# xinyandai/gradient-quantization

Measured on AMD Instinct MI355X. Metric: gradient elements quantized/sec (HSQ d=16 k=8), higher is better.
Workload: dtype f32; 1 GPU; synthetic 25,000,000-float32 flat gradient per rank, HSQ c_dim=16 k_bit=8 n_bit=6 (BASELINE configs[1]), step = encode+levels+decode-mean; elements_per_rank=25000000, random=0, ranks=1, wire_levels=bytes, wire_bytes_per_rank=3125040, inputs=3 gradients of 100 MB used in turn (never Infinity-Cache resident)

## Files before the change

### gradient-quantization_amd/build.py

```python
#!/usr/bin/env python3
import os
import shutil
import subprocess
import sys

HERE = os.path.dirname(os.path.abspath(__file__))
ROOT = os.path.dirname(HERE)
CSRC = os.path.join(HERE, "csrc")
LIB = os.path.join(HERE, "libgq_hsq.so")
TOPK_LIB = os.path.join(HERE, "libgq_topk.so")
TOPK_SOURCES = ["topk.hip"]
SIGN_LIB = os.path.join(HERE, "libgq_sign.so")
SIGN_SOURCES = ["sign.hip"]
PVQ_LIB = os.path.join(HERE, "libgq_pvq.so")
PVQ_SOURCES = ["pvq_batched.hip"]
RQ_LIB = os.path.join(HERE, "libgq_rq.so")
RQ_SOURCES = ["rq_batched.hip"]
SOURCES = ["gq_common.hip", "gq_api.hip", "hsq_encode.hip", "hsq_encode_pf.hip", "hsq_encode_pfd.hip", "hsq_levels.hip", "hsq_batched.hip", "hsq_decode.hip", "qsgd.hip", "qsgd_batched.hip", "qsgd_wide.hip", "pvq.hip"]
FLAGS = ["--offload-arch=gfx950", "-O3", "-ffp-contract=off", "-fPIC", "-shared", "-std=c++17",
         "-Xclang", "-target-feature", "-Xclang", "-packed-fp32-ops",
         "-fvisibility=hidden", "-I" + os.path.join(ROOT, "include"), "-I" + CSRC]


def hipcc():
    for c in (os.environ.get("HIPCC"), shutil.which("hipcc"), "/opt/rocm/bin/hipcc"):
        if c and os.path.exists(c):
            return c
    raise RuntimeError("hipcc not found (ROCm toolchain required)")


HOST_EXT = os.path.join(HERE, "gq_amd", "_gq_host.so")


def needs_build():
    if (not os.path.exists(LIB) or not os.path.exists(os.path.join(HERE, "libgq_hsq_clock.so")) or not os.path.exists(HOST_EXT)
            or not os.path.exists(TOPK_LIB) or not os.path.exists(SIGN_LIB) or not os.path.exists(PVQ_LIB) or not os.path.exists(RQ_LIB)):
        return True
    t = min(os.path.getmtime(LIB), os.path.getmtime(HOST_EXT), os.path.getmtime(TOPK_LIB), os.path.getmtime(SIGN_LIB), os.path.getmtime(PVQ_LIB),
            os.path.getmtime(RQ_LIB))
    deps = ([os.path.join(CSRC, f) for f in os.listdir(CSRC)] + [os.path.join(ROOT, "include", h) for h in ("gq_hsq.h", "gq_topk.h", "gq_sign.h", "gq_pvq.h", "gq_rq.h")]
            + [__file__])
    return any(os.path.getmtime(d) > t for d in deps)


EXTRA = {
    "hsq_encode_pf.hip": ["-fno-honor-nans"],
    "hsq_encode_pfd.hip": ["-fno-honor-nans", "-mllvm", "-amdgpu-mfma-vgpr-form=1"],
    "pvq.hip": ["-mllvm", "-amdgpu-mfma-vgpr-form=1"],
    "pvq_batched.hip": ["-mllvm", "-amdgpu-mfma-vgpr-form=1"],
    "rq_batched.hip": ["-mllvm", "-amdgpu-mfma-vgpr-form=1"],
}


def build(force=False, verbose=False):
    if not force and not needs_build():
        return LIB
    objdir = os.path.join(HERE, "build")
    os.makedirs(objdir, exist_ok=True)
    compile_flags = [f for f in FLAGS if f != "-shared"]
    procs = []
    for src in SOURCES:
        obj = os.path.join(objdir, src.replace(".hip", ".o"))
        cmd = [hipcc()] + compile_flags + EXTRA.get(src, []) + ["-c", os.path.join(CSRC, src), "-o", obj]
        if verbose:
            print(" ".join(cmd))
        procs.append((cmd, subprocess.Popen(cmd), obj))
    topk_objs, sign_objs, pvq_objs, rq_objs = [], [], [], []
    for srcs, own in ((TOPK_SOURCES, topk_objs), (SIGN_SOURCES, sign_objs), (PVQ_SOURCES, pvq_objs), (RQ_SOURCES, rq_objs)):
        for src in srcs:
            obj = os.path.join(objdir, src.replace(".hip", ".o"))
            cmd = [hipcc()] + compile_flags + EXTRA.get(src, []) + ["-c", os.path.join(CSRC, src), "-o", obj]
            if verbose:
                print(" ".join(cmd))
            procs.append((cmd, subprocess.Popen(cmd), obj))
            own.append(obj)
    objs = []
    for cmd, p, obj in procs:
        if p.wait() != 0:
            raise subprocess.CalledProcessError(p.returncode, cmd)
        if obj not in topk_objs and obj not in sign_objs and obj not in pvq_objs and obj not in rq_objs:
            objs.append(obj)
    link = [hipcc(), "--offload-arch=gfx950", "-shared", "-fPIC", "-o", LIB] + objs
    if verbose:
        print(" ".join(link))
    host = None
    try:
        host = build_host_ext(verbose, wait=False)
    except Exception as e:
        print("build.py: host helper not built (%s); gq_amd falls back to its Python walks" % (e,), file=sys.stderr)
    try:
        subprocess.check_call(link)
        subprocess.check_call([hipcc(), "--offload-arch=gfx950", "-shared", "-fPIC", "-o", TOPK_LIB] + topk_objs)
        subprocess.check_call([hipcc(), "--offload-arch=gfx950", "-shared", "-fPIC", "-o", SIGN_LIB] + sign_objs)
        subprocess.check_call([hipcc(), "--offload-arch=gfx950", "-shared", "-fPIC", "-o", PVQ_LIB] + pvq_objs)
        subprocess.check_call([hipcc(), "--offload-arch=gfx950", "-shared", "-fPIC", "-o", RQ_LIB] + rq_objs)
        build_clock_lib(objs, verbose)
    finally:
        if host is not None and host[1].wait() != 0:
            print("build.py: host helper failed to compile (exit %d); gq_amd falls back to its Python walks" % host[1].returncode,
                  file=sys.stderr)
    return LIB


def build_host_ext(verbose=False, wait=True):
    import sysconfig
    import torch
    from torch.utils import cpp_extension as ce
    cmd = (["g++", "-O2", "-std=c++17", "-fPIC", "-shared", "-fvisibility=hidden",
            "-D_GLIBCXX_USE_CXX11_ABI=%d" % int(torch._C._GLIBCXX_USE_CXX11_ABI)]
           + ["-I" + d for d in ce.include_paths() + [sysconfig.get_paths()["include"]]]
           + [os.path.join(CSRC, "host_ext.cpp"), "-o", HOST_EXT]
           + ["-L" + d for d in ce.library_paths()] + ["-ltorch", "-ltorch_cpu", "-ltorch_python", "-lc10"]
           + ["-Wl,-rpath," + d for d in ce.library_paths()])
    if verbose:
        print(" ".join(cmd))
    p = subprocess.Popen(cmd)
    if wait and p.wait() != 0:
        raise subprocess.CalledProcessError(p.returncode, cmd)
    return cmd, p


CLOCK_LIB = os.path.join(HERE, "libgq_hsq_clock.so")


def build_clock_lib(objs=None, verbose=False, source=None, out=None):
    objdir = os.path.join(HERE, "build")
    if objs is None:
        objs = [os.path.join(objdir, f.replace(".hip", ".o")) for f in SOURCES]
    src = source or os.path.join(CSRC, "hsq_encode_pf.hip")
    obj = os.path.join(objdir, "stamps", "hsq_encode_pf_stamps.o" if out is None else os.path.basename(out) + ".o")
    os.makedirs(os.path.dirname(obj), exist_ok=True)
    flags = [f for f in FLAGS if f != "-shared"] + EXTRA.get("hsq_encode_pf.hip", [])
    cmd = [hipcc()] + flags + ["-DGQ_PF_STAMPS", "-c", src, "-o", obj]
    if verbose:
        print(" ".join(cmd))
    subprocess.check_call(cmd, stderr=None if verbose else subprocess.DEVNULL)
    others = [o for o in objs if os.path.basename(o) != "hsq_encode_pf.o"]
    subprocess.check_call([hipcc(), "--offload-arch=gfx950", "-shared", "-fPIC", "-o", out or CLOCK_LIB, obj] + others)
    return out or CLOCK_LIB


if __name__ == "__main__":
    print(build(force="--force" in sys.argv, verbose=True))
```

### gradient-quantization_amd/csrc/gq_internal.h

```cpp
#pragma once
#include "gq_common.hpp"

GQ_INTERNAL int gqi_hsq_encode_batched_pf(const int64_t *seg_table, const int32_t *tile_seg, int nseg, int64_t ntiles,
                                          const float *codebook, int d, int K, int ef, float ef_scale, uint8_t *wire, float *u_flat,
                                          uint32_t *seg_minmax, float *workspace, int profile_slot, void *stream);
GQ_INTERNAL int gqi_hsq_encode_batched_paged(const int64_t *seg_table, const int32_t *tile_seg, int nseg, int64_t ntiles,
                                             const float *codebook, int d, int K, int ef, float ef_scale, uint8_t *wire,
                                             float *u_flat, uint32_t *seg_minmax, float *workspace, void *stream);
GQ_INTERNAL int gqi_hsq_batched_any_supported(int d, int K);
GQ_INTERNAL int gqi_hsq_encode_batched_any(const int64_t *seg_table, const int32_t *tile_seg, int nseg, int64_t ntiles,
                                           const float *codebook, int d, int K, int code_bytes, int ef, float ef_scale,
                                           uint8_t *wire, float *u_flat, uint32_t *seg_minmax, void *stream);

GQ_INTERNAL int gqi_hsq_levels_batched_d16(const int64_t *seg_table, const int32_t *tile_seg, int nseg, int64_t ntiles,
                                           const float *u_flat, const uint32_t *seg_minmax, int n_bit, int random_mode,
                                           uint64_t seed, const float *r_flat, const float *ef_codebook, int K, int packed6,
                                           uint8_t *wire, const int64_t *dense_table, int ndense, void *stream);
GQ_INTERNAL int gqi_hsq_levels_batched_ef_d(const int64_t *seg_table, const int32_t *tile_seg, int nseg, int64_t ntiles,
                                            const float *u_flat, const uint32_t *seg_minmax, int n_bit, int random_mode,
                                            uint64_t seed, const float *r_flat, const float *codebook, int d, int K, uint8_t *wire, const int64_t *dense_table, int ndense,
                                            void *stream);
GQ_INTERNAL int gqi_hsq_levels_batched_ef16(const int64_t *seg_table, const int32_t *tile_seg, int nseg, int64_t ntiles,
                                            const float *u_flat, const uint32_t *seg_minmax, int n_bit, int random_mode,
                                            uint64_t seed, const float *r_flat, const float *codebook, int d, int K, uint8_t *wire,
                                            const int64_t *dense_table, int ndense, void *stream);
GQ_INTERNAL int gqi_hsq_levels_decode_batched(const int64_t *seg_table, const int32_t *tile_seg, int nseg, int64_t ntiles,
                                              const float *u_flat, const uint32_t *seg_minmax, int n_bit, int random_mode,
                                              uint64_t seed, const float *r_flat, const float *codebook, int d, int K, int level_bytes,
                                              uint8_t *wire, const int64_t *dense_table, int ndense, int write_error, float *out,
                                              int plain, const gq::FusedTail *ft, void *stream);
GQ_INTERNAL int gqi_hsq_levels_batched_any(const int64_t *seg_table, const int32_t *tile_seg, int nseg, int64_t ntiles,
                                           const float *u_flat, const uint32_t *seg_minmax, int n_bit, int random_mode,
                                           uint64_t seed, const float *r_flat, int level_bytes, uint8_t *wire, const int64_t *dense_table, int ndense, void *stream);
GQ_INTERNAL int gqi_hsq_error_batched_any(const int64_t *seg_table, const int32_t *tile_seg, int nseg, int64_t ntiles,
                                          const uint8_t *wire, const float *codebook, int d, int K, int code_bytes,
                                          int level_bytes, int n_bit, void *stream);

GQ_INTERNAL int gqi_hsq_decode_sum_batched_d16(const int64_t *seg_table, const int32_t *tile_seg, int nseg, int64_t ntiles,
                                               const uint8_t *gathered, int64_t user_stride_bytes, int R,
                                               const float *codebook, int K, int n_bit, int packed6, float *out, int plain,
                                               const gq::StepTail *tail_or_null, int *tail_taken, void *stream);
GQ_INTERNAL int gqi_hsq_decode_sum_batched_d(const int64_t *seg_table, const int32_t *tile_seg, int nseg, int64_t ntiles,
                                             const uint8_t *gathered, int64_t user_stride_bytes, int R,
                                             const float *codebook, int d, int K, int level_bytes, int n_bit, float *out, int plain,
                                             const gq::StepTail *tail_or_null, int *tail_taken, void *stream);
GQ_INTERNAL int gqi_hsq_decode_sum_batched_any(const int64_t *seg_table, const int32_t *tile_seg, int nseg, int64_t ntiles,
                                               const uint8_t *gathered, int64_t user_stride_bytes, int R,
                                               const float *codebook, int d, int K, int code_bytes, int level_bytes,
                                               int n_bit, float *out, int plain, void *stream);

GQ_INTERNAL int gqi_qsgd_compress_batched(const int64_t *seg_table, const int32_t *bucket_seg, int nseg, int64_t nbuckets,
                                          int n_bit, int random_mode, uint64_t seed, int ef, float ef_scale, uint8_t *wire, const int64_t *dense_table, int ndense,
                                          int bucket_hint, void *stream);
GQ_INTERNAL int gqi_qsgd_decode_sum_batched(const int64_t *seg_table, const int32_t *bucket_seg, int nseg, int64_t nbuckets,
                                            int n_bit, int bits, const uint8_t *gathered, int64_t user_stride_bytes, int R,
                                            float *out, int plain, const gq::StepTail *tail_or_null, int *tail_taken, int bucket_hint,
                                            void *stream);
GQ_INTERNAL int gqi_qsgd_wide_compress(const int64_t *seg_table, const int32_t *chunk_seg, int nseg, int64_t nchunks,
                                       int n_bit, int random_mode, uint64_t seed, int ef, float ef_scale,
                                       uint32_t *norm_bits, uint8_t *wire, const int64_t *dense_table, int ndense, void *stream);
GQ_INTERNAL int gqi_qsgd_wide_decode_sum(const int64_t *seg_table, const int32_t *chunk_seg, int nseg, int64_t nchunks,
                                         int n_bit, int bits, const uint8_t *gathered, int64_t user_stride_bytes, int R,
                                         float *out, int plain, const gq::StepTail *tail_or_null, int *tail_taken, void *stream);
```

### gradient-quantization_amd/csrc/hsq_encode_pf.hip

```cpp
#include <hip/hip_ext.h>

#include <type_traits>

#include "hsq_pf_common.hpp"

#ifdef GQ_PF_STAMPS
#define GQ_STAMP(ID)                                                                                  \
    {                                                                                                 \
        __builtin_amdgcn_sched_barrier(0);                                                            \
        unsigned long long ts_;                                                                       \
        asm volatile("s_memtime %0\n\ts_waitcnt lgkmcnt(0)" : "=s"(ts_)::"memory");                   \
        __builtin_amdgcn_sched_barrier(0);                                                            \
        stamp_acc[ID] += (ts_ - ts_prev);                                                             \
        ts_prev = ts_;                                                                                \
    }
#define GQ_STAMPS_ONLY(...) __VA_ARGS__
#define GQ_LOG_SCAN(...)
#else
#define GQ_STAMP(ID)
#define GQ_STAMPS_ONLY(...)
#define GQ_LOG_SCAN(...) __VA_ARGS__
#endif

namespace gq {

constexpr int PF_WAVES = 8;
constexpr int PF_THREADS = PF_WAVES * 64;
#ifndef GQ_PF_TAIL
#define GQ_PF_TAIL 4
#endif
constexpr int PF_TAIL = GQ_PF_TAIL;
#ifndef GQ_PF_FLUSH_AHEAD
#define GQ_PF_FLUSH_AHEAD 0
#endif
#ifndef GQ_PF_PAIR
#define GQ_PF_PAIR -1
#endif
#ifndef GQ_PF_FLUSH_MIN
#define GQ_PF_FLUSH_MIN 3
#endif
#ifndef GQ_PF_SCAN1_MAX
#define GQ_PF_SCAN1_MAX 4
#endif
constexpr int PF_FLUSH_AHEAD = GQ_PF_FLUSH_AHEAD;
constexpr int PF_FLUSH_MIN = GQ_PF_FLUSH_MIN;
constexpr int PF_SCAN1_MAX = GQ_PF_SCAN1_MAX;
constexpr int PF_LDS_SEGS = 384;
template <int D>
struct PfShape {
    static_assert(D == 8 || D == 16 || D == 32, "the prefilter kernel is built for D = 8, 16 and 32");
    static constexpr int KS = D > 16 ? D / 16 : 1;
    static constexpr bool HALF = D < 16;
    static constexpr int QS = 4 * D + 4;
    static constexpr int QCAP = D > 16 ? 32 : 64;
    static constexpr bool A_REGS = D <= 16;
    static constexpr int NF = 4 * KS;
    static constexpr bool PAIR = GQ_PF_PAIR < 0 ? D > 16 : GQ_PF_PAIR != 0;
    static constexpr float ERR_REL = (D > 16 ? 1.05f : 1.03f) * 4.8828125e-04f;
    static constexpr float ERR2_REL = (D > 16 ? 2.3f : 1.2f) * 7.62939453125e-06f;
    static constexpr float ERR2_SUB = D > 16 ? 3.5e-7f : 2.4e-7f;
};
constexpr float ERR_ABS = 4.76837158203125e-07f;
constexpr unsigned N2_LO_BITS = 0x39800000u;
constexpr unsigned N2_HI_BITS = 0x4B800000u;
constexpr int SIGMA_TARGET_EXP2 = 10;

struct PfArgs {
    const float *grad;
    int64_t M;
    void *codes;
    float *u;
    const float *cb;
    float *ws;
    const int64_t *seg_table;
    const int32_t *tile_seg;
    uint8_t *wire;
    unsigned *seg_minmax;
    int64_t ntiles;
    int nseg;
    int K;
    float ef_scale;
    int tiles_q, tiles_r;
    int tiles_skew, skew_blocks;
};

#ifndef GQ_PF_SKEW_PERMILLE
#define GQ_PF_SKEW_PERMILLE 10
#endif
static void pf_split(PfArgs &a, int64_t ntiles, int64_t blocks) {
    a.tiles_q = (int)(ntiles / blocks);
    a.tiles_r = (int)(ntiles % blocks);
    a.skew_blocks = (int)(blocks & ~(int64_t)1);
    a.tiles_skew = (int)((a.tiles_q * (int64_t)GQ_PF_SKEW_PERMILLE + 500) / 1000);
    if (a.tiles_skew >= a.tiles_q) a.tiles_skew = 0;
}

template <typename CodeT, int D, bool BATCHED, bool EF = false, bool SEGLDS = true, int DR = D, int NRB = 8>
__global__ __launch_bounds__(PF_THREADS, 1) void hsq_encode_pf_kernel(const PfArgs a) {
    typedef PfShape<D> SH;
    static_assert(DR == D || (D == 16 && DR == 12) || (D == 32 && DR == 24), "padded shapes: 12 -> 16, 24 -> 32");
    static_assert(NRB == 1 || NRB == 2 || NRB == 4 || NRB == 8, "row blocks: 1, 2, 4 or 8");
    const int K = a.K;
    constexpr int KS = SH::KS, QS = SH::QS, QCAP = SH::QCAP, NF = SH::NF;
    constexpr bool HALF = SH::HALF, PF_PAIR = SH::PAIR;
    GQ_STAMPS_ONLY(const unsigned long long rt_entry = __builtin_amdgcn_s_memrealtime(); unsigned long long nscanned = 0, npassed = 0;)
    const float *__restrict__ cb = a.cb;
    float *__restrict__ ws = a.ws;
    float *__restrict__ u = a.u;
    const int64_t M = a.M;
    __shared__ __attribute__((aligned(16))) float s_cb[64 * QS];
    __shared__ int s_next;
    __shared__ int s_pairdone[PF_WAVES / 2], s_ringpub[PF_WAVES];
    __shared__ int64_t s_seg[(BATCHED && SEGLDS) ? PF_LDS_SEGS * 8 : 1];
    __shared__ __attribute__((aligned(16))) u32x4 s_frag[8 * KS * 64], s_fragl[8 * KS * 64];
    __shared__ float s_c1[PF_WAVES], s_dc[PF_WAVES];
    __shared__ __attribute__((aligned(16))) float s_qv[PF_WAVES * QCAP * D];
    __shared__ __attribute__((aligned(16))) unsigned s_qm[PF_WAVES * QCAP * 4];

    constexpr int PF_MM_SEGS = 64;
    __shared__ unsigned s_mm[BATCHED ? 2 * PF_MM_SEGS : 2];
    const int lane = threadIdx.x & 63, wave = __builtin_amdgcn_readfirstlane((int)(threadIdx.x >> 6));
    const int j = lane & 31, h = lane >> 5;

    const int64_t ntiles = BATCHED ? a.ntiles : ((M + 63) >> 6);
    const int b = (int)blockIdx.x;
    const bool skewed = b < a.skew_blocks;
    const int lo_tile = b * a.tiles_q + (b < a.tiles_r ? b : a.tiles_r) + ((skewed && (b & 1)) ? a.tiles_skew : 0);
    const int tile_end = lo_tile + a.tiles_q + (b < a.tiles_r ? 1 : 0) + (skewed ? ((b & 1) ? -a.tiles_skew : a.tiles_skew) : 0);
    const int tail_from = (tile_end - lo_tile) - (wave >= PF_WAVES / 2 ? PF_TAIL : 0);
    auto draw = [&]() {
        int k = 0x3FFFFFFF;
        if (lane == 0) {
            if (__hip_atomic_load(&s_next, __ATOMIC_RELAXED, __HIP_MEMORY_SCOPE_WORKGROUP) < tail_from)
                k = __hip_atomic_fetch_add(&s_next, 1, __ATOMIC_RELAXED, __HIP_MEMORY_SCOPE_WORKGROUP);
        }
        return lo_tile + __builtin_amdgcn_readfirstlane(k);
    };
    int t = lo_tile + wave;
    int *const worklist = ws_worklist(ws);

    float lmin = INFINITY, lmax = -INFINITY;
    bool sawnan = false;
    int cur_seg = -1;
    int seg_first = 0;
    f32x4 cur[NF], nxt[NF];
    f32x4 nxte[NF];
    if (HALF) {
#pragma unroll
        for (int i = 0; i < NF; ++i) cur[i] = nxt[i] = nxte[i] = f32x4{0.0f, 0.0f, 0.0f, 0.0f};
    }

    typedef const float __attribute__((address_space(1))) *gcf_ptr;
    typedef float __attribute__((address_space(1))) *gf_ptr;
    typedef const f32x4 __attribute__((address_space(1))) *gcv_ptr;
    typedef f32x4 __attribute__((address_space(1))) *gv_ptr;
    typedef CodeT __attribute__((address_space(1))) *gcode_ptr;
    struct Tile {
        gcf_ptr base;
        int64_t m, sv0;
        int tile0;
        int tiles_end;
        int rem;
        int seg;
        gcode_ptr codes;
        gcf_ptr err;
    };
    auto uniform64 = [](int64_t v) {
        const unsigned lo = (unsigned)__builtin_amdgcn_readfirstlane((int)(unsigned)(uint64_t)v);
        const unsigned hi = (unsigned)__builtin_amdgcn_readfirstlane((int)(unsigned)((uint64_t)v >> 32));
        return (int64_t)(((uint64_t)hi << 32) | lo);
    };
    auto tile_info = [&](int tile, int seg, auto from_global) {
        constexpr bool FROM_GLOBAL = decltype(from_global)::value;
        Tile ti;
        if (BATCHED) {
            ti.seg = seg;
            int64_t r0, r1, r2, r3, r7 = 0;
            if constexpr (SEGLDS && !FROM_GLOBAL) {
                const int64_t *rec = s_seg + 8 * seg;
                r0 = rec[0];
                r1 = rec[1];
                r2 = rec[2];
                r3 = rec[3];
                if (EF) r7 = rec[7];
            } else {
                typedef const int64_t __attribute__((address_space(1))) *grec_ptr;
                const grec_ptr rec = (grec_ptr)(a.seg_table + 8 * (int64_t)seg);
                r0 = rec[0];
                r1 = rec[1];
                r2 = rec[2];
                r3 = rec[3];
                if (EF) r7 = rec[7];
            }
            ti.base = (gcf_ptr)(uintptr_t)uniform64(r0);
            ti.m = uniform64(r1);
            ti.tile0 = (int)uniform64(r2);
            ti.tiles_end = ti.tile0 + (int)((ti.m + 63) >> 6);
            ti.sv0 = (int64_t)(tile - ti.tile0) * 64;
            ti.codes = (gcode_ptr)((uintptr_t)a.wire + (uintptr_t)uniform64(r3));
            ti.err = EF ? (gcf_ptr)(uintptr_t)uniform64(r7) : (gcf_ptr)0;
            const int rem = (int)ti.m - 1 - (int)ti.sv0;
            ti.rem = rem > 63 ? 63 : rem;
        } else {
            ti.seg = 0;
            ti.tile0 = 0;
            ti.tiles_end = 0;
            ti.base = (gcf_ptr)a.grad;
            ti.m = M;
            ti.sv0 = (int64_t)tile * 64;
            ti.codes = (gcode_ptr)static_cast<CodeT *>(a.codes);
            ti.err = (gcf_ptr)0;
            const int rem = (int)M - 1 - (int)ti.sv0;
            ti.rem = rem > 63 ? 63 : rem;
        }
        return ti;
    };
    auto lane_off = [&](const Tile &ti, int blk) {
        const unsigned li = min((unsigned)(blk * 32 + j), (unsigned)ti.rem);
        return li * (unsigned)DR + (HALF ? 0u : 8u * (unsigned)h);
    };
    auto frag_ok = [&](int s_, int q_) { return DR == D || 16 * s_ + 4 * q_ + 4 + 8 * h <= DR; };
    const bool loads_here = !HALF || h == 0;
    auto load_rows = [&](gcf_ptr tb, const Tile &ti, f32x4(&dst)[NF]) {
        if (loads_here) {
#pragma unroll
            for (int blk = 0; blk < 2; ++blk) {
                const gcv_ptr p = (gcv_ptr)(tb + lane_off(ti, blk));
#pragma unroll
                for (int s = 0; s < KS; ++s) {
                    const f32x4 z = {0.0f, 0.0f, 0.0f, 0.0f};
                    dst[(blk * KS + s) * 2] = frag_ok(s, 0) ? p[4 * s] : z;
                    dst[(blk * KS + s) * 2 + 1] = frag_ok(s, 1) ? p[4 * s + 1] : z;
                }
            }
        }
    };
    auto load_tile = [&](const Tile &ti, f32x4(&dst)[NF]) { load_rows(ti.base + ti.sv0 * DR, ti, dst); };
    auto load_err = [&](const Tile &ti, f32x4(&dst)[NF]) {
        if (EF && ti.err) load_rows(ti.err + ti.sv0 * DR, ti, dst);
    };
    auto fold_err = [&](const Tile &ti, f32x4(&g)[NF], const f32x4(&e)[NF]) {
        if (EF && ti.err) {
            const gf_ptr tb = (gf_ptr)(ti.base + ti.sv0 * DR);
#pragma unroll
            for (int blk = 0; blk < 2; ++blk) {
#pragma unroll
                for (int q = 0; q < 2 * KS; ++q) {
                    f32x4 &x = g[2 * KS * blk + q];
                    const f32x4 &y = e[2 * KS * blk + q];
#pragma unroll
                    for (int c = 0; c < 4; ++c) {
                        const float prod = a.ef_scale * y[c];
                        x[c] = x[c] + prod;
                    }
                }
                if (blk * 32 + j <= ti.rem && loads_here) {
                    const gv_ptr p = (gv_ptr)(tb + (unsigned)((blk * 32 + j) * DR + (HALF ? 0 : 8 * h)));
#pragma unroll
                    for (int s = 0; s < KS; ++s) {
                        if (frag_ok(s, 0)) p[4 * s] = g[(blk * KS + s) * 2];
                        if (frag_ok(s, 1)) p[4 * s + 1] = g[(blk * KS + s) * 2 + 1];
                    }
                }
            }
        }
    };
    auto mm_fold = [&](int seg, unsigned mlo, unsigned mhi) {
        const unsigned idx = (unsigned)(seg - seg_first);
        if (idx < (unsigned)PF_MM_SEGS) {
            atomicMin(&s_mm[2 * idx], mlo);
            atomicMax(&s_mm[2 * idx + 1], mhi);
        } else {
            unsigned *mm = a.seg_minmax + 2 * seg;
            if (mlo < __hip_atomic_load(mm, __ATOMIC_RELAXED, __HIP_MEMORY_SCOPE_AGENT)) atomicMin(mm, mlo);
            if (mhi > __hip_atomic_load(mm + 1, __ATOMIC_RELAXED, __HIP_MEMORY_SCOPE_AGENT)) atomicMax(mm + 1, mhi);
        }
    };
    auto flush_minmax = [&]() {
        const float lo = wave_min(lmin), hi = wave_max(lmax);
        if (lane == 0 && cur_seg >= 0 && lo <= hi) mm_fold(cur_seg, order_map(lo), order_map(hi));
        lmin = INFINITY;
        lmax = -INFINITY;
    };

    half8 vh[2 * KS];
    float n2p[2] = {0.0f, 0.0f};
    Tile ti = {};

    float cbv[256 * DR / PF_THREADS];
#pragma unroll
    for (int n = 0; n < 256 * DR / PF_THREADS; ++n) cbv[n] = (int)threadIdx.x + n * PF_THREADS < K * DR ? cb[threadIdx.x + n * PF_THREADS] : 0.0f;
    f32x4 aq[2 * KS];
#pragma unroll
    for (int i = 0; i < 2 * KS; ++i) aq[i] = f32x4{0.0f, 0.0f, 0.0f, 0.0f};
    if (loads_here && wave * 32 + j < K) {
#pragma unroll
        for (int s = 0; s < KS; ++s) {
            if (frag_ok(s, 0)) aq[2 * s] = *reinterpret_cast<const f32x4 *>(cb + (wave * 32 + j) * DR + 16 * s + (HALF ? 0 : 8 * h));
            if (frag_ok(s, 1)) aq[2 * s + 1] = *reinterpret_cast<const f32x4 *>(cb + (wave * 32 + j) * DR + 16 * s + (HALF ? 0 : 8 * h) + 4);
        }
    }
    const int seg_first_v = (BATCHED && lo_tile < ntiles) ? a.tile_seg[lo_tile] : 0;
    if (t < tile_end) {
        ti = tile_info(t, BATCHED ? __builtin_amdgcn_readfirstlane(a.tile_seg[t]) : 0, std::true_type{});
        load_tile(ti, cur);
        load_err(ti, nxte);
    }
    if (threadIdx.x == 0) {
        s_next = PF_WAVES;
    }
    if (threadIdx.x < PF_WAVES / 2) s_pairdone[threadIdx.x] = 0;
    seg_first = BATCHED ? __builtin_amdgcn_readfirstlane(seg_first_v) : 0;
    if (BATCHED && threadIdx.x < PF_MM_SEGS) {
        s_mm[2 * threadIdx.x] = 0xFFFFFFFFu;
        s_mm[2 * threadIdx.x + 1] = 0u;
    }
#pragma unroll
    for (int n = 0; n < 256 * DR / PF_THREADS; ++n) {
        const int i = threadIdx.x + n * PF_THREADS, k = i / DR, jj = i % DR;
        s_cb[(k >> 2) * QS + 4 * jj + (k & 3)] = cbv[n];
    }
    if constexpr (DR != D) {
#pragma unroll
        for (int n = 0; n < 256 * (D - DR) / PF_THREADS; ++n) {
            const int i = threadIdx.x + n * PF_THREADS, k = i / (D - DR), jj = DR + i % (D - DR);
            s_cb[(k >> 2) * QS + 4 * jj + (k & 3)] = 0.0f;
        }
    }
    if (BATCHED && SEGLDS) {
        const int n = (a.nseg < PF_LDS_SEGS ? a.nseg : PF_LDS_SEGS) * 8;
        for (int i = threadIdx.x; i < n; i += PF_THREADS) s_seg[i] = a.seg_table[i];
    }
    {
        float l2 = 0.0f, d2 = 0.0f;
#pragma unroll
        for (int s = 0; s < KS; ++s) {
            half8 fh, fl;
#pragma unroll
            for (int e = 0; e < 8; ++e) {
                const float x = e < 4 ? aq[2 * s][e] : aq[2 * s + 1][e - 4];
                fh[e] = (_Float16)x;
                const float rr = x - (float)fh[e];
                fl[e] = (_Float16)rr;
                l2 = __fmaf_rn(x, x, l2);
                d2 = __fmaf_rn(rr, rr, d2);
            }
            s_frag[(wave * KS + s) * 64 + lane] = __builtin_bit_cast(u32x4, fh);
            s_fragl[(wave * KS + s) * 64 + lane] = __builtin_bit_cast(u32x4, fl);
        }
        l2 += __shfl_xor(l2, 32, 64);
        d2 += __shfl_xor(d2, 32, 64);
        l2 = wave_max_nan(l2);
        d2 = wave_max_nan(d2);
        if (lane == 0) {
            s_c1[wave] = l2;
            s_dc[wave] = d2;
        }
    }
    __syncthreads();
    half8 ch[SH::A_REGS ? 8 : 1];
    if constexpr (SH::A_REGS) {
#pragma unroll
        for (int rb = 0; rb < 8; ++rb) ch[rb] = __builtin_bit_cast(half8, s_frag[rb * 64 + lane]);
    }
    auto frag_hi = [&](int rb, int s) -> half8 {
        if constexpr (SH::A_REGS) return ch[rb];
        else return __builtin_bit_cast(half8, s_frag[(rb * KS + s) * 64 + lane]);
    };
    unsigned c2b = __float_as_uint(s_c1[0]), dcb = __float_as_uint(s_dc[0]);
#pragma unroll
    for (int w = 1; w < PF_WAVES; ++w) {
        c2b = max(c2b, __float_as_uint(s_c1[w]));
        dcb = max(dcb, __float_as_uint(s_dc[w]));
    }
    const float c2 = __builtin_sqrtf(__uint_as_float(c2b)) * 1.0000002f, dc = __builtin_sqrtf(__uint_as_float(dcb)) * 1.0000002f;
    const bool cb_ok = c2b < 0x4E800000u && dcb < 0x4E800000u;
    const float err_rel = cb_ok ? c2 * SH::ERR_REL + 1.001f * dc : INFINITY;
    const float err_abs = cb_ok ? c2 * ERR_ABS : INFINITY;
    const float err2_rel = cb_ok ? c2 * SH::ERR2_REL + SH::ERR2_SUB : INFINITY;

    int tn = draw();
    float sigma_t = 1.0f;
    if (t < tile_end) {
        fold_err(ti, cur, nxte);
        float m = 0.0f;
#pragma unroll
        for (int i = 0; i < NF; ++i) m = fmaxf(fmaxf(fabsf(cur[i][0]), fabsf(cur[i][1])), fmaxf(fmaxf(fabsf(cur[i][2]), fabsf(cur[i][3])), m));
        const unsigned em = (unsigned)__builtin_amdgcn_readfirstlane((int)(__float_as_uint(wave_max(m)) >> 23));
        if (em >= 1u && em <= 254u) {
            int f = 258 - (int)em;
            f = f < 27 ? 27 : (f > 227 ? 227 : f);
            sigma_t = __uint_as_float((unsigned)__builtin_amdgcn_readfirstlane(f << 23));
        }
#pragma unroll
        for (int blk = 0; blk < 2; ++blk)
#pragma unroll
            for (int s = 0; s < KS; ++s) scale8_f16(cur[(blk * KS + s) * 2], cur[(blk * KS + s) * 2 + 1], sigma_t, vh[blk * KS + s], n2p[blk]);
    }
    auto fold_seg = [&](int seg, float v) {
        const unsigned mv = order_map(v);
        mm_fold(seg, mv, mv);
    };
    auto poison_seg = [&](int seg) {
        atomicMin(a.seg_minmax + 2 * seg, MAPPED_NAN_LO);
        atomicMax(a.seg_minmax + 2 * seg + 1, MAPPED_NAN_HI);
    };
    int qhead = 0, qcnt = 0;
    bool flushed = false;
    const int run_len = tile_end - lo_tile;
    auto scan1 = [&](int slot) {
        GQ_STAMPS_ONLY(nscanned += 1;)
        float w[D];
        {
            const f32x4 *qv = reinterpret_cast<const f32x4 *>(s_qv + D * slot);
#pragma unroll
            for (int q = 0; q < D / 4; ++q) {
                const f32x4 x = qv[q];
                w[4 * q] = x[0];
                w[4 * q + 1] = x[1];
                w[4 * q + 2] = x[2];
                w[4 * q + 3] = x[3];
            }
        }
        f32x4 p = exact_score_quad<D>(s_cb + lane * QS, w);
        if (4 * lane >= K) p = f32x4{0.0f, 0.0f, 0.0f, 0.0f};
        float bv = p[0];
        int bi = 4 * lane;
        take_if_greater_nan(bv, bi, p[1], 4 * lane + 1);
        take_if_greater_nan(bv, bi, p[2], 4 * lane + 2);
        take_if_greater_nan(bv, bi, p[3], 4 * lane + 3);
        wave_first_max_nan_dpp(bv, bi);
        const bool isnan = nan_bits(bv);
        if (isnan) sawnan = true;
        if (lane == 0) {
            const u32x4 m = *reinterpret_cast<const u32x4 *>(s_qm + 4 * slot);
            *(gcode_ptr)(uintptr_t)((uint64_t)m[0] | ((uint64_t)m[1] << 32)) = (CodeT)bi;
            ((gf_ptr)u)[m[2]] = bv;
            if (BATCHED) {
                if (isnan) poison_seg((int)m[3]);
                else fold_seg((int)m[3], bv);
            } else {
                GQ_LOG_SCAN(worklist[m[2]] = (int)m[2];)
                lmin = fminf(lmin, bv);
                lmax = fmaxf(lmax, bv);
            }
        }
    };
    auto second_pass = [&](int first, int na, int wave_b, int first_b, int nb) {
        const int n = na + nb;
        GQ_STAMPS_ONLY(npassed += n;)
        auto slot_of = [&](int c) {
            return c < na ? wave * QCAP + ((first + c) & (QCAP - 1)) : wave_b * QCAP + ((first_b + c - na) & (QCAP - 1));
        };
        const int col = j < n ? j : 0;
        const int slot = slot_of(col);
        const f32x4 *qv = reinterpret_cast<const f32x4 *>(s_qv + D * slot);
        f32x4 xs[2 * KS];
#pragma unroll
        for (int s = 0; s < KS; ++s) {
            if (HALF) {
                const f32x4 z = {0.0f, 0.0f, 0.0f, 0.0f};
                xs[0] = h ? z : qv[0];
                xs[1] = h ? z : qv[1];
            } else {
                xs[2 * s] = qv[4 * s + 2 * h];
                xs[2 * s + 1] = qv[4 * s + 2 * h + 1];
            }
        }
        auto both_halves = [&](float own, bool add) {
            float a = own, b = own;
            swap32(a, b);
            return add ? a + b : fmaxf(a, b);
        };
        float m = 0.0f;
#pragma unroll
        for (int i = 0; i < 2 * KS; ++i)
            m = fmaxf(fmaxf(fmaxf(fabsf(xs[i][0]), fabsf(xs[i][1])), fmaxf(fabsf(xs[i][2]), fabsf(xs[i][3]))), m);
        m = both_halves(m, false);
        const unsigned em = __float_as_uint(m) >> 23;
        int f = 258 - (int)em;
        f = f < 27 ? 27 : (f > 227 ? 227 : f);
        const float sig = (em >= 1u && em <= 254u) ? __uint_as_float((unsigned)f << 23) : 1.0f;
        half8 bh[KS], bl[KS];
        float n2q = 0.0f;
#pragma unroll
        for (int s = 0; s < KS; ++s) {
            u32x4 H, L;
            const f32x4 x0 = xs[2 * s], x1 = xs[2 * s + 1];
#pragma unroll
            for (int i = 0; i < 4; ++i) {
                const float a = i < 2 ? x0[2 * i] : x1[2 * i - 4], b = i < 2 ? x0[2 * i + 1] : x1[2 * i - 3];
                unsigned r, l;
                asm("v_fma_mixlo_f16 %0, %1, %2, 0" : "=v"(r) : "v"(a), "v"(sig));
                asm("v_fma_mixhi_f16 %0, %1, %2, 0" : "+v"(r) : "v"(b), "v"(sig));
                asm("v_fma_mixlo_f16 %0, %1, %2, -%3 op_sel_hi:[0,0,1]" : "=v"(l) : "v"(a), "v"(sig), "v"(r));
                asm("v_fma_mixhi_f16 %0, %1, %2, -%3 op_sel:[0,0,1] op_sel_hi:[0,0,1]" : "+v"(l) : "v"(b), "v"(sig), "v"(r));
                const unsigned e = r & 0x7C007C00u;
                asm("v_dot2_f32_f16 %0, %1, %1, %0" : "+v"(n2q) : "v"(e));
                H[i] = r;
                L[i] = l;
            }
            bh[s] = __builtin_bit_cast(half8, H);
            bl[s] = __builtin_bit_cast(half8, L);
        }
        const float n2 = both_halves(n2q, true);
        unsigned best2[2] = {0, 0}, second2[2] = {0, 0};
        unsigned vmask = KEY_MASK;
        asm volatile("" : "+v"(vmask));
        half8 al[KS], ah[KS];
        auto frags_of = [&](int rb) {
#pragma unroll
            for (int s = 0; s < KS; ++s) {
                al[s] = __builtin_bit_cast(half8, s_fragl[(rb * KS + s) * 64 + lane]);
                ah[s] = frag_hi(rb, s);
            }
        };
        auto chain3 = [&](f32x16 c) {
#pragma unroll
            for (int s = 0; s < KS; ++s) {
                c = __builtin_amdgcn_mfma_f32_32x32x16_f16(al[s], bh[s], c, 0, 0, 0);
                c = __builtin_amdgcn_mfma_f32_32x32x16_f16(ah[s], bl[s], c, 0, 0, 0);
                c = __builtin_amdgcn_mfma_f32_32x32x16_f16(ah[s], bh[s], c, 0, 0, 0);
            }
            return c;
        };
        frags_of(0);
        f32x16 acc = {0};
        acc = chain3(acc);
        if (NRB > 1) frags_of(1);
#pragma unroll
        for (int rb = 0; rb < NRB; ++rb) {
            f32x16 nacc = {0};
            if (rb + 1 < NRB) {
                __builtin_amdgcn_sched_barrier(0);
                nacc = chain3(nacc);
                if (rb + 2 < NRB) frags_of(rb + 2);
                __builtin_amdgcn_sched_barrier(0);
            }
            unsigned k[4];
#pragma unroll
            for (int q = 0; q < 4; ++q)
                k[q] = and_or(__float_as_uint(absmax4(acc[4 * q], acc[4 * q + 1], acc[4 * q + 2], acc[4 * q + 3])), vmask,
                              (unsigned)((rb & 3) * 4 + q));
            const int trk = rb >> 2;
            const unsigned t0 = max3u(best2[trk], k[0], k[1]), a0 = med3u(best2[trk], k[0], k[1]);
            const unsigned b0 = med3u(t0, k[2], k[3]);
            best2[trk] = max3u(t0, k[2], k[3]);
            second2[trk] = max3u(second2[trk], a0, b0);
            __builtin_amdgcn_sched_barrier(0);
            acc = nacc;
        }
        const bool useB = (best2[1] & KEY_MASK) > (best2[0] & KEY_MASK);
        const unsigned bw = useB ? best2[1] : best2[0], blo = useB ? best2[0] : best2[1];
        const int gid = (int)(bw & 31u);
        const int kmine = ((gid >> 2) + (useB ? 4 : 0)) * 32 + 8 * (gid & 3) + 4 * h;
        const unsigned smine = max3u(second2[0], second2[1], blo) | 31u;
        int k0 = kmine, k1_ = kmine;
        swap32(k0, k1_);
        int s0 = (int)smine, s1 = (int)smine;
        swap32(s0, s1);
        int w0 = (int)bw, w1 = (int)bw;
        swap32(w0, w1);
        const bool pick1 = ((unsigned)w1 & KEY_MASK) > ((unsigned)w0 & KEY_MASK);
        const int kc = pick1 ? k1_ : k0;
        const unsigned rest = max3u((unsigned)s0, (unsigned)s1, (unsigned)(pick1 ? w0 : w1) | 31u);
        float vf[D];
#pragma unroll
        for (int q = 0; q < D / 4; ++q) {
            const f32x4 x = qv[q];
            vf[4 * q] = x[0];
            vf[4 * q + 1] = x[1];
            vf[4 * q + 2] = x[2];
            vf[4 * q + 3] = x[3];
        }
        const f32x4 p4 = exact_score_quad<D>(s_cb + (kc >> 2) * QS, vf);
        float val = p4[0];
        int idx = kc;
        take_if_greater(val, idx, p4[1], kc + 1);
        take_if_greater(val, idx, p4[2], kc + 2);
        take_if_greater(val, idx, p4[3], kc + 3);
        const unsigned n2b = __float_as_uint(n2);
        const float E = __builtin_amdgcn_sqrtf(n2) * err2_rel + err_abs;
        bool safe = ((n2b - N2_LO_BITS) <= (N2_HI_BITS - N2_LO_BITS)) && (__uint_as_float(rest) + E < fabsf(val * sig));
        if (nan_bits(val)) safe = false;
        const bool owner = h == 0 && j < n;
        if (owner && safe) {
            const u32x4 mt = *reinterpret_cast<const u32x4 *>(s_qm + 4 * slot);
            *(gcode_ptr)(uintptr_t)((uint64_t)mt[0] | ((uint64_t)mt[1] << 32)) = (CodeT)idx;
            ((gf_ptr)u)[mt[2]] = val;
            if (BATCHED) {
                fold_seg((int)mt[3], val);
            } else {
                GQ_LOG_SCAN(worklist[mt[2]] = (int)mt[2];)
                lmin = fminf(lmin, val);
                lmax = fmaxf(lmax, val);
            }
        }
        uint64_t left = __ballot(owner && !safe);
        while (left) {
            const int i = __builtin_ctzll(left);
            left &= left - 1;
            scan1(slot_of(i));
        }
    };
    GQ_STAMPS_ONLY(const unsigned long long rt0 = __builtin_amdgcn_s_memrealtime(); unsigned long long ntl = 0, stamp_acc[6] = {0, 0, 0, 0, 0, 0}, ts_prev;
                   asm volatile("s_memtime %0\n\ts_waitcnt lgkmcnt(0)" : "=s"(ts_prev)::"memory");)
    while (t < tile_end) {
        auto chain_rb = [](int c) { return SH::A_REGS ? (c % NRB) : (c >> 1); };
        auto chain_blk = [](int c) { return SH::A_REGS ? (c / NRB) : (c & 1); };
        half8 af[2][KS];
        if constexpr (!SH::A_REGS) {
#pragma unroll
            for (int s = 0; s < KS; ++s) af[0][s] = frag_hi(0, s);
        }
        auto chain = [&](int c, f32x16 x) {
            const int rb = chain_rb(c), blk = chain_blk(c);
#pragma unroll
            for (int s = 0; s < KS; ++s)
                x = __builtin_amdgcn_mfma_f32_32x32x16_f16(SH::A_REGS ? ch[SH::A_REGS ? rb : 0] : af[rb & 1][s], vh[blk * KS + s], x, 0, 0, 0);
            return x;
        };
        f32x16 acc = {0};
        acc = chain(0, acc);
        __builtin_amdgcn_sched_barrier(0);
        Tile tin = ti;
        if (tn < tile_end) {
            if (BATCHED && tn >= ti.tile0 && tn < ti.tiles_end) {
                tin.sv0 = (int64_t)(tn - ti.tile0) * 64;
                const int rem = (int)ti.m - 1 - (int)tin.sv0;
                tin.rem = rem > 63 ? 63 : rem;
            } else {
                tin = tile_info(tn, BATCHED ? __builtin_amdgcn_readfirstlane(a.tile_seg[tn]) : 0, std::false_type{});
            }
            load_tile(tin, nxt);
            load_err(tin, nxte);
        }
        if (BATCHED && ti.seg != cur_seg) {
            flush_minmax();
            cur_seg = ti.seg;
        }
        GQ_STAMP(0)
        unsigned best[4] = {0, 0, 0, 0}, second[4] = {0, 0, 0, 0};
        unsigned vmask = KEY_MASK;
        asm volatile("" : "+v"(vmask));
        auto group_key = [&](const f32x16 &a, int rb, int q) {
            return and_or(__float_as_uint(absmax4(a[4 * q], a[4 * q + 1], a[4 * q + 2], a[4 * q + 3])), vmask,
                          (unsigned)((rb & 3) * 4 + q));
        };
        unsigned trk_t = 0, trk_a = 0;
        auto track_lo = [&](int trk, unsigned k0, unsigned k1) {
            trk_t = max3u(best[trk], k0, k1);
            trk_a = med3u(best[trk], k0, k1);
        };
        auto track_hi = [&](int trk, unsigned k2, unsigned k3) {
            const unsigned b = med3u(trk_t, k2, k3);
            best[trk] = max3u(trk_t, k2, k3);
            second[trk] = max3u(second[trk], trk_a, b);
        };
#pragma unroll
        for (int c = 0; c < 2 * NRB; ++c) {
            const int rb = chain_rb(c), trk = chain_blk(c) * 2 + (rb >> 2);
            if constexpr (!SH::A_REGS) {
                if (chain_blk(c) == 0 && rb + 1 < NRB) {
#pragma unroll
                    for (int s = 0; s < KS; ++s) af[(rb + 1) & 1][s] = frag_hi(rb + 1, s);
                }
            }
            if (c + 1 < 2 * NRB) {
                f32x16 nacc = {0};
                __builtin_amdgcn_sched_barrier(0);
                nacc = chain(c + 1, nacc);
                __builtin_amdgcn_sched_barrier(0);
                track_lo(trk, group_key(acc, rb, 0), group_key(acc, rb, 1));
                track_hi(trk, group_key(acc, rb, 2), group_key(acc, rb, 3));
                __builtin_amdgcn_sched_barrier(0);
                acc = nacc;
            } else {
                track_lo(trk, group_key(acc, rb, 0), group_key(acc, rb, 1));
                track_hi(trk, group_key(acc, rb, 2), group_key(acc, rb, 3));
            }
        }

        GQ_STAMP(1)
        int k1[2];
        unsigned s2[2], bk[2];
#pragma unroll
        for (int blk = 0; blk < 2; ++blk) {
            const unsigned bA = best[2 * blk], bB = best[2 * blk + 1];
            const bool useB = (bB & KEY_MASK) > (bA & KEY_MASK);
            const unsigned bw = useB ? bB : bA, bl = useB ? bA : bB;
            const int gid = (int)(bw & 31u);
            k1[blk] = ((gid >> 2) + (useB ? 4 : 0)) * 32 + 8 * (gid & 3) + 4 * h;
            s2[blk] = max3u(second[2 * blk], second[2 * blk + 1], bl) | 31u;
            bk[blk] = bw;
        }

        float vf[D];
#pragma unroll
        for (int s = 0; s < KS; ++s) {
#pragma unroll
            for (int e = 0; e < 8; ++e) {
                float x = cur[2 * s + (e >> 2)][e & 3];
                float y = cur[2 * KS + 2 * s + (e >> 2)][e & 3];
                swap32(x, y);
                vf[16 * s + e] = x;
                if (!HALF) vf[(16 * s + 8 + e) % D] = y;
            }
        }
        swap32(k1[0], k1[1]);
        {
            int a0 = (int)s2[0], a1 = (int)s2[1];
            swap32(a0, a1);
            s2[0] = (unsigned)a0;
            s2[1] = (unsigned)a1;
            int b0 = (int)bk[0], b1 = (int)bk[1];
            swap32(b0, b1);
            bk[0] = (unsigned)b0;
            bk[1] = (unsigned)b1;
        }
        float n2 = n2p[0];
        {
            float n2o = n2p[1];
            swap32(n2, n2o);
            n2 += n2o;
        }
        const unsigned n2b = __float_as_uint(n2);

        GQ_STAMP(2)
        const bool pick1 = (bk[1] & KEY_MASK) > (bk[0] & KEY_MASK);
        const int kc = pick1 ? k1[1] : k1[0];
        const unsigned rest = max3u(s2[0], s2[1], (pick1 ? bk[0] : bk[1]) | 31u);
        const f32x4 p4 = exact_score_quad<D>(s_cb + (kc >> 2) * QS, vf);
        float val = p4[0];
        int idx = kc;
        take_if_greater(val, idx, p4[1], kc + 1);
        take_if_greater(val, idx, p4[2], kc + 2);
        take_if_greater(val, idx, p4[3], kc + 3);

        const float E = __builtin_amdgcn_sqrtf(n2) * err_rel + err_abs;
        const float others = __uint_as_float(rest);
        const bool in_window = (n2b - N2_LO_BITS) <= (N2_HI_BITS - N2_LO_BITS);
        bool safe = in_window && (others + E < fabsf(val * sigma_t));
        if (nan_bits(val)) safe = false;
        if (__ballot(n2b == 0u)) {
            unsigned any = 0;
#pragma unroll
            for (int e = 0; e < D; e += 2) any |= (__float_as_uint(vf[e]) | __float_as_uint(vf[e + 1])) & 0x7FFFFFFFu;
            if (any == 0u && !nan_bits(val)) {
                safe = true;
                val = 0.0f;
                idx = 0;
            }
        }

        const bool valid = lane <= ti.rem;

        float sigma_n = sigma_t;
        {
            const unsigned s0 = (unsigned)__builtin_amdgcn_readlane((int)n2b, 5), s1 = (unsigned)__builtin_amdgcn_readlane((int)n2b, 58);
            const unsigned smp = s0 > s1 ? s0 : s1;
            if (smp != 0u) {
                const int e2 = (int)(smp >> 23);
                const int k = e2 >= 255 ? -16 : ((127 + SIGMA_TARGET_EXP2 - e2) >> 1);
                int f = (int)((unsigned)__builtin_amdgcn_readfirstlane((int)__float_as_uint(sigma_t)) >> 23) + k;
                f = f < 27 ? 27 : (f > 227 ? 227 : f);
                sigma_n = __uint_as_float((unsigned)f << 23);
            }
        }

        GQ_STAMP(3)
        int dk_seen = 0x3FFFFFFF;
        if (lane == 0) dk_seen = __hip_atomic_load(&s_next, __ATOMIC_RELAXED, __HIP_MEMORY_SCOPE_WORKGROUP);
        half8 nvh[2 * KS];
        float nn2p[2] = {0.0f, 0.0f};
        if (EF && tn < tile_end) fold_err(tin, nxt, nxte);
#pragma unroll
        for (int blk = 0; blk < 2; ++blk)
#pragma unroll
            for (int s = 0; s < KS; ++s) scale8_f16(nxt[(blk * KS + s) * 2], nxt[(blk * KS + s) * 2 + 1], sigma_n, nvh[blk * KS + s], nn2p[blk]);
#pragma unroll
        for (int i = 0; i < NF; ++i) cur[i] = nxt[i];
#pragma unroll
        for (int i = 0; i < 2 * KS; ++i) vh[i] = nvh[i];
#pragma unroll
        for (int blk = 0; blk < 2; ++blk) n2p[blk] = nn2p[blk];
        __builtin_amdgcn_sched_barrier(0);

        GQ_STAMP(4)
        int dk_next = 0x3FFFFFFF;
        if (lane == 0 && dk_seen < tail_from) dk_next = __hip_atomic_fetch_add(&s_next, 1, __ATOMIC_RELAXED, __HIP_MEMORY_SCOPE_WORKGROUP);
        const bool flagged = valid && !safe;
        uint64_t todo = __ballot(flagged);
        bool want_flush = PF_FLUSH_AHEAD > 0 && !flushed && (tn - lo_tile) >= run_len - PF_FLUSH_AHEAD;
        while (todo || want_flush) {
            const int rank = (int)__builtin_amdgcn_mbcnt_hi((unsigned)(todo >> 32), __builtin_amdgcn_mbcnt_lo((unsigned)todo, 0u));
            const bool mine = ((todo >> lane) & 1) && rank < QCAP - qcnt;
            if (mine) {
                const int slot = wave * QCAP + ((qhead + qcnt + rank) & (QCAP - 1));
                f32x4 *qv = reinterpret_cast<f32x4 *>(s_qv + D * slot);
#pragma unroll
                for (int q = 0; q < D / 4; ++q) qv[q] = f32x4{vf[4 * q], vf[4 * q + 1], vf[4 * q + 2], vf[4 * q + 3]};
                const uint64_t ca = (uint64_t)(uintptr_t)(ti.codes + ti.sv0) + (uint64_t)sizeof(CodeT) * (unsigned)lane;
                *reinterpret_cast<u32x4 *>(s_qm + 4 * slot) =
                    u32x4{(unsigned)ca, (unsigned)(ca >> 32), (unsigned)((BATCHED ? (int64_t)t * 64 : ti.sv0) + lane), (unsigned)ti.seg};
            }
            const uint64_t took = __ballot(mine);
            qcnt += (int)__builtin_popcountll(took);
            todo &= ~took;
            if (qcnt >= 32 || (want_flush && !todo)) {
                if (qcnt >= 32 || qcnt >= PF_FLUSH_MIN) {
                    const int n = qcnt < 32 ? qcnt : 32;
                    second_pass(qhead, n, wave, 0, 0);
                    qhead = (qhead + n) & (QCAP - 1);
                    qcnt -= n;
                    if (want_flush && !todo) flushed = true;
                }
                if (!todo) want_flush = false;
            }
        }

        if (valid && safe) {
            (ti.codes + ti.sv0)[(unsigned)lane] = (CodeT)idx;
            ((gf_ptr)u + (BATCHED ? (int64_t)t * 64 : ti.sv0))[(unsigned)lane] = val;
            lmin = fminf(lmin, val);
            lmax = fmaxf(lmax, val);
        }
        ti = tin;
        t = tn;
        tn = lo_tile + __builtin_amdgcn_readfirstlane(dk_next);
        sigma_t = sigma_n;
        GQ_STAMP(5)
        GQ_STAMPS_ONLY(++ntl;)
    }
    GQ_STAMPS_ONLY(const unsigned long long rt1 = __builtin_amdgcn_s_memrealtime();)
    if (BATCHED) flush_minmax();

    int other_first = 0, other_n = 0;
    const int partner = wave ^ (PF_WAVES / 2);
    if (PF_PAIR) {
        int old = 0;
        if (lane == 0) {
            __hip_atomic_store(&s_ringpub[wave], (qhead << 8) | qcnt, __ATOMIC_RELAXED, __HIP_MEMORY_SCOPE_WORKGROUP);
            old = __hip_atomic_fetch_add(&s_pairdone[wave & (PF_WAVES / 2 - 1)], 1, __ATOMIC_ACQ_REL, __HIP_MEMORY_SCOPE_WORKGROUP);
        }
        old = __builtin_amdgcn_readfirstlane(old);
        if (old == 0) {
            qcnt = 0;
        } else {
            int pub = 0;
            if (lane == 0) pub = __hip_atomic_load(&s_ringpub[partner], __ATOMIC_RELAXED, __HIP_MEMORY_SCOPE_WORKGROUP);
            pub = __builtin_amdgcn_readfirstlane(pub);
            other_first = pub >> 8;
            other_n = pub & 255;
        }
    }
    while (qcnt + other_n) {
        if (qcnt + other_n <= PF_SCAN1_MAX) {
            if (qcnt) {
                scan1(wave * QCAP + qhead);
                qhead = (qhead + 1) & (QCAP - 1);
                qcnt -= 1;
            } else {
                scan1(partner * QCAP + other_first);
                other_first = (other_first + 1) & (QCAP - 1);
                other_n -= 1;
            }
        } else {
            const int na = qcnt < 32 ? qcnt : 32, nb = other_n < 32 - na ? other_n : 32 - na;
            second_pass(qhead, na, partner, other_first, nb);
            qhead = (qhead + na) & (QCAP - 1);
            qcnt -= na;
            other_first = (other_first + nb) & (QCAP - 1);
            other_n -= nb;
        }
    }
#ifdef GQ_PF_STAMPS
    if (lane == 0 && blockIdx.x < 256) {
        unsigned long long *o = reinterpret_cast<unsigned long long *>(ws_worklist(ws) + (M - 65536)) + (blockIdx.x * 8 + wave) * 12;
        for (int i = 0; i < 6; ++i) o[i] = stamp_acc[i];
        o[6] = rt_entry, o[7] = rt0, o[8] = rt1, o[9] = ntl, o[10] = __builtin_amdgcn_s_memrealtime(), o[11] = 1000 * nscanned + npassed;
    }
#endif
    if (BATCHED) {
        __syncthreads();
        if (threadIdx.x < PF_MM_SEGS) {
            const unsigned lo = s_mm[2 * threadIdx.x], hi = s_mm[2 * threadIdx.x + 1];
            if (lo != 0xFFFFFFFFu || hi != 0u) {
                unsigned *mm = a.seg_minmax + 2 * (seg_first + (int)threadIdx.x);
                if (lo < __hip_atomic_load(mm, __ATOMIC_RELAXED, __HIP_MEMORY_SCOPE_AGENT)) atomicMin(mm, lo);
                if (hi > __hip_atomic_load(mm + 1, __ATOMIC_RELAXED, __HIP_MEMORY_SCOPE_AGENT)) atomicMax(mm + 1, hi);
            }
        }
        return;
    }
    write_minmax_partials<PF_WAVES>(lmin, lmax, ws, sawnan);
}

static int64_t pf16_grid(int64_t ntiles, int bpc) {
    int64_t blocks = (ntiles + PF_WAVES - 1) / PF_WAVES;
    int64_t cap = (int64_t)cu_count() * bpc;
    if (cap > GQ_MAIN_PARTIALS) cap = GQ_MAIN_PARTIALS;
    if (blocks > cap) blocks = cap;
    return blocks < 1 ? 1 : blocks;
}

template <typename CodeT, int D, int DR, int NRB>
static int launch_pf_rows(const float *grad, const float *codebook, int64_t M, int K, CodeT *codes, float *u, float *ws,
                          hipStream_t st, int profile_slot) {
    if (M > 0x7FFFFFFFLL) return fail(GQ_ERR_UNSUPPORTED, "gq_hsq_encode: prefilter path needs M < 2^31");
    static const int bpc = resident_blocks_per_cu(hsq_encode_pf_kernel<CodeT, D, false, false, true, DR, NRB>, PF_THREADS, 0);
    PfArgs a = {};
    a.grad = grad;
    a.M = M;
    a.codes = codes;
    a.u = u;
    a.cb = codebook;
    a.ws = ws;
    a.K = K;
    const int64_t blocks = pf16_grid((M + 63) / 64, bpc);
    pf_split(a, (M + 63) / 64, blocks);
    hipEvent_t ev_start, ev_stop;
    if (profile_events(profile_slot, &ev_start, &ev_stop)) {
        hipExtLaunchKernelGGL(HIP_KERNEL_NAME(hsq_encode_pf_kernel<CodeT, D, false, false, true, DR, NRB>), dim3((unsigned)blocks),
                              dim3(PF_THREADS), 0, st, ev_start, ev_stop, 0, a);
    } else {
        hipLaunchKernelGGL(HIP_KERNEL_NAME(hsq_encode_pf_kernel<CodeT, D, false, false, true, DR, NRB>), dim3((unsigned)blocks),
                           dim3(PF_THREADS), 0, st, a);
    }
    GQ_CHECK_LAUNCH("gq_hsq_encode (prefilter)");
    return GQ_OK;
}

template <typename CodeT, int D, int DR = D>
static int launch_pf(const float *grad, const float *codebook, int64_t M, int K, CodeT *codes, float *u, float *ws,
                     hipStream_t st, int profile_slot) {
    if constexpr (sizeof(CodeT) == 1) {
        if (K <= 32) return launch_pf_rows<CodeT, D, DR, 1>(grad, codebook, M, K, codes, u, ws, st, profile_slot);
        if (K <= 64) return launch_pf_rows<CodeT, D, DR, 2>(grad, codebook, M, K, codes, u, ws, st, profile_slot);
    }
    return launch_pf_rows<CodeT, D, DR, 8>(grad, codebook, M, K, codes, u, ws, st, profile_slot);
}

template <typename CodeT>
int launch_encode_pf(const float *grad, const float *codebook, int64_t M, int d, int K, CodeT *codes, float *u, float *ws,
                     hipStream_t st, int profile_slot) {
    if (K < 4 || K > 256 || (K & 3)) return fail(GQ_ERR_INVALID_ARG, "gq_hsq_encode: the prefilter kernel was asked for K = %d", K);
    if (d == 16) return launch_pf<CodeT, 16>(grad, codebook, M, K, codes, u, ws, st, profile_slot);
    if (d == 32) return launch_pf<CodeT, 32>(grad, codebook, M, K, codes, u, ws, st, profile_slot);
    if (d == 8) return launch_pf<CodeT, 8>(grad, codebook, M, K, codes, u, ws, st, profile_slot);
    if (d == 12) return launch_pf<CodeT, 16, 12>(grad, codebook, M, K, codes, u, ws, st, profile_slot);
    if (d == 24) return launch_pf<CodeT, 32, 24>(grad, codebook, M, K, codes, u, ws, st, profile_slot);
    return fail(GQ_ERR_INVALID_ARG, "gq_hsq_encode: the prefilter kernel was asked for d = %d", d);
}

template int launch_encode_pf<uint8_t>(const float *, const float *, int64_t, int, int, uint8_t *, float *, float *, hipStream_t, int);
template int launch_encode_pf<int32_t>(const float *, const float *, int64_t, int, int, int32_t *, float *, float *, hipStream_t, int);

}

namespace gq {
template <int D, bool EF, int DR, int NRB>
static int encode_batched_rows(const char *what, const int64_t *seg_table, const int32_t *tile_seg, int nseg, int64_t ntiles,
                               const float *codebook, int K, uint8_t *wire, float *u_flat, uint32_t *seg_minmax, float *workspace,
                               float ef_scale, int profile_slot, void *stream) {
    if (nseg < 1 || ntiles < 1 || ntiles * 64 > 0x7FFFFFFFLL)
        return fail(GQ_ERR_INVALID_ARG, "%s: bad sizes nseg=%d ntiles=%lld", what, nseg, (long long)ntiles);
    if (!seg_table || !tile_seg || !codebook || !wire || !u_flat || !seg_minmax || !workspace)
        return fail(GQ_ERR_INVALID_ARG, "%s: null pointer", what);
    static const int bpc = resident_blocks_per_cu(hsq_encode_pf_kernel<uint8_t, D, true, EF, true, DR, NRB>, PF_THREADS, 0);
    PfArgs a = {};
    a.K = K;
    a.M = ntiles * 64;
    a.u = u_flat;
    a.cb = codebook;
    a.ws = workspace;
    a.seg_table = seg_table;
    a.tile_seg = tile_seg;
    a.wire = wire;
    a.seg_minmax = seg_minmax;
    a.ntiles = ntiles;
    a.nseg = nseg;
    a.ef_scale = ef_scale;
    hipStream_t st = as_stream(stream);
    const int64_t blocks = pf16_grid(ntiles, bpc);
    pf_split(a, ntiles, blocks);
    hipEvent_t ev_start, ev_stop;
    if (nseg <= PF_LDS_SEGS && profile_events(profile_slot, &ev_start, &ev_stop)) {
        hipExtLaunchKernelGGL(HIP_KERNEL_NAME(hsq_encode_pf_kernel<uint8_t, D, true, EF, true, DR, NRB>), dim3((unsigned)blocks),
                              dim3(PF_THREADS), 0, st, ev_start, ev_stop, 0, a);
    } else if (nseg <= PF_LDS_SEGS) {
        hipLaunchKernelGGL(HIP_KERNEL_NAME(hsq_encode_pf_kernel<uint8_t, D, true, EF, true, DR, NRB>), dim3((unsigned)blocks),
                           dim3(PF_THREADS), 0, st, a);
    } else {
        hipLaunchKernelGGL(HIP_KERNEL_NAME(hsq_encode_pf_kernel<uint8_t, D, true, EF, false, DR, 8>), dim3((unsigned)blocks),
                           dim3(PF_THREADS), 0, st, a);
    }
    GQ_CHECK_LAUNCH(what);
    return GQ_OK;
}

template <int D, bool EF, int DR = D>
static int encode_batched(const char *what, const int64_t *seg_table, const int32_t *tile_seg, int nseg, int64_t ntiles,
                          const float *codebook, int K, uint8_t *wire, float *u_flat, uint32_t *seg_minmax, float *workspace,
                          float ef_scale, int profile_slot, void *stream) {
    if (K <= 32 && nseg <= PF_LDS_SEGS)
        return encode_batched_rows<D, EF, DR, 1>(what, seg_table, tile_seg, nseg, ntiles, codebook, K, wire, u_flat, seg_minmax, workspace, ef_scale, profile_slot, stream);
    if (K <= 64 && nseg <= PF_LDS_SEGS)
        return encode_batched_rows<D, EF, DR, 2>(what, seg_table, tile_seg, nseg, ntiles, codebook, K, wire, u_flat, seg_minmax, workspace, ef_scale, profile_slot, stream);
    return encode_batched_rows<D, EF, DR, 8>(what, seg_table, tile_seg, nseg, ntiles, codebook, K, wire, u_flat, seg_minmax, workspace, ef_scale, profile_slot, stream);
}
}

namespace gq {
int launch_pfd_batched_paged(const int64_t *seg_table, const int32_t *tile_seg, int nseg, int64_t ntiles,
                             const float *codebook, int d, int K, int ef, float ef_scale, uint8_t *wire, float *u_flat,
                             uint32_t *seg_minmax, float *ws, hipStream_t st);

}

GQ_INTERNAL int gqi_hsq_encode_batched_paged(const int64_t *seg_table, const int32_t *tile_seg, int nseg, int64_t ntiles,
                                       const float *codebook, int d, int K, int ef, float ef_scale, uint8_t *wire,
                                       float *u_flat, uint32_t *seg_minmax, float *workspace, void *stream) {
    if (nseg < 1 || ntiles < 1 || ntiles * 64 > 0x7FFFFFFFLL)
        return gq::fail(GQ_ERR_INVALID_ARG, "gq_hsq_encode_batched (paged): bad sizes nseg=%d ntiles=%lld", nseg,
                        (long long)ntiles);
    if (!seg_table || !tile_seg || !codebook || !wire || !u_flat || !seg_minmax || !workspace)
        return gq::fail(GQ_ERR_INVALID_ARG, "gq_hsq_encode_batched (paged): null pointer");
    if ((d != 8 && d != 16 && d != 32) || K <= 256 || (K & 255) != 0 || K > 65536)
        return gq::fail(GQ_ERR_UNSUPPORTED, "gq_hsq_encode_batched (paged): d must be 8, 16 or 32 and K a multiple of 256 above 256");
    if (nseg > (d == 16 ? gq::PF_LDS_SEGS : 384))
        return gq::fail(GQ_ERR_UNSUPPORTED, "gq_hsq_encode_batched (paged): at most 384 tensors per launch");
    hipStream_t st = gq::as_stream(stream);
    return gq::launch_pfd_batched_paged(seg_table, tile_seg, nseg, ntiles, codebook, d, K, ef, ef_scale, wire, u_flat,
                                        seg_minmax, workspace, st);
}

GQ_INTERNAL int gqi_hsq_encode_batched_pf(const int64_t *seg_table, const int32_t *tile_seg, int nseg, int64_t ntiles,
                                          const float *codebook, int d, int K, int ef, float ef_scale, uint8_t *wire, float *u_flat,
                                          uint32_t *seg_minmax, float *workspace, int profile_slot, void *stream) {
    const char *what = "gq_hsq_encode_batched";
    if (K < 4 || K > 256 || (K & 3)) return gq::fail(GQ_ERR_UNSUPPORTED, "%s: the prefilter launch takes K <= 256, a multiple of 4 (K = %d)", what, K);
#define GQ_PF_BATCHED(DD, DP)                                                                                             \
    if (d == DD)                                                                                                          \
        return ef ? gq::encode_batched<DP, true, DD>(what, seg_table, tile_seg, nseg, ntiles, codebook, K, wire, u_flat, seg_minmax, \
                                                     workspace, ef_scale, profile_slot, stream)                           \
                  : gq::encode_batched<DP, false, DD>(what, seg_table, tile_seg, nseg, ntiles, codebook, K, wire, u_flat, seg_minmax, \
                                                      workspace, 0.0f, profile_slot, stream);
    GQ_PF_BATCHED(16, 16)
    GQ_PF_BATCHED(32, 32)
    GQ_PF_BATCHED(8, 8)
    GQ_PF_BATCHED(12, 16)
    GQ_PF_BATCHED(24, 32)
#undef GQ_PF_BATCHED
    return gq::fail(GQ_ERR_UNSUPPORTED, "%s: d must be 8, 12, 16, 24 or 32 (K <= 256)", what);
}
```

### gradient-quantization_amd/gq_amd/native.py

```python
import ctypes
import os

import torch

_PKG_DIR = os.path.dirname(os.path.dirname(os.path.abspath(__file__)))
LIB_PATH = os.environ.get("GQ_LIB_PATH") or os.path.join(_PKG_DIR, "libgq_hsq.so")

GQ_MAX_PARTIALS = 1024
WS_LOG_FIRST = 2 * GQ_MAX_PARTIALS + 4
GQ_FIXUP_PARTIALS = 256
RANDOM_OFF, RANDOM_GIVEN, RANDOM_DEVICE, RANDOM_DEVICE_KEYED, RANDOM_DEVICE_COUNTER = 0, 1, 2, 3, 4
ENCODE_AUTO, ENCODE_MFMA_D16K256, ENCODE_MFMA_GENERIC, ENCODE_VALU, ENCODE_PREFILTER_D16K256 = 0, 1, 2, 3, 4
ENCODE_MFMA_LDS = 5
TICKET_WORDS = 544

EXPORTS = [
    "gq_abi_version", "gq_last_error", "gq_device_info", "gq_hsq_workspace_bytes", "gq_profile_read",
    "gq_hsq_encode", "gq_hsq_encode_ex", "gq_hsq_levels", "gq_minmax_partials", "gq_hsq_decode_sum", "gq_hsq_decode_sum_strided",
    "gq_hsq_levels_decode",
    "gq_hsq_batched_path", "gq_hsq_encode_batched", "gq_hsq_levels_batched", "gq_hsq_decode_sum_batched", "gq_hsq_decode_sum_batched_tail",
    "gq_hsq_levels_decode_batched",
    "gq_axpy_inplace", "gq_sub", "gq_mean_rows", "gq_qsgd_compress", "gq_qsgd_decode_sum", "gq_qsgd_code_bits",
    "gq_qsgd_compress_batched", "gq_qsgd_decode_sum_batched", "gq_qsgd_decode_sum_batched_tail", "gq_pvq_encode",
    "gq_launch_plan_create", "gq_launch_plan_run", "gq_launch_plan_destroy",
]
ABI_VERSION = 5
ERR_INVALID_ARG, ERR_UNSUPPORTED, ERR_HIP = -1, -2, -3

_lib = None


class GQNativeError(RuntimeError):
    pass


def lib():
    global _lib
    if _lib is None:
        if not os.path.exists(LIB_PATH):
            raise GQNativeError(
                "libgq_hsq.so not found at %s -- build it with `python gradient-quantization_amd/build.py` "
                "(there is no CPU fallback)" % LIB_PATH)
        L = ctypes.CDLL(LIB_PATH)
        L.gq_last_error.restype = ctypes.c_char_p
        L.gq_abi_version.restype = ctypes.c_int
        L.gq_hsq_workspace_bytes.restype = ctypes.c_size_t
        L.gq_launch_plan_destroy.restype = None
        for name in EXPORTS:
            getattr(L, name)
        if L.gq_abi_version() != ABI_VERSION:
            raise GQNativeError("%s has ABI version %d, this binding is written for %d: rebuild it"
                                % (LIB_PATH, L.gq_abi_version(), ABI_VERSION))
        _lib = L
    return _lib


CALLS = [0]


def _check(rc, what):
    CALLS[0] += 1
    if rc != 0:
        raise GQNativeError("%s failed (%d): %s" % (what, rc, lib().gq_last_error().decode()))


def _dev_ptr(t, dtype=None, name="tensor"):
    if not isinstance(t, torch.Tensor):
        raise TypeError("%s must be a torch.Tensor" % name)
    if t.device.type != "cuda":
        raise GQNativeError("%s is on %s: the HIP kernels need a tensor in MI355X HBM (no CPU fallback)"
                            % (name, t.device))
    if t.device.index != torch._C._cuda_getDevice():
        raise GQNativeError("%s is on %s but the current device is cuda:%d: wrap the call in torch.cuda.device(...) "
                            "or call torch.cuda.set_device first" % (name, t.device, torch._C._cuda_getDevice()))
    if dtype is not None and t.dtype != dtype:
        raise TypeError("%s must be %s, got %s" % (name, dtype, t.dtype))
    if not t.is_contiguous():
        raise ValueError("%s must be contiguous" % name)
    return ctypes.c_void_p(t.data_ptr())


def _stream():
    try:
        return ctypes.c_void_p(torch._C._cuda_getCurrentRawStream(torch._C._cuda_getDevice()))
    except AttributeError:
        return ctypes.c_void_p(torch.cuda.current_stream().cuda_stream)


_CODE_BYTES = {torch.uint8: 1, torch.int32: 4}
AGGREGATE_FMA = 0x100
LEVELS_PACKED6 = -6
PACKED6 = "packed6"
_LEVEL_BYTES = {torch.uint8: 1, torch.int16: 2, torch.int32: 4, torch.float32: 0, PACKED6: LEVELS_PACKED6}


def packed6_bytes(M):
    return 3 * ((int(M) + 3) // 4)


def packed6_alloc_bytes(M):
    return packed6_bytes(M) + 1


def workspace_floats(M):
    nbytes = int(lib().gq_hsq_workspace_bytes(ctypes.c_int64(int(M))))
    return (nbytes + 3) // 4


def new_workspace(device, M=0):
    return torch.zeros(workspace_floats(M), dtype=torch.float32, device=device)


def fixup_count(workspace, M):
    wl = workspace[WS_LOG_FIRST:WS_LOG_FIRST + M].view(torch.int32)
    return int((wl >= 0).sum().item())


def mark_worklist(workspace, M):
    workspace[WS_LOG_FIRST:WS_LOG_FIRST + M].view(torch.int32).fill_(-1)


def profile_read(slot):
    ms = ctypes.c_float(0.0)
    _check(lib().gq_profile_read(ctypes.c_int(slot), ctypes.byref(ms)), "gq_profile_read")
    return ms.value


def device_info(device=0):
    cus = ctypes.c_int(0)
    arch = ctypes.create_string_buffer(128)
    _check(lib().gq_device_info(ctypes.c_int(device), ctypes.byref(cus), arch, ctypes.c_size_t(128)), "gq_device_info")
    return cus.value, arch.value.decode()


def hsq_encode(grad, codebook, codes, u, partials, impl=ENCODE_AUTO, profile_slot=-1):
    K, d = codebook.shape
    M = grad.numel() // d
    assert grad.numel() == M * d and codes.numel() == M and u.numel() == M
    assert partials.numel() >= workspace_floats(M), "encode workspace too small: use native.new_workspace(device, M)"
    rc = lib().gq_hsq_encode_ex(_dev_ptr(grad, torch.float32, "grad"), _dev_ptr(codebook, torch.float32, "codebook"),
                                ctypes.c_int64(M), ctypes.c_int(d), ctypes.c_int(K), _dev_ptr(codes, None, "codes"),
                                ctypes.c_int(_CODE_BYTES[codes.dtype]), _dev_ptr(u, torch.float32, "u"),
                                _dev_ptr(partials, torch.float32, "partials"), ctypes.c_int(impl), ctypes.c_int(profile_slot),
                                _stream())
    _check(rc, "gq_hsq_encode")


def hsq_compress(grad, codebook, codes, u, workspace, n_bit, random_mode, r, seed, lb_ub, levels, packed6=False):
    hsq_encode(grad, codebook, codes, u, workspace)
    hsq_levels(u, n_bit, random_mode, r, seed, workspace, lb_ub, levels, packed6)


def hsq_levels(u, n_bit, random_mode, r, seed, partials, lb_ub, levels, packed6=False):
    M = u.numel()
    assert lb_ub.numel() == 2
    if packed6:
        assert levels.dtype == torch.uint8 and levels.numel() >= packed6_bytes(M)
    else:
        assert levels.numel() == M
    rp = _dev_ptr(r, torch.float32, "r") if r is not None else ctypes.c_void_p(0)
    if r is not None:
        assert r.numel() == M
    rc = lib().gq_hsq_levels(_dev_ptr(u, torch.float32, "u"), ctypes.c_int64(M), ctypes.c_int(n_bit),
                             ctypes.c_int(random_mode), rp, ctypes.c_uint64(seed & (2 ** 64 - 1)),
                             _dev_ptr(partials, torch.float32, "partials"), _dev_ptr(lb_ub, torch.float32, "lb_ub"),
                             _dev_ptr(levels, None, "levels"),
                             ctypes.c_int(LEVELS_PACKED6 if packed6 else _LEVEL_BYTES[levels.dtype]), _stream())
    _check(rc, "gq_hsq_levels")


def hsq_levels_decode(u, n_bit, random_mode, r, seed, partials, lb_ub, levels, codes, codebook, out, packed6=False):
    M = u.numel()
    K, d = codebook.shape
    if (d != 16 or K > 256 or codes.dtype != torch.uint8 or (not packed6 and levels.dtype != torch.uint8)
            or u.data_ptr() % 4 or codes.data_ptr() % 4 or (not packed6 and levels.data_ptr() % 4) or out.data_ptr() % 16
            or codebook.data_ptr() % 16):
        return False
    assert lb_ub.numel() == 2 and codes.numel() == M and out.numel() == M * d
    if packed6:
        assert levels.dtype == torch.uint8 and levels.numel() >= packed6_bytes(M)
    else:
        assert levels.numel() == M
    rp = _dev_ptr(r, torch.float32, "r") if r is not None else ctypes.c_void_p(0)
    if r is not None:
        assert r.numel() == M
    rc = lib().gq_hsq_levels_decode(_dev_ptr(u, torch.float32, "u"), ctypes.c_int64(M), ctypes.c_int(n_bit),
                                    ctypes.c_int(random_mode), rp, ctypes.c_uint64(seed & (2 ** 64 - 1)),
                                    _dev_ptr(partials, torch.float32, "partials"), _dev_ptr(lb_ub, torch.float32, "lb_ub"),
                                    _dev_ptr(levels, None, "levels"), ctypes.c_int(LEVELS_PACKED6 if packed6 else 1),
                                    _dev_ptr(codes, None, "codes"), _dev_ptr(codebook, torch.float32, "codebook"),
                                    ctypes.c_int(K), _dev_ptr(out, torch.float32, "out"), _stream())
    if rc == ERR_UNSUPPORTED:
        return False
    _check(rc, "gq_hsq_levels_decode")
    return True


def minmax_partials(v, partials):
    _check(lib().gq_minmax_partials(_dev_ptr(v, torch.float32, "v"), ctypes.c_int64(v.numel()),
                                    _dev_ptr(partials, torch.float32, "partials"), _stream()), "gq_minmax_partials")


def hsq_decode_sum(codes, levels, lb_ub, codebook, n_bit, out, R=1):
    K, d = codebook.shape
    M = codes.numel() // R
    assert codes.numel() == R * M and levels.numel() == R * M and out.numel() == M * d
    lvl_bytes = _LEVEL_BYTES[levels.dtype]
    if lvl_bytes:
        assert lb_ub is not None and lb_ub.numel() == 2 * R
        lp = _dev_ptr(lb_ub, torch.float32, "lb_ub")
    else:
        lp = ctypes.c_void_p(0)
    rc = lib().gq_hsq_decode_sum(_dev_ptr(codes, None, "codes"), ctypes.c_int(_CODE_BYTES[codes.dtype]),
                                 _dev_ptr(levels, None, "levels"), ctypes.c_int(lvl_bytes), lp,
                                 _dev_ptr(codebook, torch.float32, "codebook"), ctypes.c_int(R), ctypes.c_int64(M),
                                 ctypes.c_int(d), ctypes.c_int(K), ctypes.c_int(n_bit if lvl_bytes else 0),
                                 _dev_ptr(out, torch.float32, "out"), _stream())
    _check(rc, "gq_hsq_decode_sum")


def hsq_decode_sum_packed(wire, M, codebook, n_bit, out, R, codes_off=0, levels_off=None, lbub_off=None,
                          code_dtype=torch.uint8, level_dtype=torch.uint8):
    K, d = codebook.shape
    assert wire.dtype == torch.uint8 and wire.dim() == 2 and wire.shape[0] == R and wire.is_contiguous()
    P = wire.shape[1]
    cb_, lb_ = _CODE_BYTES[code_dtype], _LEVEL_BYTES[level_dtype]
    assert out.numel() == M * d
    if level_dtype == PACKED6:
        assert levels_off + packed6_bytes(M) + 1 <= P, "a packed level section must be followed by one more byte of its row"
    base = wire.data_ptr()
    _dev_ptr(wire, torch.uint8, "wire")
    rc = lib().gq_hsq_decode_sum_strided(
        ctypes.c_void_p(base + codes_off), ctypes.c_int(cb_), ctypes.c_int64(P),
        ctypes.c_void_p(base + levels_off), ctypes.c_int(lb_), ctypes.c_int64(P),
        ctypes.c_void_p(base + lbub_off), ctypes.c_int64(P),
        _dev_ptr(codebook, torch.float32, "codebook"), ctypes.c_int(R), ctypes.c_int64(M), ctypes.c_int(d),
        ctypes.c_int(K), ctypes.c_int(n_bit), _dev_ptr(out, torch.float32, "out"), _stream())
    _check(rc, "gq_hsq_decode_sum_strided")


class _HSQBatchStruct(ctypes.Structure):
    _fields_ = [("struct_bytes", ctypes.c_uint32), ("d", ctypes.c_int32), ("K", ctypes.c_int32),
                ("code_bytes", ctypes.c_int32), ("level_bytes", ctypes.c_int32), ("n_bit", ctypes.c_int32),
                ("nseg", ctypes.c_int32), ("profile_slot", ctypes.c_int32), ("ntiles", ctypes.c_int64),
                ("seg_table", ctypes.c_void_p), ("tile_seg", ctypes.c_void_p), ("codebook", ctypes.c_void_p),
                ("u_flat", ctypes.c_void_p), ("seg_minmax", ctypes.c_void_p), ("workspace", ctypes.c_void_p),
                ("dense_table", ctypes.c_void_p), ("ndense", ctypes.c_int32), ("reserved", ctypes.c_int32)]


_NAN = float("nan")
BATCH_PREFILTER, BATCH_PAGED, BATCH_EXACT = 1, 2, 3


class HSQBatch(object):

    def __init__(self, seg_table, tile_seg, nseg, ntiles, codebook, code_dtype, level_dtype, n_bit, u_flat=None,
                 seg_minmax=None, workspace=None):
        self.L = lib()
        self.keep = (seg_table, tile_seg, codebook, u_flat, seg_minmax, workspace)
        self.device = seg_table.device.index
        K, d = int(codebook.shape[0]), int(codebook.shape[1])
        if workspace is not None:
            assert workspace.numel() >= workspace_floats(ntiles * 64)
        opt = lambda t, dt, nm: _dev_ptr(t, dt, nm).value if t is not None else None
        self.s = _HSQBatchStruct(ctypes.sizeof(_HSQBatchStruct), d, K, _CODE_BYTES[code_dtype], _LEVEL_BYTES[level_dtype],
                                 int(n_bit), int(nseg), -1, int(ntiles), _dev_ptr(seg_table, torch.int64, "seg_table").value,
                                 _dev_ptr(tile_seg, torch.int32, "tile_seg").value,
                                 _dev_ptr(codebook, torch.float32, "codebook").value, opt(u_flat, torch.float32, "u_flat"),
                                 opt(seg_minmax, torch.int32, "seg_minmax"), opt(workspace, torch.float32, "workspace"), None, 0, 0)
        self.ref = ctypes.byref(self.s)
        self.path = int(self.L.gq_hsq_batched_path(self.ref))

    def set_table(self, seg_table):
        self.keep_table = seg_table
        self.s.seg_table = _dev_ptr(seg_table, torch.int64, "seg_table").value

    def set_dense(self, dense_table, ndense):
        self.keep_dense = dense_table
        self.s.dense_table = _dev_ptr(dense_table, torch.int64, "dense_table").value if dense_table is not None else None
        self.s.ndense = int(ndense) if dense_table is not None else 0

    def part(self, seg_table, tile_seg, nseg, ntiles):
        codebook = self.keep[2]
        code_dtype = {v: k for k, v in _CODE_BYTES.items()}[self.s.code_bytes]
        level_dtype = {v: k for k, v in _LEVEL_BYTES.items()}[self.s.level_bytes]
        return HSQBatch(seg_table, tile_seg, nseg, ntiles, codebook, code_dtype, level_dtype, self.s.n_bit)

    def _wire(self, wire):
        if wire.device.index != self.device or wire.device.index != torch._C._cuda_getDevice():
            raise GQNativeError("wire is on %s, this batch's launches are for cuda:%d (the current device must match)"
                                % (wire.device, self.device))
        return ctypes.c_void_p(wire.data_ptr())

    def encode(self, wire, ef_scale=None, profile_slot=-1):
        self.s.profile_slot = profile_slot
        rc = self.L.gq_hsq_encode_batched(self.ref, self._wire(wire), ctypes.c_float(_NAN if ef_scale is None else ef_scale),
                                          _stream())
        self.s.profile_slot = -1
        _check(rc, "gq_hsq_encode_batched")

    def levels(self, wire, random_mode, seed, r_flat=None, write_error=False):
        rp = _dev_ptr(r_flat, torch.float32, "r_flat") if r_flat is not None else ctypes.c_void_p(0)
        rc = self.L.gq_hsq_levels_batched(self.ref, self._wire(wire), ctypes.c_int(random_mode),
                                          ctypes.c_uint64(seed & (2 ** 64 - 1)), rp, ctypes.c_int(1 if write_error else 0),
                                          _stream())
        _check(rc, "gq_hsq_levels_batched")

    def levels_decode(self, wire, random_mode, seed, r_flat, write_error, out, plain=False, tail=None):
        rp = _dev_ptr(r_flat, torch.float32, "r_flat") if r_flat is not None else ctypes.c_void_p(0)
        rc = self.L.gq_hsq_levels_decode_batched(self.ref, self._wire(wire), ctypes.c_int(random_mode), ctypes.c_uint64(seed & (2 ** 64 - 1)), rp,
                                                 ctypes.c_int(1 if write_error else 0), _dev_ptr(out, torch.float32, "out"),
                                                 ctypes.c_int(1 if plain else 0), tail.ref if tail is not None else None, _stream())
        _check(rc, "gq_hsq_levels_decode_batched")

    def decode(self, gathered, R, out, plain=False, fma=False, tail=None):
        assert gathered.dtype == torch.uint8 and gathered.dim() == 2 and gathered.shape[0] == R and gathered.stride(1) == 1
        stride = int(gathered.stride(0)) if R > 1 else int(gathered.shape[1])
        if tail is not None:
            rc = self.L.gq_hsq_decode_sum_batched_tail(self.ref, self._wire(gathered), ctypes.c_int64(stride), ctypes.c_int(R),
                                                       _dev_ptr(out, torch.float32, "out"),
                                                       ctypes.c_int(1 if plain else (2 if fma else 0)), tail.ref, _stream())
            _check(rc, "gq_hsq_decode_sum_batched_tail")
            return
        rc = self.L.gq_hsq_decode_sum_batched(self.ref, self._wire(gathered), ctypes.c_int64(stride), ctypes.c_int(R),
                                              _dev_ptr(out, torch.float32, "out"),
                                              ctypes.c_int(1 if plain else (2 if fma else 0)), _stream())
        _check(rc, "gq_hsq_decode_sum_batched")


def hsq_batched_path(d, K, code_dtype, nseg=1):
    s = _HSQBatchStruct(ctypes.sizeof(_HSQBatchStruct), int(d), int(K), _CODE_BYTES[code_dtype], 1, 6, int(nseg), -1, 1, 1, 1, 1,
                        None, None, None, None, 0, 0)
    return int(lib().gq_hsq_batched_path(ctypes.byref(s)))


class _StepTailStruct(ctypes.Structure):
    _fields_ = [("struct_bytes", ctypes.c_uint32), ("rows_R", ctypes.c_int32), ("rows", ctypes.c_void_p),
                ("row_stride_bytes", ctypes.c_int64), ("n", ctypes.c_int64), ("out", ctypes.c_void_p),
                ("rng_state", ctypes.c_void_p), ("reset_dst", ctypes.c_void_p), ("reset_src", ctypes.c_void_p),
                ("rng_pairs", ctypes.c_int32), ("reset_words", ctypes.c_int32), ("ticket", ctypes.c_void_p)]


class StepTail(object):

    def __init__(self, rows=None, out=None, rng_state=None, reset=None, ticket=None):
        self.keep = (rows, out, rng_state, reset, ticket)
        R, n, stride, rp, op = 1, 0, 0, None, None
        if rows is not None:
            assert rows.dtype == torch.float32 and rows.dim() == 2 and rows.stride(1) == 1
            R, n = int(rows.shape[0]), int(rows.shape[1])
            stride = int(rows.stride(0)) * 4 if R > 1 else n * 4
            rp, op = rows.data_ptr(), _dev_ptr(out, torch.float32, "out").value
        sp, pairs = (rng_state.data_ptr(), int(rng_state.shape[0])) if rng_state is not None else (None, 0)
        rd, rs, rw = _reset_args(reset)
        self.s = _StepTailStruct(ctypes.sizeof(_StepTailStruct), R, rp, stride, n, op, sp, rd.value, rs.value, pairs, rw.value,
                                 _dev_ptr(ticket, torch.int32, "ticket").value if ticket is not None else None)
        self.ref = ctypes.byref(self.s)


def _reset_args(reset):
    if reset is None:
        return ctypes.c_void_p(0), ctypes.c_void_p(0), ctypes.c_int(0)
    dst, src = reset
    assert dst.dtype == torch.int64 and src.dtype == torch.int64 and dst.numel() == src.numel() and dst.is_contiguous() and src.is_contiguous()
    return _dev_ptr(dst, torch.int64, "reset_dst"), _dev_ptr(src, torch.int64, "reset_src"), ctypes.c_int(int(dst.numel()))


def mean_rows(rows, out, rng_state=None, reset=None):
    assert rows.dtype == torch.float32 and rows.dim() == 2 and rows.stride(1) == 1
    R, n = int(rows.shape[0]), int(rows.shape[1])
    stride = int(rows.stride(0)) * 4 if R > 1 else n * 4
    if rows.device.index != torch._C._cuda_getDevice():
        raise GQNativeError("rows are on %s but the current device is cuda:%d" % (rows.device, torch._C._cuda_getDevice()))
    sp, pairs = (ctypes.c_void_p(rng_state.data_ptr()), int(rng_state.shape[0])) if rng_state is not None else (ctypes.c_void_p(0), 0)
    _check(lib().gq_mean_rows(ctypes.c_void_p(rows.data_ptr()), ctypes.c_int64(stride), ctypes.c_int(R), ctypes.c_int64(n),
                                   _dev_ptr(out, torch.float32, "out"), sp, ctypes.c_int(pairs), *_reset_args(reset), _stream()), "gq_mean_rows")


def rng_step(rng_state, reset=None):
    assert rng_state.dtype == torch.int64 and rng_state.dim() == 2 and rng_state.shape[1] == 2 and rng_state.is_contiguous()
    _check(lib().gq_mean_rows(ctypes.c_void_p(0), ctypes.c_int64(0), ctypes.c_int(1), ctypes.c_int64(0), ctypes.c_void_p(0),
                              ctypes.c_void_p(rng_state.data_ptr()), ctypes.c_int(int(rng_state.shape[0])), *_reset_args(reset), _stream()),
           "gq_mean_rows (step)")



class _QSGDBatchStruct(ctypes.Structure):
    _fields_ = [("struct_bytes", ctypes.c_uint32), ("n_bit", ctypes.c_int32), ("bits", ctypes.c_int32),
                ("wide", ctypes.c_int32), ("nseg", ctypes.c_int32), ("bucket_hint", ctypes.c_int32), ("nitems", ctypes.c_int64),
                ("seg_table", ctypes.c_void_p), ("item_seg", ctypes.c_void_p), ("norm_bits", ctypes.c_void_p),
                ("dense_table", ctypes.c_void_p), ("ndense", ctypes.c_int32), ("reserved2", ctypes.c_int32)]


class QSGDBatch(object):

    def __init__(self, seg_table, item_seg, nseg, nitems, n_bit, bits, wide=False, norm_bits=None, bucket_hint=0):
        self.L = lib()
        self.keep = (seg_table, item_seg, norm_bits)
        self.s = _QSGDBatchStruct(ctypes.sizeof(_QSGDBatchStruct), int(n_bit), int(bits), 1 if wide else 0, int(nseg), int(bucket_hint),
                                  int(nitems), _dev_ptr(seg_table, torch.int64, "seg_table").value,
                                  _dev_ptr(item_seg, torch.int32, "item_seg").value,
                                  _dev_ptr(norm_bits, torch.int32, "norm_bits").value if norm_bits is not None else None, None, 0, 0)
        self.ref = ctypes.byref(self.s)

    def set_table(self, seg_table):
        self.keep_table = seg_table
        self.s.seg_table = _dev_ptr(seg_table, torch.int64, "seg_table").value

    def set_dense(self, dense_table, ndense):
        self.keep_dense = dense_table
        self.s.dense_table = _dev_ptr(dense_table, torch.int64, "dense_table").value if dense_table is not None else None
        self.s.ndense = int(ndense) if dense_table is not None else 0

    def part(self, seg_table, item_seg, nseg, nitems):
        return QSGDBatch(seg_table, item_seg, nseg, nitems, self.s.n_bit, self.s.bits, bool(self.s.wide), self.keep[2], self.s.bucket_hint)

    def compress(self, wire, random_mode, seed, ef_scale=None):
        rc = self.L.gq_qsgd_compress_batched(self.ref, _dev_ptr(wire, torch.uint8, "wire"), ctypes.c_int(random_mode),
                                             ctypes.c_uint64(seed & (2 ** 64 - 1)),
                                             ctypes.c_float(_NAN if ef_scale is None else ef_scale), _stream())
        _check(rc, "gq_qsgd_compress_batched")

    def decode(self, gathered, R, out, plain=False, tail=None):
        assert gathered.dtype == torch.uint8 and gathered.dim() == 2 and gathered.shape[0] == R and gathered.is_contiguous()
        if tail is not None:
            rc = self.L.gq_qsgd_decode_sum_batched_tail(self.ref, _dev_ptr(gathered, torch.uint8, "gathered"),
                                                        ctypes.c_int64(gathered.shape[1]), ctypes.c_int(R),
                                                        _dev_ptr(out, torch.float32, "out"), ctypes.c_int(1 if plain else 0), tail.ref, _stream())
            _check(rc, "gq_qsgd_decode_sum_batched_tail")
            return
        rc = self.L.gq_qsgd_decode_sum_batched(self.ref, _dev_ptr(gathered, torch.uint8, "gathered"),
                                               ctypes.c_int64(gathered.shape[1]), ctypes.c_int(R),
                                               _dev_ptr(out, torch.float32, "out"), ctypes.c_int(1 if plain else 0), _stream())
        _check(rc, "gq_qsgd_decode_sum_batched")


class _PVQStage1(ctypes.Structure):
    _fields_ = [("codes1", ctypes.c_void_p), ("code1_bytes", ctypes.c_int32), ("reserved", ctypes.c_int32),
                ("norm1", ctypes.c_void_p), ("codebook1", ctypes.c_void_p)]


def pvq_encode(grad, c_dagger, codes, u, workspace, random_mode, r, seed, stage1=None):
    K, d = c_dagger.shape
    M = grad.numel() // d
    assert grad.numel() == M * d and codes.numel() == M and u.numel() == M
    rp = _dev_ptr(r, torch.float32, "r") if r is not None else ctypes.c_void_p(0)
    st1 = ctypes.c_void_p(0)
    if stage1 is not None:
        codes1, norm1, codebook1 = stage1
        assert codes1.numel() == M and norm1.numel() == M and codebook1.shape[1] == d
        st1 = ctypes.byref(_PVQStage1(_dev_ptr(codes1, None, "codes1").value, _CODE_BYTES[codes1.dtype], 0,
                                      _dev_ptr(norm1, torch.float32, "norm1").value,
                                      _dev_ptr(codebook1, torch.float32, "codebook1").value))
    rc = lib().gq_pvq_encode(_dev_ptr(grad, torch.float32, "grad"), _dev_ptr(c_dagger, torch.float32, "c_dagger"),
                             ctypes.c_int64(M), ctypes.c_int(d), ctypes.c_int(K), ctypes.c_int(random_mode), rp,
                             ctypes.c_uint64(seed & (2 ** 64 - 1)), _dev_ptr(codes, None, "codes"),
                             ctypes.c_int(_CODE_BYTES[codes.dtype]), _dev_ptr(u, torch.float32, "u"),
                             _dev_ptr(workspace, torch.float32, "workspace"), st1, _stream())
    _check(rc, "gq_pvq_encode")


def pvq_encode_residual(grad, codes1, norm1, codebook1, c_dagger, codes, u, workspace, random_mode, r, seed):
    pvq_encode(grad, c_dagger, codes, u, workspace, random_mode, r, seed, stage1=(codes1, norm1, codebook1))


class LaunchPlan(object):

    def __init__(self, graph):
        self.graph = graph
        self.L = lib()
        self.plan, n = ctypes.c_void_p(0), ctypes.c_int(0)
        rc = self.L.gq_launch_plan_create(ctypes.c_void_p(int(graph.raw_cuda_graph())), ctypes.byref(self.plan), ctypes.byref(n))
        if rc != 0:
            raise GQNativeError("gq_launch_plan_create failed (%d): %s" % (rc, self.L.gq_last_error().decode()))
        self.nodes = n.value
        self._run = self.L.gq_launch_plan_run

    def replay(self):
        rc = self._run(self.plan, _stream())
        if rc != 0:
            raise GQNativeError("gq_launch_plan_run failed (%d): %s" % (rc, self.L.gq_last_error().decode()))

    def __del__(self):
        try:
            if self.plan:
                self.L.gq_launch_plan_destroy(self.plan)
                self.plan = ctypes.c_void_p(0)
        except Exception:
            pass


def qsgd_code_bits(n_bit, random_mode):
    return int(lib().gq_qsgd_code_bits(ctypes.c_int(n_bit), ctypes.c_int(random_mode)))


QSGD_WIDE_CHUNK = 1024


def axpy_inplace(grad, err, scale):
    assert grad.numel() == err.numel()
    _check(lib().gq_axpy_inplace(_dev_ptr(grad, torch.float32, "grad"), _dev_ptr(err, torch.float32, "err"),
                                 ctypes.c_float(scale), ctypes.c_int64(grad.numel()), _stream()), "gq_axpy_inplace")


def sub(grad, decoded, err):
    assert grad.numel() == decoded.numel() == err.numel()
    _check(lib().gq_sub(_dev_ptr(grad, torch.float32, "grad"), _dev_ptr(decoded, torch.float32, "decoded"),
                        _dev_ptr(err, torch.float32, "err"), ctypes.c_int64(grad.numel()), _stream()), "gq_sub")


def qsgd_compress(grad, d, n_bit, random_mode, r, seed, norm, signs, levels):
    Mb = grad.numel() // d
    assert grad.numel() == Mb * d and norm.numel() == Mb and signs.numel() == Mb * d and levels.numel() == Mb * d
    rp = _dev_ptr(r, torch.float32, "r") if r is not None else ctypes.c_void_p(0)
    sg = signs.view(torch.uint8) if signs.dtype == torch.bool else signs
    rc = lib().gq_qsgd_compress(_dev_ptr(grad, torch.float32, "grad"), ctypes.c_int64(Mb), ctypes.c_int(d),
                                ctypes.c_int(n_bit), ctypes.c_int(random_mode), rp,
                                ctypes.c_uint64(seed & (2 ** 64 - 1)), _dev_ptr(norm, torch.float32, "norm"),
                                _dev_ptr(sg, torch.uint8, "signs"), _dev_ptr(levels, None, "levels"),
                                ctypes.c_int(_LEVEL_BYTES[levels.dtype]), _stream())
    _check(rc, "gq_qsgd_compress")


def qsgd_decode_sum(norm, signs, levels, d, n_bit, out, R=1):
    Mb = norm.numel() // R
    assert signs.numel() == R * Mb * d and levels.numel() == R * Mb * d and out.numel() == Mb * d
    sg = signs.view(torch.uint8) if signs.dtype == torch.bool else signs
    rc = lib().gq_qsgd_decode_sum(_dev_ptr(norm, torch.float32, "norm"), _dev_ptr(sg, torch.uint8, "signs"),
                                  _dev_ptr(levels, None, "levels"), ctypes.c_int(_LEVEL_BYTES[levels.dtype]),
                                  ctypes.c_int(R), ctypes.c_int64(Mb), ctypes.c_int(d), ctypes.c_int(n_bit),
                                  _dev_ptr(out, torch.float32, "out"), _stream())
    _check(rc, "gq_qsgd_decode_sum")


TOPK_LIB_PATH = os.environ.get("GQ_TOPK_LIB_PATH") or os.path.join(_PKG_DIR, "libgq_topk.so")
TOPK_ABI_VERSION = 1
TOPK_EXPORTS = ["gq_topk_abi_version", "gq_topk_last_error", "gq_topk_compress_batched", "gq_topk_decode_sum_batched"]
TOPK_CHUNK = 4096
TOPK_HIST_BINS = 2048

_topk_lib = None


def topk_lib():
    global _topk_lib
    if _topk_lib is None:
        if not os.path.exists(TOPK_LIB_PATH):
            raise GQNativeError("libgq_topk.so not found at %s -- build it with `python gradient-quantization_amd/build.py` "
                                "(there is no CPU fallback)" % TOPK_LIB_PATH)
        L = ctypes.CDLL(TOPK_LIB_PATH)
        L.gq_topk_last_error.restype = ctypes.c_char_p
        L.gq_topk_abi_version.restype = ctypes.c_int
        for name in TOPK_EXPORTS:
            getattr(L, name)
        if L.gq_topk_abi_version() != TOPK_ABI_VERSION:
            raise GQNativeError("%s has ABI version %d, this binding is written for %d: rebuild it"
                                % (TOPK_LIB_PATH, L.gq_topk_abi_version(), TOPK_ABI_VERSION))
        _topk_lib = L
    return _topk_lib


def _check_topk(rc, what):
    CALLS[0] += 1
    if rc != 0:
        raise GQNativeError("%s failed (%d): %s" % (what, rc, topk_lib().gq_topk_last_error().decode()))


class _TopKBatchStruct(ctypes.Structure):
    _fields_ = [("struct_bytes", ctypes.c_uint32), ("nseg", ctypes.c_int32), ("nitems", ctypes.c_int64),
                ("seg_table", ctypes.c_void_p), ("item_seg", ctypes.c_void_p), ("hist", ctypes.c_void_p), ("state", ctypes.c_void_p),
                ("counts", ctypes.c_void_p), ("dense_table", ctypes.c_void_p), ("ndense", ctypes.c_int32), ("reserved", ctypes.c_int32)]


class TopKBatch(object):

    def __init__(self, seg_table, item_seg, nseg, nitems, hist=None, state=None, counts=None):
        self.L = topk_lib()
        self.keep = (seg_table, item_seg, hist, state, counts)
        ptr = lambda t, name: _dev_ptr(t, torch.int32, name).value if t is not None else None
        self.s = _TopKBatchStruct(ctypes.sizeof(_TopKBatchStruct), int(nseg), int(nitems), _dev_ptr(seg_table, torch.int64, "seg_table").value,
                                  _dev_ptr(item_seg, torch.int32, "item_seg").value, ptr(hist, "hist"), ptr(state, "state"),
                                  ptr(counts, "counts"), None, 0, 0)
        self.ref = ctypes.byref(self.s)

    def set_table(self, seg_table):
        self.keep_table = seg_table
        self.s.seg_table = _dev_ptr(seg_table, torch.int64, "seg_table").value

    def set_dense(self, dense_table, ndense):
        self.keep_dense = dense_table
        self.s.dense_table = _dev_ptr(dense_table, torch.int64, "dense_table").value if dense_table is not None else None
        self.s.ndense = int(ndense) if dense_table is not None else 0

    def part(self, seg_table, item_seg, nseg, nitems):
        return TopKBatch(seg_table, item_seg, nseg, nitems)

    def compress(self, wire, out=None, ef_scale=None):
        rc = self.L.gq_topk_compress_batched(self.ref, _dev_ptr(wire, torch.uint8, "wire"),
                                             ctypes.c_float(_NAN if ef_scale is None else ef_scale),
                                             _dev_ptr(out, torch.float32, "out") if out is not None else ctypes.c_void_p(0), _stream())
        _check_topk(rc, "gq_topk_compress_batched")

    def decode(self, gathered, R, out, plain=False):
        assert gathered.dtype == torch.uint8 and gathered.dim() == 2 and gathered.shape[0] == R and gathered.stride(1) == 1
        stride = int(gathered.stride(0)) if R > 1 else int(gathered.shape[1])
        rc = self.L.gq_topk_decode_sum_batched(self.ref, _dev_ptr(gathered[0], torch.uint8, "gathered"), ctypes.c_int64(stride),
                                               ctypes.c_int(R), _dev_ptr(out, torch.float32, "out"), ctypes.c_int(1 if plain else 0),
                                               _stream())
        _check_topk(rc, "gq_topk_decode_sum_batched")


SIGN_LIB_PATH = os.environ.get("GQ_SIGN_LIB_PATH") or os.path.join(_PKG_DIR, "libgq_sign.so")
SIGN_ABI_VERSION = 1
SIGN_EXPORTS = ["gq_sign_abi_version", "gq_sign_last_error", "gq_sign_compress_batched", "gq_sign_decode_sum_batched"]
SIGN_ITEM_BYTES = 4096

_sign_lib = None


def sign_lib():
    global _sign_lib
    if _sign_lib is None:
        if not os.path.exists(SIGN_LIB_PATH):
            raise GQNativeError("libgq_sign.so not found at %s -- build it with `python gradient-quantization_amd/build.py` "
                                "(there is no CPU fallback)" % SIGN_LIB_PATH)
        L = ctypes.CDLL(SIGN_LIB_PATH)
        L.gq_sign_last_error.restype = ctypes.c_char_p
        L.gq_sign_abi_version.restype = ctypes.c_int
        for name in SIGN_EXPORTS:
            getattr(L, name)
        if L.gq_sign_abi_version() != SIGN_ABI_VERSION:
            raise GQNativeError("%s has ABI version %d, this binding is written for %d: rebuild it"
                                % (SIGN_LIB_PATH, L.gq_sign_abi_version(), SIGN_ABI_VERSION))
        _sign_lib = L
    return _sign_lib


def _check_sign(rc, what):
    CALLS[0] += 1
    if rc != 0:
        raise GQNativeError("%s failed (%d): %s" % (what, rc, sign_lib().gq_sign_last_error().decode()))


class _SignBatchStruct(ctypes.Structure):
    _fields_ = [("struct_bytes", ctypes.c_uint32), ("nseg", ctypes.c_int32), ("nitems", ctypes.c_int64),
                ("seg_table", ctypes.c_void_p), ("item_seg", ctypes.c_void_p), ("dense_table", ctypes.c_void_p),
                ("ndense", ctypes.c_int32), ("reserved", ctypes.c_int32)]


class SignBatch(object):

    def __init__(self, seg_table, item_seg, nseg, nitems):
        self.L = sign_lib()
        self.keep = (seg_table, item_seg)
        self.s = _SignBatchStruct(ctypes.sizeof(_SignBatchStruct), int(nseg), int(nitems), _dev_ptr(seg_table, torch.int64, "seg_table").value,
                                  _dev_ptr(item_seg, torch.int32, "item_seg").value, None, 0, 0)
        self.ref = ctypes.byref(self.s)

    def set_table(self, seg_table):
        self.keep_table = seg_table
        self.s.seg_table = _dev_ptr(seg_table, torch.int64, "seg_table").value

    def set_dense(self, dense_table, ndense):
        self.keep_dense = dense_table
        self.s.dense_table = _dev_ptr(dense_table, torch.int64, "dense_table").value if dense_table is not None else None
        self.s.ndense = int(ndense) if dense_table is not None else 0

    def part(self, seg_table, item_seg, nseg, nitems):
        return SignBatch(seg_table, item_seg, nseg, nitems)

    def compress(self, wire, out=None, ef_scale=None):
        rc = self.L.gq_sign_compress_batched(self.ref, _dev_ptr(wire, torch.uint8, "wire"),
                                             ctypes.c_float(_NAN if ef_scale is None else ef_scale),
                                             _dev_ptr(out, torch.float32, "out") if out is not None else ctypes.c_void_p(0), _stream())
        _check_sign(rc, "gq_sign_compress_batched")

    def decode(self, gathered, R, out, plain=False):
        assert gathered.dtype == torch.uint8 and gathered.dim() == 2 and gathered.shape[0] == R and gathered.stride(1) == 1
        stride = int(gathered.stride(0)) if R > 1 else int(gathered.shape[1])
        rc = self.L.gq_sign_decode_sum_batched(self.ref, _dev_ptr(gathered[0], torch.uint8, "gathered"), ctypes.c_int64(stride),
                                               ctypes.c_int(R), _dev_ptr(out, torch.float32, "out"), ctypes.c_int(1 if plain else 0),
                                               _stream())
        _check_sign(rc, "gq_sign_decode_sum_batched")


PVQ_LIB_PATH = os.environ.get("GQ_PVQ_LIB_PATH") or os.path.join(_PKG_DIR, "libgq_pvq.so")
PVQ_ABI_VERSION = 1
PVQ_EXPORTS = ["gq_pvq_abi_version", "gq_pvq_last_error", "gq_pvq_batched_serves", "gq_pvq_encode_batched"]

_pvq_lib = None


def pvq_lib():
    global _pvq_lib
    if _pvq_lib is None:
        if not os.path.exists(PVQ_LIB_PATH):
            raise GQNativeError("libgq_pvq.so not found at %s -- build it with `python gradient-quantization_amd/build.py` "
                                "(there is no CPU fallback)" % PVQ_LIB_PATH)
        L = ctypes.CDLL(PVQ_LIB_PATH)
        L.gq_pvq_last_error.restype = ctypes.c_char_p
        L.gq_pvq_abi_version.restype = ctypes.c_int
        for name in PVQ_EXPORTS:
            getattr(L, name)
        if L.gq_pvq_abi_version() != PVQ_ABI_VERSION:
            raise GQNativeError("%s has ABI version %d, this binding is written for %d: rebuild it"
                                % (PVQ_LIB_PATH, L.gq_pvq_abi_version(), PVQ_ABI_VERSION))
        _pvq_lib = L
    return _pvq_lib


def _check_pvq(rc, what):
    CALLS[0] += 1
    if rc != 0:
        raise GQNativeError("%s failed (%d): %s" % (what, rc, pvq_lib().gq_pvq_last_error().decode()))


def pvq_batched_serves(d, K, code_dtype):
    return d in (8, 16, 32) and 32 <= K <= 256 and K % 32 == 0 and code_dtype == torch.uint8


class _PVQBatchStruct(ctypes.Structure):
    _fields_ = [("struct_bytes", ctypes.c_uint32), ("reserved", ctypes.c_int32), ("hsq", ctypes.c_void_p), ("c_dagger", ctypes.c_void_p)]


class PVQBatch(HSQBatch):

    def __init__(self, seg_table, tile_seg, nseg, ntiles, codebook, c_dagger, code_dtype, level_dtype, n_bit, u_flat=None,
                 seg_minmax=None, workspace=None):
        HSQBatch.__init__(self, seg_table, tile_seg, nseg, ntiles, codebook, code_dtype, level_dtype, n_bit, u_flat, seg_minmax, workspace)
        self.PL = pvq_lib()
        assert c_dagger.shape == codebook.shape
        self.c_dagger = c_dagger
        self.ps = _PVQBatchStruct(ctypes.sizeof(_PVQBatchStruct), 0, ctypes.addressof(self.s), _dev_ptr(c_dagger, torch.float32, "c_dagger").value)
        self.pref = ctypes.byref(self.ps)
        if not self.PL.gq_pvq_batched_serves(ctypes.c_int(self.s.d), ctypes.c_int(self.s.K), ctypes.c_int(self.s.code_bytes)):
            self.path = 0

    def encode(self, wire, ef_scale, random_mode, seed, r_flat=None):
        rp = _dev_ptr(r_flat, torch.float32, "r_flat") if r_flat is not None else ctypes.c_void_p(0)
        rc = self.PL.gq_pvq_encode_batched(self.pref, self._wire(wire), ctypes.c_int(random_mode), ctypes.c_uint64(seed & (2 ** 64 - 1)), rp,
                                           ctypes.c_float(_NAN if ef_scale is None else ef_scale), _stream())
        _check_pvq(rc, "gq_pvq_encode_batched")


RQ_LIB_PATH = os.environ.get("GQ_RQ_LIB_PATH") or os.path.join(_PKG_DIR, "libgq_rq.so")
RQ_ABI_VERSION = 1
RQ_EXPORTS = ["gq_rq_abi_version", "gq_rq_last_error", "gq_rq_batched_serves", "gq_rq_encode2_batched", "gq_rq_decode_sum_batched"]
RQ_MEAN, RQ_PLAIN, RQ_ERROR = 0, 1, 2

_rq_lib = None


def rq_lib():
    global _rq_lib
    if _rq_lib is None:
        if not os.path.exists(RQ_LIB_PATH):
            raise GQNativeError("libgq_rq.so not found at %s -- build it with `python gradient-quantization_amd/build.py` "
                                "(there is no CPU fallback)" % RQ_LIB_PATH)
        L = ctypes.CDLL(RQ_LIB_PATH)
        L.gq_rq_last_error.restype = ctypes.c_char_p
        L.gq_rq_abi_version.restype = ctypes.c_int
        for name in RQ_EXPORTS:
            getattr(L, name)
        if L.gq_rq_abi_version() != RQ_ABI_VERSION:
            raise GQNativeError("%s has ABI version %d, this binding is written for %d: rebuild it"
                                % (RQ_LIB_PATH, L.gq_rq_abi_version(), RQ_ABI_VERSION))
        _rq_lib = L
    return _rq_lib


def _check_rq(rc, what):
    CALLS[0] += 1
    if rc != 0:
        raise GQNativeError("%s failed (%d): %s" % (what, rc, rq_lib().gq_rq_last_error().decode()))


def rq_batched_serves(d, K, code_dtype):
    return pvq_batched_serves(d, K, code_dtype)


class _RQBatchStruct(ctypes.Structure):
    _fields_ = [("struct_bytes", ctypes.c_uint32), ("reserved", ctypes.c_int32), ("stage1", ctypes.c_void_p), ("stage2", ctypes.c_void_p),
                ("c_dagger", ctypes.c_void_p), ("level2_words", ctypes.c_void_p)]


class RQBatch(object):

    def __init__(self, seg_table, seg_table2, tile_seg, nseg, ntiles, codebook1, codebook2, c_dagger, code_dtype, level_dtype, n_bit,
                 u_flat1=None, seg_minmax1=None, workspace1=None, u_flat2=None, seg_minmax2=None, level2_words=None):
        self.RL = rq_lib()
        self.b1 = HSQBatch(seg_table, tile_seg, nseg, ntiles, codebook1, code_dtype, level_dtype, n_bit, u_flat1, seg_minmax1, workspace1)
        self.b2 = HSQBatch(seg_table2, tile_seg, nseg, ntiles, codebook2, code_dtype, level_dtype, n_bit, u_flat2, seg_minmax2, None)
        assert c_dagger.shape == codebook2.shape == codebook1.shape
        self.keep = (c_dagger, level2_words, code_dtype, level_dtype, n_bit)
        self.device = self.b1.device
        self.s = _RQBatchStruct(ctypes.sizeof(_RQBatchStruct), 0, ctypes.addressof(self.b1.s), ctypes.addressof(self.b2.s),
                                _dev_ptr(c_dagger, torch.float32, "c_dagger").value,
                                _dev_ptr(level2_words, torch.int64, "level2_words").value if level2_words is not None else None)
        self.ref = ctypes.byref(self.s)
        self.level2_seed = level2_words.data_ptr() if level2_words is not None else None
        serves = self.RL.gq_rq_batched_serves(ctypes.c_int(self.b1.s.d), ctypes.c_int(self.b1.s.K), ctypes.c_int(self.b1.s.code_bytes))
        self.path = self.b1.path if (serves and self.b2.path) else 0

    def set_table(self, seg_table):
        self.b1.set_table(seg_table)

    def set_dense(self, dense_table, ndense):
        self.b1.set_dense(dense_table, ndense)

    def part(self, seg_table, seg_table2, tile_seg, nseg, ntiles):
        c_dagger, _, code_dtype, level_dtype, n_bit = self.keep
        return RQBatch(seg_table, seg_table2, tile_seg, nseg, ntiles, self.b1.keep[2], self.b2.keep[2], c_dagger, code_dtype, level_dtype, n_bit)

    def encode2(self, wire, random_mode, seed, r_flat=None):
        rp = _dev_ptr(r_flat, torch.float32, "r_flat") if r_flat is not None else ctypes.c_void_p(0)
        rc = self.RL.gq_rq_encode2_batched(self.ref, self.b1._wire(wire), ctypes.c_int(random_mode), ctypes.c_uint64(seed & (2 ** 64 - 1)), rp,
                                           _stream())
        _check_rq(rc, "gq_rq_encode2_batched")

    def decode(self, gathered, R, out, plain=False, mode=None):
        assert gathered.dtype == torch.uint8 and gathered.dim() == 2 and gathered.shape[0] == R and gathered.stride(1) == 1
        stride = int(gathered.stride(0)) if R > 1 else int(gathered.shape[1])
        if mode is None:
            mode = RQ_PLAIN if (plain and R == 1) else RQ_MEAN
        op = _dev_ptr(out, torch.float32, "out") if out is not None else ctypes.c_void_p(0)
        rc = self.RL.gq_rq_decode_sum_batched(self.ref, self.b1._wire(gathered), ctypes.c_int64(stride), ctypes.c_int(R), op,
                                              ctypes.c_int(mode), _stream())
        _check_rq(rc, "gq_rq_decode_sum_batched")
```

### gradient-quantization_amd/gq_amd/quantizers.py

```python
import math
import operator
import os
import warnings

import torch

from . import exchange, native
from .compressors import IdenticalCompressor, TopKSparsificationCompressor, _next_seed, shared_seeds

_HOST = None
if os.environ.get("GQ_HOST_EXT", "1") != "0":
    try:
        from . import _gq_host as _HOST
    except ImportError as _e:
        warnings.warn("gq_amd: the host helper _gq_host.so is not built (%s); run gradient-quantization_amd/build.py" % (_e,))


from .codecs import (
    BatchedHSQ, BatchedPVQ, BatchedQSGD, BatchedResidual, BatchedSign, BatchedTopK, DenseCodec, GenericCodec, HSQCodec, QSGDCodec,
    ResidualCodec, SignCodec, TopKCodec,
    _BatchedBase, _DATA_PTR, _DTYPE_OF, _F32_ONLY, _GET_DEVICE, _IS_CONTIGUOUS, _esize, _kernel_copy, _up, aggregate_fma, default_codec_factory,
    quantizer_codec_factory,
    wire_levels_mode)


def _ef_scale(args, epoch):
    if args.scale == 'exp':
        return 2 / (math.exp(-epoch) + 1) - 1
    return float(args.scale)


def _dist_world(process_group):
    import torch.distributed as dist
    if dist.is_available() and dist.is_initialized():
        return dist.get_world_size(process_group), dist.get_rank(process_group)
    return 1, 0


class _capturing(object):

    def __init__(self, direct):
        self.graph = _new_graph(direct)
        self._ctx = torch.cuda.graph(self.graph, capture_error_mode="thread_local")
        self._gc = False

    def __enter__(self):
        import gc
        self._gc = gc.isenabled()
        gc.disable()
        try:
            self._ctx.__enter__()
        except BaseException:
            if self._gc:
                gc.enable()
            raise
        return self.graph

    def __exit__(self, *exc):
        import gc
        try:
            return self._ctx.__exit__(*exc)
        finally:
            if self._gc:
                gc.enable()


def _new_graph(direct):
    if direct:
        try:
            return torch.cuda.CUDAGraph(keep_graph=True)
        except TypeError:
            pass
    return torch.cuda.CUDAGraph()


def _replayable(graph, direct):
    if direct and hasattr(graph, "raw_cuda_graph"):
        try:
            return native.LaunchPlan(graph)
        except Exception:
            pass
    try:
        graph.instantiate()
    except Exception:
        pass
    return graph


class _GraphCache(dict):

    def __init__(self, max_captured=48, max_counting=64):
        dict.__init__(self)
        self.max_captured, self.max_counting = max_captured, max_counting
        self.address_free = set()

    def sight(self, key, address_free=False):
        ent = self.get(key)
        if ent is None:
            if not address_free and self.captured()[0] >= self.max_captured:
                return None
            counting = [k for k, e in self.items() if e[1] is None]
            if len(counting) >= self.max_counting:
                del self[counting[0]]
                self.address_free.discard(counting[0])
            ent = self[key] = [0, None, None]
            if address_free:
                self.address_free.add(key)
        ent[0] += 1
        return ent

    def captured(self):
        keys = [k for k, e in self.items() if e[1] is not None]
        free = sum(1 for k in keys if k in self.address_free)
        return len(keys) - free, free


class PSQuantizer(object):
    def __init__(self, Compressor, parameters, args, process_group=None, codec_factory=None):
        self.parameters = list(parameters)
        self.num_layers = len(self.parameters)
        self.args = args
        self.error_feedback = args.ef
        self.two_phase = args.two_phase
        self.process_group = process_group
        factory = codec_factory or quantizer_codec_factory
        self.aggregate_fma = aggregate_fma(args)
        self.wire_levels = wire_levels_mode(args, _dist_world(process_group)[0])
        if self.wire_levels == "packed6":
            base_factory = factory
            factory = lambda comp, n, shape: base_factory(comp, n, shape, packed6=True)
        self.compressors = []
        self.codecs = []
        for param in self.parameters:
            param_size = param.flatten().shape[0]
            comp = Compressor(param_size, param.shape, args) if param_size > 1000 else IdenticalCompressor()
            self.compressors.append(comp)
            self.codecs.append(factory(comp, param_size, param.shape))
            if self.aggregate_fma and isinstance(self.codecs[-1], HSQCodec):
                self.codecs[-1].fma = True
            if self.error_feedback:
                param.error = [torch.zeros_like(param) for _ in range(args.num_users)]
            if self.error_feedback and self.two_phase:
                param.server_error = torch.zeros_like(param)
        self.offsets = [0] * self.num_layers
        off = 0
        self.dense_idx = [i for i, c in enumerate(self.codecs) if type(c) is DenseCodec]
        for i, c in enumerate(self.codecs):
            if i not in self.dense_idx:
                self.offsets[i] = off
                off = _up(off + c.nbytes)
        self.dense_off = off
        for i in self.dense_idx:
            self.offsets[i] = off
            off += self.codecs[i].nbytes
        self.dense_bytes = off - self.dense_off
        self._dense_mean, self._dense_views, self._dense_turn = [None, None], [None, None], 0
        self._dense_in = {}
        self.user_bytes = _up(off)
        self._groups = []
        g = getattr(args, "gq_graph", None)
        self.use_graphs = bool(int(os.environ.get("GQ_GRAPH", "1"))) if g is None else bool(g)
        self._fuse_steps = type(self) is PSQuantizer and os.environ.get("GQ_FUSE_STEP", "1") != "0"
        self._direct = os.environ.get("GQ_DIRECT_REPLAY", "1") != "0"
        self._step_tail = os.environ.get("GQ_STEP_TAIL", "1") != "0"
        self._fuse_levels = os.environ.get("GQ_FUSE_LEVELS", "1") != "0"
        BatchedQSGD.place_lone_buckets(self.codecs)
        for cls in (BatchedHSQ, BatchedPVQ, BatchedResidual, BatchedQSGD, BatchedTopK, BatchedSign):
            keyed = {}
            for i, c in enumerate(self.codecs):
                if cls.eligible(c):
                    keyed.setdefault(cls.group_key(c), []).append(i)
            for key in sorted(keyed):
                idx = keyed[key]
                if len(idx) >= 2 and not getattr(args, "gq_no_batch", False):
                    self._groups.append([cls, idx, None])
        self.batch_idx = [i for g in self._groups for i in g[1]]
        self._pick_dense = operator.itemgetter(*self.dense_idx) if len(self.dense_idx) >= 2 else None
        self._pick_group = {}
        self._rng_state = None
        self._ticket = None
        self._rec_graphs = _GraphCache(self.MAX_ADDRESS_GRAPHS)
        self._apply_graphs = _GraphCache()
        self._step_graphs = _GraphCache()
        self._fused = None
        self._phase2_base = None
        self._fast_ok = None
        self._apply_key_memo, self._dense_gen = {}, 0
        self._fast_misses = 0
        self.record_paths = {"graph": 0, "graph_any_address": 0, "whole_step": 0, "whole_step_any_address": 0, "eager": 0}
        self._phase2_calls = 0
        self._draw_off, n = {}, 0
        for i, c in enumerate(self.codecs):
            if isinstance(c, (HSQCodec, ResidualCodec)) and c.uses_reference_draws():
                self._draw_off[i] = n
                n += c.draw_count()
        self._draw_total = n
        self._draw_host = None
        self._assembled = {}
        self._plan = None
        self.capacity = max(1, int(args.num_users))
        self.recorded = 0
        self._wire = None
        self._ex = None
        self.exchange_mode = exchange.configured_mode()
        bounds = [self.offsets[i] for i in range(self.num_layers) if i not in self.dense_idx]
        later = [o for o in bounds if o >= self.dense_off // 2]
        self.cut = min(later) if later else 0
        nchunks = max(2, int(os.environ.get("GQ_PIPELINE_CHUNKS", "4")))
        self.cuts = []
        for k in range(1, nchunks):
            inner = [o for o in bounds if o > 0]
            if inner:
                c = min(inner, key=lambda o: (abs(o - self.dense_off * k // nchunks), o))
                if c not in self.cuts:
                    self.cuts.append(c)
        self.cuts.sort()

    def _ensure_wire(self, device, slots):
        world, rank = _dist_world(self.process_group)
        if (self._wire is None or self._wire.device != device or self._wire.shape[0] < slots
                or (world > 1) != (self._ex is not None)):
            cap = max(self.capacity, slots)
            old = self._wire
            if world > 1:
                self._ex = exchange.WireExchange(world, rank, cap, self.user_bytes, device, self.process_group)
                new = self._ex.local
            else:
                self._ex = None
                new = torch.zeros((cap, self.user_bytes), dtype=torch.uint8, device=device)
            if old is not None and old.device == device:
                new[:min(cap, old.shape[0])].copy_(old[:cap])
            self._wire = new
            self.capacity = cap
        return self._wire

    def wire_bytes_per_user(self):
        return self.user_bytes

    RNG_SLOTS = 17
    TWO_PHASE_RNG_SLOT = RNG_SLOTS - 1

    def _rng_pairs_for(self, device, group_index):
        if self._rng_state is None or self._rng_state.device != device:
            world, rank = _dist_world(self.process_group)
            n = max(1, len(self._groups)) * self.RNG_SLOTS
            host = torch.zeros((n, 2), dtype=torch.int64)
            base = _next_seed()
            shared = self._second_phase_base(device) if self.two_phase else base
            for i in range(n):
                if i % self.RNG_SLOTS == self.TWO_PHASE_RNG_SLOT:
                    host[i, 0] = ((shared ^ ((i + 1) * 0x9E3779B97F4A7C15)) & (2 ** 63 - 1))
                else:
                    host[i, 0] = ((base ^ ((rank * 1000003 + i + 1) * 0x9E3779B97F4A7C15)) & (2 ** 63 - 1))
            self._rng_state = host.to(device)
        return self._rng_state[group_index * self.RNG_SLOTS:(group_index + 1) * self.RNG_SLOTS]

    def _second_phase_base(self, device):
        if self._phase2_base is None:
            base = _next_seed()
            world, rank = _dist_world(self.process_group)
            if world > 1:
                import torch.distributed as dist
                on_gpu = device.type == "cuda" and dist.get_backend(self.process_group) != "gloo"
                t = torch.tensor([base], dtype=torch.int64, device=device if on_gpu else "cpu")
                dist.broadcast(t, src=0 if self.process_group is None else dist.get_global_rank(self.process_group, 0),
                               group=self.process_group)
                base = int(t.item())
            self._phase2_base, self._phase2_calls = base, 0
        return self._phase2_base

    def _second_phase_seed(self):
        self._phase2_calls += 1
        return (self._phase2_base * 0x9E3779B97F4A7C15 + self._phase2_calls * 0xD1B54A32D192ED03) & (2 ** 63 - 1)

    def _draws(self, device):
        if not self._draw_total:
            return None
        if device.type != "cuda":
            return torch.rand(self._draw_total), self._draw_off
        if self._draw_host is None:
            self._draw_host = [torch.empty(self._draw_total).pin_memory() for _ in range(2)]
            self._draw_turn = 0
            self._draw_events = [None, None]
        k = self._draw_turn
        self._draw_turn ^= 1
        if self._draw_events[k] is not None:
            self._draw_events[k].synchronize()
        torch.rand(self._draw_total, out=self._draw_host[k])
        dev_r = self._draw_host[k].to(device, non_blocking=True)
        ev = torch.cuda.Event()
        ev.record()
        self._draw_events[k] = ev
        return dev_r, self._draw_off

    def _replay_known_step(self, user):
        if not self._fast_ok and not self._fast_check():
            return False
        if self._fast_misses >= 8:
            self._fast_misses += 1
            if self._fast_misses & 31:
                return False
        if (self.recorded != 0 or not self.use_graphs or not self._fuse_steps or torch.cuda.is_current_stream_capturing()
                or _dist_world(self.process_group)[0] != 1):
            return False
        key, ok, index = _HOST.scan_key(self.parameters)
        wire = self._wire
        if not ok or index != wire.device.index or index != torch._C._cuda_getDevice():
            self._fast_misses += 1
            return False
        graph_key = (0, user, wire.data_ptr(), key)
        ent = self._rec_graphs.get(graph_key)
        fent = self._step_graphs.get((graph_key, self._apply_key_for(1, wire.data_ptr()))) if (ent is not None and ent[1] is not None) else None
        if fent is None or fent[1] is None:
            self._fast_misses += 1
            return False
        self._fast_misses = 0
        self._replayed(fent, "whole_step", True, True, True)
        return True

    def _fast_check(self):
        if (_HOST is None or not hasattr(_HOST, "scan_key") or not self.use_graphs or not self._fuse_steps or self.error_feedback
                or self.two_phase or self._draw_total or self.capacity != 1 or not self._groups):
            self._fast_ok = False
            return False
        if self._wire is None or not self._whole_step_ok(_dist_world(self.process_group)[0], 0) or not self._graphable():
            return False
        self._fast_ok = True
        return True

    def _graphable(self):
        return all(g[2] is not None and g[2].ready and g[2].graphable() for g in self._groups)

    def _whole_step_ok(self, world, slot):
        return (self._fuse_steps and world == 1 and slot == 0 and self.capacity == 1 and not self.two_phase
                and self._plan is not None and not self._plan[2])

    def _replayed(self, ent, path, clean, table_replaced, decoded):
        if clean:
            for g in self._groups:
                g[2].ensure_clean()
        ent[1].replay()
        turn = decoded and not self.two_phase
        for g in self._groups:
            g[2].after_replay(turn, table_replaced)
        if decoded and len(self.dense_idx) >= 2:
            self._dense_turn ^= 1
        if path is not None:
            if decoded:
                self._fused = ent[2]
            self.recorded += 1
            self.record_paths[path] += 1

    def record(self, user, epoch):
        if self._fast_ok is not False and self._replay_known_step(user):
            return
        scale = _ef_scale(self.args, epoch)
        scan = _HOST.scan_grads(self.parameters) if _HOST is not None else None
        all_grads = scan[0] if scan is not None else [p.grad for p in self.parameters]
        dev = all_grads[0].device
        slot = self.recorded
        wire = self._ensure_wire(dev, slot + 1)[slot]
        world, rank = _dist_world(self.process_group)
        salt = ((rank * 1000003 + user) * 0x9E3779B1) & (2 ** 62 - 1)
        draws = self._draws(dev)
        graph_key = None
        if (self.use_graphs and dev.type == "cuda" and not self._draw_total and slot < self.TWO_PHASE_RNG_SLOT and self._graphable()
                and not torch.cuda.is_current_stream_capturing()):
            graph_key = (slot, user, self._wire.data_ptr(), scan[1] if scan is not None else tuple(map(_DATA_PTR, all_grads)))
            generic_key = ("any", slot, user, self._wire.data_ptr())
            if self.error_feedback:
                graph_key += (scale, tuple(p.error[user].data_ptr() for p in self.parameters))
                generic_key += (scale,)
            plain_f32 = scan[2] if scan is not None else (all(map(_IS_CONTIGUOUS, all_grads)) and set(map(_DTYPE_OF, all_grads)) == _F32_ONLY)
            ent = self._rec_graphs.get(graph_key) if plain_f32 else None
            tied = ent is not None and ent[1] is not None
            if plain_f32 and not tied:
                ent = self._rec_graphs.get(generic_key)
                if ent is None or ent[1] is None or not self._upload_headers(all_grads, slot, user):
                    ent = None
                else:
                    own = self._rec_graphs.sight(graph_key)
                    if own is not None and own[0] >= 2 and own[1] is None:
                        self._capture_record(own, all_grads, wire, slot, user, salt, scale, dev)
            if ent is not None:
                key = graph_key if tied else generic_key
                step_key = (key, self._apply_key_for(1, self._wire.data_ptr())) if self._whole_step_ok(world, slot) else None
                fent = self._step_graphs.get(step_key)
                if fent is not None and fent[1] is not None:
                    self._replayed(fent, "whole_step" if tied else "whole_step_any_address", tied, tied, True)
                    return
                self._replayed(ent, "graph" if tied else "graph_any_address", tied, tied, False)
                if step_key is not None:
                    fent = self._step_graphs.sight(step_key, address_free=not tied)
                    if fent is not None and fent[0] >= 2 and fent[1] is None:
                        self._capture_step(fent, ent[2], all_grads, wire, slot, user, salt, scale, dev)
                return
        self.record_paths["eager"] += 1
        skip = self._record_launches(all_grads, wire, slot, user, salt, scale, draws, dev)
        if len(skip) == self.num_layers:
            self.recorded += 1
            if graph_key is not None:
                gent = self._rec_graphs.sight(generic_key, address_free=True)
                if gent[1] is None and gent[0] >= 2 and self._generic_ok():
                    self._capture_record(gent, all_grads, wire, slot, user, salt, scale, dev, generic=True)
                ent = self._rec_graphs.sight(graph_key)
                if ent is not None and ent[0] >= 2 and ent[1] is None:
                    self._capture_record(ent, all_grads, wire, slot, user, salt, scale, dev)
            return
        for i, param in enumerate(self.parameters):
            if i in skip:
                continue
            codec, off = self.codecs[i], self.offsets[i]
            grad = param.grad.data
            if self.error_feedback:
                if grad.device.type == "cuda" and grad.is_contiguous() and grad.dtype == torch.float32:
                    native.axpy_inplace(grad, param.error[user].contiguous(), scale)
                else:
                    grad.add_(scale * param.error[user])
                if hasattr(codec, "encode_decode_into"):
                    decoded = torch.empty(grad.numel(), dtype=torch.float32, device=grad.device)
                    codec.encode_decode_into(grad, wire, off, salt, decoded, **self._slice(draws, i))
                    decoded = decoded.view(param.shape)
                elif hasattr(codec, "decode_wire"):
                    codec.encode_into(grad, wire, off, salt, **self._slice(draws, i))
                    decoded = torch.empty(grad.numel(), dtype=torch.float32, device=grad.device)
                    codec.decode_wire(wire, off, decoded)
                    decoded = decoded.view(param.shape)
                else:
                    raise TypeError("%s has neither encode_decode_into nor decode_wire: under error feedback its payload must be both "
                                    "written to the wire and decoded (ps_quantizer.py:37)" % type(codec).__name__)
                if grad.device.type == "cuda" and grad.is_contiguous():
                    err = torch.empty_like(grad)
                    native.sub(grad, decoded.contiguous(), err)
                    param.error[user].data = err
                else:
                    param.error[user].data = grad - decoded
            else:
                codec.encode_into(grad, wire, off, salt, **self._slice(draws, i))
        self.recorded += 1

    MAX_ADDRESS_GRAPHS = 8

    def graph_counts(self):
        rec, rec_any = self._rec_graphs.captured()
        step, step_any = self._step_graphs.captured()
        return {"record": rec, "record_any_address": rec_any, "apply": sum(self._apply_graphs.captured()),
                "whole_step": step, "whole_step_any_address": step_any}

    def _generic_ok(self):
        return bool(self._groups) and (len(self.dense_idx) < 2 or bool(self._groups[0][2] is not None and self._groups[0][2].ndense))

    def _upload_headers(self, all_grads, slot, user):
        for grp in self._groups:
            cls, idxs, obj = grp
            grads = list(self._pick_group[id(grp)](all_grads))
            errs = [self.parameters[i].error[user] for i in idxs] if self.error_feedback else None
            dense = list(self._pick_dense(all_grads)) if obj.ndense else None
            if not obj.upload(grads, slot, errs, dense):
                return False
        return True

    def _make_group(self, grp, dev):
        cls, idxs = grp[0], grp[1]
        dense = ([(self.offsets[i], self.codecs[i].numel) for i in self.dense_idx]
                 if (grp is self._groups[0] and len(self.dense_idx) >= 2) else None)
        obj = grp[2] = cls(self.codecs, self.offsets, idxs, dev, self.capacity, self.user_bytes, dense=dense)
        obj.fma = bool(self.aggregate_fma and cls is BatchedHSQ)
        if dev.type == "cuda":
            self._ticket_for(dev)
        if getattr(obj, "counter", False) and len(self._groups) * self.RNG_SLOTS <= 256:
            obj.rng_pairs = self._rng_pairs_for(dev, self._groups.index(grp))
        return obj

    def _ticket_for(self, dev):
        if self._ticket is None or self._ticket.device != dev:
            if torch.cuda.is_current_stream_capturing():
                raise RuntimeError("the ticket words are made by the first eager record (_make_group), not under stream capture")
            self._ticket = torch.zeros(native.TICKET_WORDS, dtype=torch.int32, device=dev)
        return self._ticket

    def _record_launches(self, all_grads, wire, slot, user, salt, scale, draws, dev, headers=None, defer_resets=None, fuse_levels=False,
                         table_current=False):
        skip = set()
        for gi, grp in enumerate(self._groups if dev.type == "cuda" else []):
            cls, idxs, obj = grp
            if obj is None:
                obj = self._make_group(grp, dev)
            pick = self._pick_group.get(id(grp))
            if pick is None:
                pick = self._pick_group[id(grp)] = operator.itemgetter(*idxs)
            grads = list(pick(all_grads))
            errs = [self.parameters[i].error[user] for i in idxs] if self.error_feedback else None
            hdr = headers[gi] if headers is not None else None
            dense = list(self._pick_dense(all_grads)) if obj.ndense else None
            kw = {"skip_levels": True} if fuse_levels else {}
            if obj.encode(grads, wire, slot, salt, errs, scale, draws=draws, graph_header=hdr, dense=dense, defer_reset=defer_resets,
                          table_current=table_current, **kw):
                skip.update(idxs)
                if dense is not None:
                    skip.update(self.dense_idx)
        if len(self.dense_idx) >= 2 and self.dense_idx[0] not in skip:
            key = (self._wire.data_ptr(), slot)
            views = self._dense_in.get(key)
            if views is None:
                region = wire[self.dense_off:self.dense_off + self.dense_bytes].view(torch.float32)
                views, o = [], 0
                for i in self.dense_idx:
                    n = self.codecs[i].numel
                    views.append(region[o:o + n].view(self.codecs[i].shape))
                    o += n
                self._dense_in = {k: v for k, v in self._dense_in.items() if k[0] == key[0]}
                self._dense_in[key] = views
            with torch.no_grad():
                torch._foreach_copy_(views, list(self._pick_dense(all_grads)))
            skip.update(self.dense_idx)
        return skip

    def _capture_record(self, ent, all_grads, wire, slot, user, salt, scale, dev, generic=False):
        try:
            headers = None if generic else [g[2]._host[g[2]._last_slot].to(dev) for g in self._groups]
            with _capturing(self._direct) as graph:
                self._record_launches(all_grads, wire, slot, user, salt, scale, None, dev, headers=headers, table_current=generic)
            ent[1], ent[2] = _replayable(graph, self._direct), headers
        except Exception as e:
            self.use_graphs = False
            warnings.warn("gq_graph: capturing a record failed (%s); continuing with eager launches" % (e,))

    def _capture_step(self, fent, headers, all_grads, wire, slot, user, salt, scale, dev):
        after = ([g[2]._out_turn for g in self._groups], self._dense_turn)
        try:
            with _capturing(self._direct) as graph:
                resets = []
                fuse = self._can_fuse_levels()
                self._record_launches(all_grads, wire, slot, user, salt, scale, None, dev, headers=headers, defer_resets=resets,
                                      fuse_levels=fuse, table_current=headers is None)
                decoded = self._decode_all(self._wire[:1], False, (), resets=resets, fused_levels=fuse)
            fent[1], fent[2] = _replayable(graph, self._direct), decoded
        except Exception as e:
            self._fuse_steps = False
            for g in self._groups:
                g[2].graph_tables_abort()
            warnings.warn("gq_graph: capturing a whole step failed (%s); record and apply keep their own graphs" % (e,))
        finally:
            self._set_turns(after)

    def _capture_apply(self, ent, graph_key, gathered, decoded):
        after = ([g[2]._out_turn for g in self._groups], self._dense_turn)
        try:
            self._set_turns((graph_key[2], graph_key[3]))
            hdrs2 = [g[2]._host[g[2]._last_slot].to(gathered.device) for g in self._groups] if self.two_phase else None
            calls = self._phase2_calls
            with _capturing(self._direct) as graph:
                again = self._decode_all(gathered, self.two_phase, (), phase2_headers=hdrs2)
            if self._phase2_calls != calls:
                raise RuntimeError("a captured second phase must not take per-call seeds")
            if len(again) == len(decoded) and all(a is b for a, b in zip(again, decoded)):
                ent[1], ent[2] = _replayable(graph, self._direct), decoded
                ent.append(hdrs2)
        except Exception as e:
            self.use_graphs = False
            for g in self._groups:
                g[2].graph_tables_abort()
            warnings.warn("gq_graph: capturing an apply failed (%s); continuing with eager launches" % (e,))
        finally:
            self._set_turns(after)

    def _set_turns(self, turns):
        for g, t in zip(self._groups, turns[0]):
            g[2].set_out_turn(t)
        self._dense_turn = turns[1]

    def _can_fuse_levels(self):
        if not self._fuse_levels or not self._groups:
            return False
        if self.error_feedback:
            return False
        return (all(isinstance(g[2], BatchedHSQ) and g[2].fusable_levels() for g in self._groups)
                and (not self.dense_idx or (len(self.dense_idx) >= 2 and self._groups[0][2].ndense)) and self._step_tail)

    def _apply_key_for(self, R, ptr):
        turns = tuple([g[2]._out_turn for g in self._groups])
        gen = (turns, self._dense_turn, self._dense_gen, tuple([g[2]._out_gen for g in self._groups]))
        hit = self._apply_key_memo.get(gen)
        if hit is None:
            if len(self._apply_key_memo) > 16:
                self._apply_key_memo.clear()
            hit = self._apply_key_memo[gen] = (tuple(0 if o is None else o.data_ptr() for g in self._groups for o in g[2]._outs),
                                               tuple(0 if m is None else m.data_ptr() for m in self._dense_mean))
        return (R, ptr, turns, self._dense_turn, hit[0], hit[1])

    def _slice(self, draws, i):
        if draws is None or i not in self._draw_off:
            return {}
        o = self._draw_off[i]
        return {"r": draws[0][o:o + self.codecs[i].draw_count()]}

    def _decode_all(self, gathered, two_phase, pending=(), plain=False, resets=None, fused_levels=False, phase2_headers=None):
        R = gathered.shape[0]
        done = {}
        pending = list(pending)
        chunked = len(pending) >= 2
        on_gpu = gathered.device.type == "cuda"
        key = (on_gpu,) + tuple(g[2] is not None and g[2].ready for g in self._groups)
        if self._plan is None or self._plan[0] != key:
            groups = [g for g in (self._groups if on_gpu else []) if g[2] is not None and g[2].ready]
            batched = set(i for g in groups for i in g[1])
            dense = set(self.dense_idx) if len(self.dense_idx) >= 2 else set()
            single = [i for i in range(self.num_layers) if i not in batched and i not in dense]
            self._plan = (key, groups, single, {})
        _, groups, single, seg_ranges = self._plan
        single = list(single)
        group_views = {}

        step_rng = self._rng_state is not None and on_gpu
        dense_job = None
        if len(self.dense_idx) >= 2:
            rows = gathered[:, self.dense_off:self.dense_off + self.dense_bytes].view(torch.float32)
            k = self._dense_turn
            self._dense_turn ^= 1
            if self._dense_mean[k] is None or self._dense_mean[k].device != rows.device:
                mean = torch.empty(rows.shape[1], dtype=torch.float32, device=rows.device)
                views, o = [], 0
                for i in self.dense_idx:
                    n = self.codecs[i].numel
                    views.append(mean[o:o + n].view(self.codecs[i].shape))
                    o += n
                self._dense_mean[k], self._dense_views[k] = mean, views
                self._dense_gen += 1
            dense_job = (rows, k)
        tail, tail_group = None, -1
        if on_gpu and not chunked and not two_phase and self._step_tail:
            takers = [gi for gi, g in enumerate(groups) if g[2].takes_tail]
            mean_in_tail = dense_job is not None and not (plain and R == 1)
            if takers and (mean_in_tail or step_rng or resets):
                tail_group = takers[-1]
                tail = native.StepTail(rows=dense_job[0] if mean_in_tail else None,
                                       out=self._dense_mean[dense_job[1]] if mean_in_tail else None,
                                       rng_state=self._rng_state if step_rng else None, reset=resets.pop(0) if resets else None,
                                       ticket=self._ticket_for(gathered.device))
                step_rng = False
                if mean_in_tail:
                    dense_job = (None, dense_job[1])

        def decode_range(lo, hi, first):
            for gi, (cls, idxs, obj) in enumerate(groups):
                part = None
                if lo is not None:
                    part = seg_ranges.get((gi, lo, hi))
                    if part is None:
                        part = seg_ranges[(gi, lo, hi)] = (sum(1 for i in idxs if self.offsets[i] < lo),
                                                          sum(1 for i in idxs if self.offsets[i] < hi))
                    part = part + (first,)
                t = tail if gi == tail_group else None
                if fused_levels and lo is None and obj._pending_levels is not None:
                    group_views[gi] = obj.levels_decode(plain, t)
                else:
                    group_views[gi] = obj.decode_mean(gathered, R, part, plain=plain, tail=t)
            for i in single:
                if lo is None or lo <= self.offsets[i] < hi:
                    done[i] = self.codecs[i].decode_mean(gathered, self.offsets[i], R, plain=plain)

        if not chunked:
            if pending:
                pending.pop(0).wait()
            decode_range(None, None, True)
        else:
            for k, pnd in enumerate(pending):
                pnd.wait()
                decode_range(pnd.lo, self.user_bytes if pnd.hi is None else pnd.hi, k == 0)
        draws2 = self._draws(gathered.device) if two_phase else None
        if two_phase:
            self._second_phase_base(gathered.device)
        if phase2_headers is not None and resets is None:
            resets = []
        sources = []
        for gi, (cls, idxs, obj) in enumerate(groups):
            gs = group_views[gi]
            if two_phase:
                serr = [self.parameters[i].server_error for i in idxs] if self.error_feedback else None
                hdr = phase2_headers[gi] if phase2_headers is not None else None
                with shared_seeds(self._second_phase_seed):
                    dec = obj.roundtrip(list(gs), self.capacity, 0, serr, 1.0, draws=draws2, rng_slot=self.TWO_PHASE_RNG_SLOT,
                                        graph_header=hdr, defer_reset=resets if hdr is not None else None)
                if dec is None:
                    for i, g in zip(idxs, gs):
                        done[i] = g
                        single.append(i)
                    continue
                gs = dec
            sources.append((idxs, gs))
        if dense_job is not None:
            rows, k = dense_job
            if rows is None:
                pass
            elif plain and R == 1:
                self._dense_mean[k].copy_(rows[0])
            elif rows.device.type == "cuda":
                native.mean_rows(rows, self._dense_mean[k], rng_state=self._rng_state if step_rng else None,
                                 reset=resets.pop(0) if resets else None)
                step_rng = False
            else:
                torch.mean(rows, dim=0, out=self._dense_mean[k])
            sources.append((self.dense_idx, self._dense_views[k]))
        if step_rng:
            native.rng_step(self._rng_state, reset=resets.pop(0) if resets else None)
        for dst, src in (resets or ()):
            _kernel_copy(dst, src)
        if not single and not done:
            key = tuple(id(v) for _, v in sources)
            hit = self._assembled.get(key)
            if hit is not None and all(a is b for a, (_, b) in zip(hit[0], sources)):
                return hit[1]
            for idxs, vs in sources:
                for i, v in zip(idxs, vs):
                    done[i] = v
            out = [done[i] for i in range(self.num_layers)]
            if len(self._assembled) > 8:
                self._assembled.clear()
            self._assembled[key] = ([v for _, v in sources], out)
            return out
        for idxs, vs in sources:
            for i, v in zip(idxs, vs):
                done[i] = v
        if two_phase:
            for i in single:
                param, codec, g = self.parameters[i], self.codecs[i], done[i]
                kw = self._slice(draws2, i)
                with shared_seeds(self._second_phase_seed):
                    if self.error_feedback:
                        g = g + param.server_error
                        decoded = codec.roundtrip(g, 0, **kw)
                        param.server_error = g - decoded
                        g = decoded
                    else:
                        g = codec.roundtrip(g, 0, **kw)
                done[i] = g
        return [done[i] for i in range(self.num_layers)]

    def apply(self, refresh_grads=False):
        if self.recorded == 0:
            return
        world, rank = _dist_world(self.process_group)
        if world > 1:
            ex = self._ex
            if self.exchange_mode == "auto":
                def step(mode):
                    buf, pend = ex.start(mode, self.recorded, self.cut)
                    self._decode_all(buf, False, pend)
                self.exchange_mode = ex.autotune(
                    step, preflight=lambda mode: ex.start(mode, self.recorded, self.cut, dry_run=True))
            gathered, pending = ex.start(self.exchange_mode, self.recorded, self.cut, cuts=self.cuts)
        else:
            gathered, pending = self._wire[:self.recorded], ()
        decoded = None
        graph_key = None
        fused, self._fused = self._fused, None
        if fused is not None and self.recorded == 1 and world == 1:
            decoded = fused
        elif (self.use_graphs and len(pending) <= 1 and gathered.device.type == "cuda"
                and all(g[2] is not None and g[2].ready for g in self._groups) and not torch.cuda.is_current_stream_capturing()
                and (not self.two_phase or (not self._draw_total and all(g[2].graphable() for g in self._groups)))):
            for pnd in pending:
                pnd.wait()
            pending = ()
            graph_key = self._apply_key_for(gathered.shape[0], gathered.data_ptr())
            if self.two_phase and self.error_feedback:
                graph_key += (tuple(p.server_error.data_ptr() for p in self.parameters),)
            ent = self._apply_graphs.get(graph_key)
            if ent is not None and ent[1] is not None:
                self._replayed(ent, None, self.two_phase, True, True)
                decoded = ent[2]
        if decoded is None:
            decoded = self._decode_all(gathered, self.two_phase, pending)
            if graph_key is not None and self._plan is not None and not self._plan[2]:
                ent = self._apply_graphs.sight(graph_key)
                if ent is not None and ent[0] >= 2 and ent[1] is None:
                    self._capture_apply(ent, graph_key, gathered, decoded)
        if _HOST is not None and hasattr(_HOST, "set_grad_data") and type(decoded) is list and len(decoded) == len(self.parameters):
            _HOST.set_grad_data(self.parameters, decoded)
        else:
            for p, g in zip(self.parameters, decoded):
                p.grad.data = g
        self.recorded = 0

    aggregate = apply


def _ring_codec_factory(compressor, numel, shape, packed6=False):
    if isinstance(compressor, TopKSparsificationCompressor):
        return GenericCodec(compressor, numel, shape)
    return quantizer_codec_factory(compressor, numel, shape, packed6)


class RingQuantizer(PSQuantizer):

    def __init__(self, Compressor, parameters, args, process_group=None, codec_factory=None):
        two_phase = args.two_phase
        args.two_phase = False
        try:
            super().__init__(Compressor, parameters, args, process_group, codec_factory or _ring_codec_factory)
        finally:
            args.two_phase = two_phase
        self.two_phase = False
        self.running = None
        self._inbox = None

    def record(self, user, epoch):
        world, rank = _dist_world(self.process_group)
        dev = self.parameters[0].grad.device
        if self.running is None and rank > 0:
            import torch.distributed as dist
            if self._inbox is None or self._inbox.device != dev:
                self._inbox = torch.empty((1, self.user_bytes), dtype=torch.uint8, device=dev)
            dist.recv(self._inbox.view(-1), src=self._peer(rank - 1), group=self.process_group)
            self._ready_for_wire(dev)
            self.running = self._decode_all(self._inbox, False, plain=True)
        if self.running is not None:
            torch._foreach_add_([p.grad.data for p in self.parameters], list(self.running))
        self.recorded = 0
        super().record(user, epoch)
        self.running = self._decode_all(self._wire[:1], False, plain=True)

    def _peer(self, group_rank):
        import torch.distributed as dist
        return group_rank if self.process_group is None else dist.get_global_rank(self.process_group, group_rank)

    def _ready_for_wire(self, dev):
        for grp in (self._groups if dev.type == "cuda" else []):
            if grp[2] is None:
                self._make_group(grp, dev)
            if not grp[2].ready:
                grp[2].upload_layout()

    def apply(self):
        world, rank = _dist_world(self.process_group)
        if world > 1:
            import torch.distributed as dist
            if self.recorded == 0 and self.running is None:
                return
            dev = self._wire.device
            if rank < world - 1:
                dist.send(self._wire[0], dst=self._peer(rank + 1), group=self.process_group)
            final = self._wire[:1] if rank == world - 1 else self._inbox_for(dev)
            dist.broadcast(final.view(-1), src=self._peer(world - 1), group=self.process_group)
            if rank != world - 1:
                self.running = self._decode_all(final, False, plain=True)
        if self.running is not None:
            if _HOST is not None and type(self.running) is list and len(self.running) == len(self.parameters):
                _HOST.set_grad_data(self.parameters, self.running)
            else:
                for param, g in zip(self.parameters, self.running):
                    param.grad.data = g
        self.running = None
        self.recorded = 0

    def _inbox_for(self, dev):
        if self._inbox is None or self._inbox.device != dev:
            self._inbox = torch.empty((1, self.user_bytes), dtype=torch.uint8, device=dev)
        return self._inbox

    aggregate = apply


def Quantizer(Compressor, parameters, args, **kw):
    if args.mode == 'ps':
        return PSQuantizer(Compressor, parameters, args, **kw)
    elif args.mode == 'ring':
        return RingQuantizer(Compressor, parameters, args, **kw)
    assert False, "mode {} not recognized".format(args.mode)


__all__ = ["Quantizer", "PSQuantizer", "RingQuantizer"]
```

Measured before the change: 425.2 billion elements/s.

## Precompute codebook LDS image once and load it in the prefilter encode kernel

Adds a prepared codebook "image": a device buffer holding the codebook already in LDS layout, the fp16 hi/lo MFMA fragments and the folded norm bounds. It is built once per codebook version and reused by the prefilter encode kernels. Each block then copies the image straight into LDS instead of re-deriving the layout, fp16 splits and the wave reductions at kernel start. This trims per-block prologue work. In exchange it adds a separate library, version tracking of the codebook, and a rule that the image must be prepared before any graph capture.

Measured after the change: 425.8 billion elements/s (median of 6 runs). Within noise of the previous version (+0.1%).

```diff
diff --git a/gradient-quantization_amd/build.py b/gradient-quantization_amd/build.py
--- a/gradient-quantization_amd/build.py
+++ b/gradient-quantization_amd/build.py
@@ -16,6 +16,9 @@
 PVQ_SOURCES = ["pvq_batched.hip"]
 RQ_LIB = os.path.join(HERE, "libgq_rq.so")
 RQ_SOURCES = ["rq_batched.hip"]
+IMAGE_LIB = os.path.join(HERE, "libgq_hsq_image.so")
+IMAGE_SOURCES = ["hsq_image.hip"]
+IMAGE_MAP = os.path.join(CSRC, "hsq_image.map")
 SOURCES = ["gq_common.hip", "gq_api.hip", "hsq_encode.hip", "hsq_encode_pf.hip", "hsq_encode_pfd.hip", "hsq_levels.hip", "hsq_batched.hip", "hsq_decode.hip", "qsgd.hip", "qsgd_batched.hip", "qsgd_wide.hip", "pvq.hip"]
 FLAGS = ["--offload-arch=gfx950", "-O3", "-ffp-contract=off", "-fPIC", "-shared", "-std=c++17",
          "-Xclang", "-target-feature", "-Xclang", "-packed-fp32-ops",
@@ -34,11 +37,13 @@
 
 def needs_build():
     if (not os.path.exists(LIB) or not os.path.exists(os.path.join(HERE, "libgq_hsq_clock.so")) or not os.path.exists(HOST_EXT)
-            or not os.path.exists(TOPK_LIB) or not os.path.exists(SIGN_LIB) or not os.path.exists(PVQ_LIB) or not os.path.exists(RQ_LIB)):
+            or not os.path.exists(TOPK_LIB) or not os.path.exists(SIGN_LIB) or not os.path.exists(PVQ_LIB) or not os.path.exists(RQ_LIB)
+            or not os.path.exists(IMAGE_LIB) or not os.path.exists(image_twin(os.path.join(HERE, "libgq_hsq_clock.so")))):
         return True
     t = min(os.path.getmtime(LIB), os.path.getmtime(HOST_EXT), os.path.getmtime(TOPK_LIB), os.path.getmtime(SIGN_LIB), os.path.getmtime(PVQ_LIB),
-            os.path.getmtime(RQ_LIB))
-    deps = ([os.path.join(CSRC, f) for f in os.listdir(CSRC)] + [os.path.join(ROOT, "include", h) for h in ("gq_hsq.h", "gq_topk.h", "gq_sign.h", "gq_pvq.h", "gq_rq.h")]
+            os.path.getmtime(RQ_LIB), os.path.getmtime(IMAGE_LIB))
+    deps = ([os.path.join(CSRC, f) for f in os.listdir(CSRC)]
+            + [os.path.join(ROOT, "include", h) for h in ("gq_hsq.h", "gq_topk.h", "gq_sign.h", "gq_pvq.h", "gq_rq.h", "gq_hsq_image.h")]
             + [__file__])
     return any(os.path.getmtime(d) > t for d in deps)
 
@@ -65,8 +70,9 @@
         if verbose:
             print(" ".join(cmd))
         procs.append((cmd, subprocess.Popen(cmd), obj))
-    topk_objs, sign_objs, pvq_objs, rq_objs = [], [], [], []
-    for srcs, own in ((TOPK_SOURCES, topk_objs), (SIGN_SOURCES, sign_objs), (PVQ_SOURCES, pvq_objs), (RQ_SOURCES, rq_objs)):
+    topk_objs, sign_objs, pvq_objs, rq_objs, image_objs = [], [], [], [], []
+    for srcs, own in ((TOPK_SOURCES, topk_objs), (SIGN_SOURCES, sign_objs), (PVQ_SOURCES, pvq_objs), (RQ_SOURCES, rq_objs),
+                      (IMAGE_SOURCES, image_objs)):
         for src in srcs:
             obj = os.path.join(objdir, src.replace(".hip", ".o"))
             cmd = [hipcc()] + compile_flags + EXTRA.get(src, []) + ["-c", os.path.join(CSRC, src), "-o", obj]
@@ -78,7 +84,7 @@
     for cmd, p, obj in procs:
         if p.wait() != 0:
             raise subprocess.CalledProcessError(p.returncode, cmd)
-        if obj not in topk_objs and obj not in sign_objs and obj not in pvq_objs and obj not in rq_objs:
+        if obj not in topk_objs and obj not in sign_objs and obj not in pvq_objs and obj not in rq_objs and obj not in image_objs:
             objs.append(obj)
     link = [hipcc(), "--offload-arch=gfx950", "-shared", "-fPIC", "-o", LIB] + objs
     if verbose:
@@ -94,6 +100,7 @@
         subprocess.check_call([hipcc(), "--offload-arch=gfx950", "-shared", "-fPIC", "-o", SIGN_LIB] + sign_objs)
         subprocess.check_call([hipcc(), "--offload-arch=gfx950", "-shared", "-fPIC", "-o", PVQ_LIB] + pvq_objs)
         subprocess.check_call([hipcc(), "--offload-arch=gfx950", "-shared", "-fPIC", "-o", RQ_LIB] + rq_objs)
+        link_image_lib(IMAGE_LIB, objs + image_objs)
         build_clock_lib(objs, verbose)
     finally:
         if host is not None and host[1].wait() != 0:
@@ -123,6 +130,15 @@
 CLOCK_LIB = os.path.join(HERE, "libgq_hsq_clock.so")
 
 
+def image_twin(lib_path):
+    d, base = os.path.split(lib_path)
+    return os.path.join(d, base.replace("libgq_hsq", "libgq_hsq_image", 1) if base.startswith("libgq_hsq") else base + ".image.so")
+
+
+def link_image_lib(out, objs):
+    subprocess.check_call([hipcc(), "--offload-arch=gfx950", "-shared", "-fPIC", "-Wl,--version-script=" + IMAGE_MAP, "-o", out] + objs)
+
+
 def build_clock_lib(objs=None, verbose=False, source=None, out=None):
     objdir = os.path.join(HERE, "build")
     if objs is None:
@@ -137,6 +153,7 @@
     subprocess.check_call(cmd, stderr=None if verbose else subprocess.DEVNULL)
     others = [o for o in objs if os.path.basename(o) != "hsq_encode_pf.o"]
     subprocess.check_call([hipcc(), "--offload-arch=gfx950", "-shared", "-fPIC", "-o", out or CLOCK_LIB, obj] + others)
+    link_image_lib(image_twin(out or CLOCK_LIB), [obj] + others + [os.path.join(objdir, f.replace(".hip", ".o")) for f in IMAGE_SOURCES])
     return out or CLOCK_LIB
 
 
diff --git a/gradient-quantization_amd/csrc/gq_internal.h b/gradient-quantization_amd/csrc/gq_internal.h
--- a/gradient-quantization_amd/csrc/gq_internal.h
+++ b/gradient-quantization_amd/csrc/gq_internal.h
@@ -4,6 +4,13 @@
 GQ_INTERNAL int gqi_hsq_encode_batched_pf(const int64_t *seg_table, const int32_t *tile_seg, int nseg, int64_t ntiles,
                                           const float *codebook, int d, int K, int ef, float ef_scale, uint8_t *wire, float *u_flat,
                                           uint32_t *seg_minmax, float *workspace, int profile_slot, void *stream);
+GQ_INTERNAL int gqi_hsq_encode_batched_pf_image(const int64_t *seg_table, const int32_t *tile_seg, int nseg, int64_t ntiles,
+                                                const float *codebook, int d, int K, int ef, float ef_scale, uint8_t *wire, float *u_flat,
+                                                uint32_t *seg_minmax, float *workspace, int profile_slot, const void *image, void *stream);
+GQ_INTERNAL int gqi_hsq_encode_pf_image(const float *grad, const float *codebook, int64_t M, int d, int K, void *codes, int code_bytes,
+                                        float *u, float *workspace, int profile_slot, const void *image, void *image_dump, void *stream);
+GQ_INTERNAL size_t gqi_hsq_image_bytes(int d, int K);
+GQ_INTERNAL int gqi_hsq_image_prepare(const float *codebook, int d, int K, void *image, void *stream);
 GQ_INTERNAL int gqi_hsq_encode_batched_paged(const int64_t *seg_table, const int32_t *tile_seg, int nseg, int64_t ntiles,
                                              const float *codebook, int d, int K, int ef, float ef_scale, uint8_t *wire,
                                              float *u_flat, uint32_t *seg_minmax, float *workspace, void *stream);
diff --git a/gradient-quantization_amd/csrc/hsq_encode_pf.hip b/gradient-quantization_amd/csrc/hsq_encode_pf.hip
--- a/gradient-quantization_amd/csrc/hsq_encode_pf.hip
+++ b/gradient-quantization_amd/csrc/hsq_encode_pf.hip
@@ -2,7 +2,7 @@
 
 #include <type_traits>
 
-#include "hsq_pf_common.hpp"
+#include "hsq_pf_image.hpp"
 
 #ifdef GQ_PF_STAMPS
 #define GQ_STAMP(ID)                                                                                  \
@@ -24,17 +24,12 @@
 
 namespace gq {
 
-constexpr int PF_WAVES = 8;
-constexpr int PF_THREADS = PF_WAVES * 64;
 #ifndef GQ_PF_TAIL
 #define GQ_PF_TAIL 4
 #endif
 constexpr int PF_TAIL = GQ_PF_TAIL;
 #ifndef GQ_PF_FLUSH_AHEAD
 #define GQ_PF_FLUSH_AHEAD 0
-#endif
-#ifndef GQ_PF_PAIR
-#define GQ_PF_PAIR -1
 #endif
 #ifndef GQ_PF_FLUSH_MIN
 #define GQ_PF_FLUSH_MIN 3
@@ -46,20 +41,6 @@
 constexpr int PF_FLUSH_MIN = GQ_PF_FLUSH_MIN;
 constexpr int PF_SCAN1_MAX = GQ_PF_SCAN1_MAX;
 constexpr int PF_LDS_SEGS = 384;
-template <int D>
-struct PfShape {
-    static_assert(D == 8 || D == 16 || D == 32, "the prefilter kernel is built for D = 8, 16 and 32");
-    static constexpr int KS = D > 16 ? D / 16 : 1;
-    static constexpr bool HALF = D < 16;
-    static constexpr int QS = 4 * D + 4;
-    static constexpr int QCAP = D > 16 ? 32 : 64;
-    static constexpr bool A_REGS = D <= 16;
-    static constexpr int NF = 4 * KS;
-    static constexpr bool PAIR = GQ_PF_PAIR < 0 ? D > 16 : GQ_PF_PAIR != 0;
-    static constexpr float ERR_REL = (D > 16 ? 1.05f : 1.03f) * 4.8828125e-04f;
-    static constexpr float ERR2_REL = (D > 16 ? 2.3f : 1.2f) * 7.62939453125e-06f;
-    static constexpr float ERR2_SUB = D > 16 ? 3.5e-7f : 2.4e-7f;
-};
 constexpr float ERR_ABS = 4.76837158203125e-07f;
 constexpr unsigned N2_LO_BITS = 0x39800000u;
 constexpr unsigned N2_HI_BITS = 0x4B800000u;
@@ -82,6 +63,8 @@
     float ef_scale;
     int tiles_q, tiles_r;
     int tiles_skew, skew_blocks;
+    const u32x4 *img;
+    u32x4 *img_dump;
 };
 
 #ifndef GQ_PF_SKEW_PERMILLE
@@ -287,18 +270,23 @@
     float n2p[2] = {0.0f, 0.0f};
     Tile ti = {};
 
-    float cbv[256 * DR / PF_THREADS];
-#pragma unroll
-    for (int n = 0; n < 256 * DR / PF_THREADS; ++n) cbv[n] = (int)threadIdx.x + n * PF_THREADS < K * DR ? cb[threadIdx.x + n * PF_THREADS] : 0.0f;
-    f32x4 aq[2 * KS];
-#pragma unroll
-    for (int i = 0; i < 2 * KS; ++i) aq[i] = f32x4{0.0f, 0.0f, 0.0f, 0.0f};
-    if (loads_here && wave * 32 + j < K) {
-#pragma unroll
-        for (int s = 0; s < KS; ++s) {
-            if (frag_ok(s, 0)) aq[2 * s] = *reinterpret_cast<const f32x4 *>(cb + (wave * 32 + j) * DR + 16 * s + (HALF ? 0 : 8 * h));
-            if (frag_ok(s, 1)) aq[2 * s + 1] = *reinterpret_cast<const f32x4 *>(cb + (wave * 32 + j) * DR + 16 * s + (HALF ? 0 : 8 * h) + 4);
-        }
+    typedef PfImage<D> IM;
+    const bool has_img = a.img != nullptr;
+    PfCodebookWords<D, DR> cw;
+    u32x4 iv[IM::LOADS], fold = {0u, 0u, 0u, 0u};
+    if (has_img) {
+        typedef const u32x4 __attribute__((address_space(1))) *gimg_ptr;
+        const gimg_ptr img = (gimg_ptr)a.img;
+#pragma unroll
+        for (int n = 0; n < IM::CB_LOADS; ++n) {
+            const int i = threadIdx.x + n * PF_THREADS;
+            iv[n] = ((n + 1) * PF_THREADS <= IM::CB_UNITS || i < IM::CB_UNITS) ? img[i] : u32x4{0u, 0u, 0u, 0u};
+        }
+#pragma unroll
+        for (int n = 0; n < 2 * KS; ++n) iv[IM::CB_LOADS + n] = img[IM::CB_UNITS + threadIdx.x + n * PF_THREADS];
+        fold = img[IM::FOLD_UNIT];
+    } else {
+        pf_codebook_request<D, DR>(cw, cb, K, wave, lane);
     }
     const int seg_first_v = (BATCHED && lo_tile < ntiles) ? a.tile_seg[lo_tile] : 0;
     if (t < tile_end) {
@@ -315,47 +303,23 @@
         s_mm[2 * threadIdx.x] = 0xFFFFFFFFu;
         s_mm[2 * threadIdx.x + 1] = 0u;
     }
-#pragma unroll
-    for (int n = 0; n < 256 * DR / PF_THREADS; ++n) {
-        const int i = threadIdx.x + n * PF_THREADS, k = i / DR, jj = i % DR;
-        s_cb[(k >> 2) * QS + 4 * jj + (k & 3)] = cbv[n];
-    }
-    if constexpr (DR != D) {
-#pragma unroll
-        for (int n = 0; n < 256 * (D - DR) / PF_THREADS; ++n) {
-            const int i = threadIdx.x + n * PF_THREADS, k = i / (D - DR), jj = DR + i % (D - DR);
-            s_cb[(k >> 2) * QS + 4 * jj + (k & 3)] = 0.0f;
-        }
-    }
     if (BATCHED && SEGLDS) {
         const int n = (a.nseg < PF_LDS_SEGS ? a.nseg : PF_LDS_SEGS) * 8;
         for (int i = threadIdx.x; i < n; i += PF_THREADS) s_seg[i] = a.seg_table[i];
     }
-    {
-        float l2 = 0.0f, d2 = 0.0f;
-#pragma unroll
-        for (int s = 0; s < KS; ++s) {
-            half8 fh, fl;
-#pragma unroll
-            for (int e = 0; e < 8; ++e) {
-                const float x = e < 4 ? aq[2 * s][e] : aq[2 * s + 1][e - 4];
-                fh[e] = (_Float16)x;
-                const float rr = x - (float)fh[e];
-                fl[e] = (_Float16)rr;
-                l2 = __fmaf_rn(x, x, l2);
-                d2 = __fmaf_rn(rr, rr, d2);
-            }
-            s_frag[(wave * KS + s) * 64 + lane] = __builtin_bit_cast(u32x4, fh);
-            s_fragl[(wave * KS + s) * 64 + lane] = __builtin_bit_cast(u32x4, fl);
-        }
-        l2 += __shfl_xor(l2, 32, 64);
-        d2 += __shfl_xor(d2, 32, 64);
-        l2 = wave_max_nan(l2);
-        d2 = wave_max_nan(d2);
-        if (lane == 0) {
-            s_c1[wave] = l2;
-            s_dc[wave] = d2;
-        }
+    if (has_img) {
+#pragma unroll
+        for (int n = 0; n < IM::CB_LOADS; ++n) {
+            const int i = threadIdx.x + n * PF_THREADS;
+            if ((n + 1) * PF_THREADS <= IM::CB_UNITS || i < IM::CB_UNITS) reinterpret_cast<u32x4 *>(s_cb)[i] = iv[n];
+        }
+#pragma unroll
+        for (int n = 0; n < KS; ++n) {
+            s_frag[threadIdx.x + n * PF_THREADS] = iv[IM::CB_LOADS + n];
+            s_fragl[threadIdx.x + n * PF_THREADS] = iv[IM::CB_LOADS + KS + n];
+        }
+    } else {
+        pf_codebook_stage<D, DR>(cw, s_cb, s_frag, s_fragl, s_c1, s_dc, wave, lane);
     }
     __syncthreads();
     half8 ch[SH::A_REGS ? 8 : 1];
@@ -367,12 +331,9 @@
         if constexpr (SH::A_REGS) return ch[rb];
         else return __builtin_bit_cast(half8, s_frag[(rb * KS + s) * 64 + lane]);
     };
-    unsigned c2b = __float_as_uint(s_c1[0]), dcb = __float_as_uint(s_dc[0]);
-#pragma unroll
-    for (int w = 1; w < PF_WAVES; ++w) {
-        c2b = max(c2b, __float_as_uint(s_c1[w]));
-        dcb = max(dcb, __float_as_uint(s_dc[w]));
-    }
+    unsigned c2b = fold[0], dcb = fold[1];
+    if (!has_img) pf_codebook_fold(s_c1, s_dc, c2b, dcb);
+    if (a.img_dump != nullptr && blockIdx.x == 0) pf_image_write<D>(a.img_dump, s_cb, s_frag, s_fragl, c2b, dcb);
     const float c2 = __builtin_sqrtf(__uint_as_float(c2b)) * 1.0000002f, dc = __builtin_sqrtf(__uint_as_float(dcb)) * 1.0000002f;
     const bool cb_ok = c2b < 0x4E800000u && dcb < 0x4E800000u;
     const float err_rel = cb_ok ? c2 * SH::ERR_REL + 1.001f * dc : INFINITY;
@@ -896,6 +857,11 @@
     write_minmax_partials<PF_WAVES>(lmin, lmax, ws, sawnan);
 }
 
+struct PfImageArg {
+    const void *img = nullptr;
+    void *dump = nullptr;
+};
+
 static int64_t pf16_grid(int64_t ntiles, int bpc) {
     int64_t blocks = (ntiles + PF_WAVES - 1) / PF_WAVES;
     int64_t cap = (int64_t)cu_count() * bpc;
@@ -906,7 +872,7 @@
 
 template <typename CodeT, int D, int DR, int NRB>
 static int launch_pf_rows(const float *grad, const float *codebook, int64_t M, int K, CodeT *codes, float *u, float *ws,
-                          hipStream_t st, int profile_slot) {
+                          hipStream_t st, int profile_slot, PfImageArg im) {
     if (M > 0x7FFFFFFFLL) return fail(GQ_ERR_UNSUPPORTED, "gq_hsq_encode: prefilter path needs M < 2^31");
     static const int bpc = resident_blocks_per_cu(hsq_encode_pf_kernel<CodeT, D, false, false, true, DR, NRB>, PF_THREADS, 0);
     PfArgs a = {};
@@ -917,6 +883,8 @@
     a.cb = codebook;
     a.ws = ws;
     a.K = K;
+    a.img = static_cast<const u32x4 *>(im.img);
+    a.img_dump = static_cast<u32x4 *>(im.dump);
     const int64_t blocks = pf16_grid((M + 63) / 64, bpc);
     pf_split(a, (M + 63) / 64, blocks);
     hipEvent_t ev_start, ev_stop;
@@ -933,24 +901,30 @@
 
 template <typename CodeT, int D, int DR = D>
 static int launch_pf(const float *grad, const float *codebook, int64_t M, int K, CodeT *codes, float *u, float *ws,
-                     hipStream_t st, int profile_slot) {
+                     hipStream_t st, int profile_slot, PfImageArg im) {
     if constexpr (sizeof(CodeT) == 1) {
-        if (K <= 32) return launch_pf_rows<CodeT, D, DR, 1>(grad, codebook, M, K, codes, u, ws, st, profile_slot);
-        if (K <= 64) return launch_pf_rows<CodeT, D, DR, 2>(grad, codebook, M, K, codes, u, ws, st, profile_slot);
-    }
-    return launch_pf_rows<CodeT, D, DR, 8>(grad, codebook, M, K, codes, u, ws, st, profile_slot);
+        if (K <= 32) return launch_pf_rows<CodeT, D, DR, 1>(grad, codebook, M, K, codes, u, ws, st, profile_slot, im);
+        if (K <= 64) return launch_pf_rows<CodeT, D, DR, 2>(grad, codebook, M, K, codes, u, ws, st, profile_slot, im);
+    }
+    return launch_pf_rows<CodeT, D, DR, 8>(grad, codebook, M, K, codes, u, ws, st, profile_slot, im);
+}
+
+template <typename CodeT>
+static int launch_encode_pf_image(const float *grad, const float *codebook, int64_t M, int d, int K, CodeT *codes, float *u, float *ws,
+                                  hipStream_t st, int profile_slot, PfImageArg im) {
+    if (K < 4 || K > 256 || (K & 3)) return fail(GQ_ERR_INVALID_ARG, "gq_hsq_encode: the prefilter kernel was asked for K = %d", K);
+    if (d == 16) return launch_pf<CodeT, 16>(grad, codebook, M, K, codes, u, ws, st, profile_slot, im);
+    if (d == 32) return launch_pf<CodeT, 32>(grad, codebook, M, K, codes, u, ws, st, profile_slot, im);
+    if (d == 8) return launch_pf<CodeT, 8>(grad, codebook, M, K, codes, u, ws, st, profile_slot, im);
+    if (d == 12) return launch_pf<CodeT, 16, 12>(grad, codebook, M, K, codes, u, ws, st, profile_slot, im);
+    if (d == 24) return launch_pf<CodeT, 32, 24>(grad, codebook, M, K, codes, u, ws, st, profile_slot, im);
+    return fail(GQ_ERR_INVALID_ARG, "gq_hsq_encode: the prefilter kernel was asked for d = %d", d);
 }
 
 template <typename CodeT>
 int launch_encode_pf(const float *grad, const float *codebook, int64_t M, int d, int K, CodeT *codes, float *u, float *ws,
                      hipStream_t st, int profile_slot) {
-    if (K < 4 || K > 256 || (K & 3)) return fail(GQ_ERR_INVALID_ARG, "gq_hsq_encode: the prefilter kernel was asked for K = %d", K);
-    if (d == 16) return launch_pf<CodeT, 16>(grad, codebook, M, K, codes, u, ws, st, profile_slot);
-    if (d == 32) return launch_pf<CodeT, 32>(grad, codebook, M, K, codes, u, ws, st, profile_slot);
-    if (d == 8) return launch_pf<CodeT, 8>(grad, codebook, M, K, codes, u, ws, st, profile_slot);
-    if (d == 12) return launch_pf<CodeT, 16, 12>(grad, codebook, M, K, codes, u, ws, st, profile_slot);
-    if (d == 24) return launch_pf<CodeT, 32, 24>(grad, codebook, M, K, codes, u, ws, st, profile_slot);
-    return fail(GQ_ERR_INVALID_ARG, "gq_hsq_encode: the prefilter kernel was asked for d = %d", d);
+    return launch_encode_pf_image<CodeT>(grad, codebook, M, d, K, codes, u, ws, st, profile_slot, PfImageArg{});
 }
 
 template int launch_encode_pf<uint8_t>(const float *, const float *, int64_t, int, int, uint8_t *, float *, float *, hipStream_t, int);
@@ -962,7 +936,7 @@
 template <int D, bool EF, int DR, int NRB>
 static int encode_batched_rows(const char *what, const int64_t *seg_table, const int32_t *tile_seg, int nseg, int64_t ntiles,
                                const float *codebook, int K, uint8_t *wire, float *u_flat, uint32_t *seg_minmax, float *workspace,
-                               float ef_scale, int profile_slot, void *stream) {
+                               float ef_scale, int profile_slot, void *stream, const void *image) {
     if (nseg < 1 || ntiles < 1 || ntiles * 64 > 0x7FFFFFFFLL)
         return fail(GQ_ERR_INVALID_ARG, "%s: bad sizes nseg=%d ntiles=%lld", what, nseg, (long long)ntiles);
     if (!seg_table || !tile_seg || !codebook || !wire || !u_flat || !seg_minmax || !workspace)
@@ -981,6 +955,7 @@
     a.ntiles = ntiles;
     a.nseg = nseg;
     a.ef_scale = ef_scale;
+    a.img = static_cast<const u32x4 *>(image);
     hipStream_t st = as_stream(stream);
     const int64_t blocks = pf16_grid(ntiles, bpc);
     pf_split(a, ntiles, blocks);
@@ -1002,12 +977,12 @@
 template <int D, bool EF, int DR = D>
 static int encode_batched(const char *what, const int64_t *seg_table, const int32_t *tile_seg, int nseg, int64_t ntiles,
                           const float *codebook, int K, uint8_t *wire, float *u_flat, uint32_t *seg_minmax, float *workspace,
-                          float ef_scale, int profile_slot, void *stream) {
+                          float ef_scale, int profile_slot, void *stream, const void *image) {
     if (K <= 32 && nseg <= PF_LDS_SEGS)
-        return encode_batched_rows<D, EF, DR, 1>(what, seg_table, tile_seg, nseg, ntiles, codebook, K, wire, u_flat, seg_minmax, workspace, ef_scale, profile_slot, stream);
+        return encode_batched_rows<D, EF, DR, 1>(what, seg_table, tile_seg, nseg, ntiles, codebook, K, wire, u_flat, seg_minmax, workspace, ef_scale, profile_slot, stream, image);
     if (K <= 64 && nseg <= PF_LDS_SEGS)
-        return encode_batched_rows<D, EF, DR, 2>(what, seg_table, tile_seg, nseg, ntiles, codebook, K, wire, u_flat, seg_minmax, workspace, ef_scale, profile_slot, stream);
-    return encode_batched_rows<D, EF, DR, 8>(what, seg_table, tile_seg, nseg, ntiles, codebook, K, wire, u_flat, seg_minmax, workspace, ef_scale, profile_slot, stream);
+        return encode_batched_rows<D, EF, DR, 2>(what, seg_table, tile_seg, nseg, ntiles, codebook, K, wire, u_flat, seg_minmax, workspace, ef_scale, profile_slot, stream, image);
+    return encode_batched_rows<D, EF, DR, 8>(what, seg_table, tile_seg, nseg, ntiles, codebook, K, wire, u_flat, seg_minmax, workspace, ef_scale, profile_slot, stream, image);
 }
 }
 
@@ -1035,17 +1010,17 @@
                                         seg_minmax, workspace, st);
 }
 
-GQ_INTERNAL int gqi_hsq_encode_batched_pf(const int64_t *seg_table, const int32_t *tile_seg, int nseg, int64_t ntiles,
-                                          const float *codebook, int d, int K, int ef, float ef_scale, uint8_t *wire, float *u_flat,
-                                          uint32_t *seg_minmax, float *workspace, int profile_slot, void *stream) {
+GQ_INTERNAL int gqi_hsq_encode_batched_pf_image(const int64_t *seg_table, const int32_t *tile_seg, int nseg, int64_t ntiles,
+                                                const float *codebook, int d, int K, int ef, float ef_scale, uint8_t *wire, float *u_flat,
+                                                uint32_t *seg_minmax, float *workspace, int profile_slot, const void *image, void *stream) {
     const char *what = "gq_hsq_encode_batched";
     if (K < 4 || K > 256 || (K & 3)) return gq::fail(GQ_ERR_UNSUPPORTED, "%s: the prefilter launch takes K <= 256, a multiple of 4 (K = %d)", what, K);
 #define GQ_PF_BATCHED(DD, DP)                                                                                             \
     if (d == DD)                                                                                                          \
         return ef ? gq::encode_batched<DP, true, DD>(what, seg_table, tile_seg, nseg, ntiles, codebook, K, wire, u_flat, seg_minmax, \
-                                                     workspace, ef_scale, profile_slot, stream)                           \
+                                                     workspace, ef_scale, profile_slot, stream, image)                    \
                   : gq::encode_batched<DP, false, DD>(what, seg_table, tile_seg, nseg, ntiles, codebook, K, wire, u_flat, seg_minmax, \
-                                                      workspace, 0.0f, profile_slot, stream);
+                                                      workspace, 0.0f, profile_slot, stream, image);
     GQ_PF_BATCHED(16, 16)
     GQ_PF_BATCHED(32, 32)
     GQ_PF_BATCHED(8, 8)
@@ -1054,3 +1029,78 @@
 #undef GQ_PF_BATCHED
     return gq::fail(GQ_ERR_UNSUPPORTED, "%s: d must be 8, 12, 16, 24 or 32 (K <= 256)", what);
 }
+
+GQ_INTERNAL int gqi_hsq_encode_batched_pf(const int64_t *seg_table, const int32_t *tile_seg, int nseg, int64_t ntiles,
+                                          const float *codebook, int d, int K, int ef, float ef_scale, uint8_t *wire, float *u_flat,
+                                          uint32_t *seg_minmax, float *workspace, int profile_slot, void *stream) {
+    return gqi_hsq_encode_batched_pf_image(seg_table, tile_seg, nseg, ntiles, codebook, d, K, ef, ef_scale, wire, u_flat, seg_minmax,
+                                           workspace, profile_slot, nullptr, stream);
+}
+
+namespace gq {
+
+template <int D, int DR>
+__global__ __launch_bounds__(PF_THREADS, 1) void hsq_pf_image_kernel(const float *__restrict__ cb, int K, u32x4 *__restrict__ image) {
+    typedef PfShape<D> SH;
+    __shared__ __attribute__((aligned(16))) float s_cb[64 * SH::QS];
+    __shared__ __attribute__((aligned(16))) u32x4 s_frag[8 * SH::KS * 64], s_fragl[8 * SH::KS * 64];
+    __shared__ float s_c1[PF_WAVES], s_dc[PF_WAVES];
+    const int lane = threadIdx.x & 63, wave = __builtin_amdgcn_readfirstlane((int)(threadIdx.x >> 6));
+    PfCodebookWords<D, DR> cw;
+    pf_codebook_request<D, DR>(cw, cb, K, wave, lane);
+    pf_codebook_stage<D, DR>(cw, s_cb, s_frag, s_fragl, s_c1, s_dc, wave, lane);
+    __syncthreads();
+    unsigned c2b, dcb;
+    pf_codebook_fold(s_c1, s_dc, c2b, dcb);
+    pf_image_write<D>(image, s_cb, s_frag, s_fragl, c2b, dcb);
+}
+
+static size_t pf_image_bytes(int d) {
+    if (d == 8) return (size_t)PfImage<8>::UNITS * 16;
+    if (d == 12 || d == 16) return (size_t)PfImage<16>::UNITS * 16;
+    if (d == 24 || d == 32) return (size_t)PfImage<32>::UNITS * 16;
+    return 0;
+}
+
+}
+
+GQ_INTERNAL size_t gqi_hsq_image_bytes(int d, int K) {
+    if (K < 4 || K > 256 || (K & 3)) return 0;
+    return gq::pf_image_bytes(d);
+}
+
+GQ_INTERNAL int gqi_hsq_image_prepare(const float *codebook, int d, int K, void *image, void *stream) {
+    const char *what = "gq_hsq_image_prepare";
+    if (!codebook || !image) return gq::fail(GQ_ERR_INVALID_ARG, "%s: null pointer", what);
+    if (gqi_hsq_image_bytes(d, K) == 0)
+        return gq::fail(GQ_ERR_UNSUPPORTED, "%s: d must be 8, 12, 16, 24 or 32 and K <= 256, a multiple of 4 (d = %d, K = %d)", what, d, K);
+    if (((uintptr_t)image & 15) != 0 || ((uintptr_t)codebook & 15) != 0)
+        return gq::fail(GQ_ERR_INVALID_ARG, "%s: codebook and image must be 16-byte aligned", what);
+    hipStream_t st = gq::as_stream(stream);
+    gq::u32x4 *out = static_cast<gq::u32x4 *>(image);
+    if (d == 16) hipLaunchKernelGGL(HIP_KERNEL_NAME(gq::hsq_pf_image_kernel<16, 16>), dim3(1), dim3(gq::PF_THREADS), 0, st, codebook, K, out);
+    else if (d == 32) hipLaunchKernelGGL(HIP_KERNEL_NAME(gq::hsq_pf_image_kernel<32, 32>), dim3(1), dim3(gq::PF_THREADS), 0, st, codebook, K, out);
+    else if (d == 8) hipLaunchKernelGGL(HIP_KERNEL_NAME(gq::hsq_pf_image_kernel<8, 8>), dim3(1), dim3(gq::PF_THREADS), 0, st, codebook, K, out);
+    else if (d == 12) hipLaunchKernelGGL(HIP_KERNEL_NAME(gq::hsq_pf_image_kernel<16, 12>), dim3(1), dim3(gq::PF_THREADS), 0, st, codebook, K, out);
+    else hipLaunchKernelGGL(HIP_KERNEL_NAME(gq::hsq_pf_image_kernel<32, 24>), dim3(1), dim3(gq::PF_THREADS), 0, st, codebook, K, out);
+    GQ_CHECK_LAUNCH(what);
+    return GQ_OK;
+}
+
+GQ_INTERNAL int gqi_hsq_encode_pf_image(const float *grad, const float *codebook, int64_t M, int d, int K, void *codes, int code_bytes,
+                                        float *u, float *workspace, int profile_slot, const void *image, void *image_dump, void *stream) {
+    const char *what = "gq_hsq_image_encode";
+    if (M < 1 || !grad || !codebook || !codes || !u || !workspace) return gq::fail(GQ_ERR_INVALID_ARG, "%s: bad size or null pointer", what);
+    if (gqi_hsq_image_bytes(d, K) == 0)
+        return gq::fail(GQ_ERR_UNSUPPORTED, "%s: d must be 8, 12, 16, 24 or 32 and K <= 256, a multiple of 4 (d = %d, K = %d)", what, d, K);
+    if (((uintptr_t)grad & 15) != 0 || ((uintptr_t)codebook & 15) != 0 || ((uintptr_t)image & 15) != 0 || ((uintptr_t)image_dump & 15) != 0)
+        return gq::fail(GQ_ERR_INVALID_ARG, "%s: grad, codebook and image must be 16-byte aligned", what);
+    if (profile_slot >= GQ_PROFILE_SLOTS) return gq::fail(GQ_ERR_INVALID_ARG, "%s: profile_slot %d", what, profile_slot);
+    const gq::PfImageArg im = {image, image_dump};
+    hipStream_t st = gq::as_stream(stream);
+    if (code_bytes == 1)
+        return gq::launch_encode_pf_image<uint8_t>(grad, codebook, M, d, K, static_cast<uint8_t *>(codes), u, workspace, st, profile_slot, im);
+    if (code_bytes == 4)
+        return gq::launch_encode_pf_image<int32_t>(grad, codebook, M, d, K, static_cast<int32_t *>(codes), u, workspace, st, profile_slot, im);
+    return gq::fail(GQ_ERR_INVALID_ARG, "%s: code_bytes must be 1 or 4", what);
+}
diff --git a/gradient-quantization_amd/csrc/hsq_image.hip b/gradient-quantization_amd/csrc/hsq_image.hip
--- /dev/null
+++ b/gradient-quantization_amd/csrc/hsq_image.hip
@@ -0,0 +1,34 @@
+#include <math.h>
+
+#include "gq_hsq_image.h"
+#include "gq_internal.h"
+
+GQ_API int gq_hsq_image_abi_version(void) { return GQ_HSQ_IMAGE_ABI_VERSION; }
+
+GQ_API const char *gq_hsq_image_last_error(void) { return gq_last_error(); }
+
+GQ_API size_t gq_hsq_image_bytes(int d, int K) { return gqi_hsq_image_bytes(d, K); }
+
+GQ_API int gq_hsq_image_prepare(const float *codebook, int d, int K, void *image, void *stream) {
+    return gqi_hsq_image_prepare(codebook, d, K, image, stream);
+}
+
+GQ_API int gq_hsq_image_encode(const float *grad, const float *codebook, const void *image, int64_t M, int d, int K, void *codes,
+                               int code_bytes, float *u, float *minmax_partials, int profile_slot, void *image_dump, void *stream) {
+    return gqi_hsq_encode_pf_image(grad, codebook, M, d, K, codes, code_bytes, u, minmax_partials, profile_slot, image, image_dump,
+                                   stream);
+}
+
+GQ_API int gq_hsq_image_encode_batched(const gq_hsq_batch *b, const void *image, uint8_t *wire, float ef_scale, void *stream) {
+    const char *what = "gq_hsq_image_encode_batched";
+    if (gq_hsq_batched_path(b) != GQ_BATCH_PREFILTER)
+        return gq::fail(GQ_ERR_UNSUPPORTED, "%s: the descriptor's path is not GQ_BATCH_PREFILTER", what);
+    if (!wire || !b->u_flat || !b->seg_minmax || !b->workspace) return gq::fail(GQ_ERR_INVALID_ARG, "%s: null pointer", what);
+    if (((uintptr_t)image & 15) != 0) return gq::fail(GQ_ERR_INVALID_ARG, "%s: the image must be 16-byte aligned", what);
+    const int ef = isnan(ef_scale) ? 0 : 1;
+    return gqi_hsq_encode_batched_pf_image(b->seg_table, b->tile_seg, b->nseg, b->ntiles, b->codebook, b->d, b->K, ef,
+                                           ef ? ef_scale : 0.0f, wire, b->u_flat, b->seg_minmax, b->workspace, b->profile_slot, image,
+                                           stream);
+}
+
+GQ_API int gq_hsq_image_profile_read(int slot, float *kernel_ms) { return gq_profile_read(slot, kernel_ms); }
diff --git a/gradient-quantization_amd/csrc/hsq_pf_image.hpp b/gradient-quantization_amd/csrc/hsq_pf_image.hpp
--- /dev/null
+++ b/gradient-quantization_amd/csrc/hsq_pf_image.hpp
@@ -0,0 +1,130 @@
+#pragma once
+#include "hsq_pf_common.hpp"
+
+#ifndef GQ_PF_PAIR
+#define GQ_PF_PAIR -1
+#endif
+
+namespace gq {
+
+constexpr int PF_WAVES = 8;
+constexpr int PF_THREADS = PF_WAVES * 64;
+
+template <int D>
+struct PfShape {
+    static_assert(D == 8 || D == 16 || D == 32, "the prefilter kernel is built for D = 8, 16 and 32");
+    static constexpr int KS = D > 16 ? D / 16 : 1;
+    static constexpr bool HALF = D < 16;
+    static constexpr int QS = 4 * D + 4;
+    static constexpr int QCAP = D > 16 ? 32 : 64;
+    static constexpr bool A_REGS = D <= 16;
+    static constexpr int NF = 4 * KS;
+    static constexpr bool PAIR = GQ_PF_PAIR < 0 ? D > 16 : GQ_PF_PAIR != 0;
+    static constexpr float ERR_REL = (D > 16 ? 1.05f : 1.03f) * 4.8828125e-04f;
+    static constexpr float ERR2_REL = (D > 16 ? 2.3f : 1.2f) * 7.62939453125e-06f;
+    static constexpr float ERR2_SUB = D > 16 ? 3.5e-7f : 2.4e-7f;
+};
+
+template <int D>
+struct PfImage {
+    static constexpr int CB_UNITS = 16 * PfShape<D>::QS;
+    static constexpr int FRAG_UNITS = 8 * PfShape<D>::KS * 64;
+    static constexpr int FOLD_UNIT = CB_UNITS + 2 * FRAG_UNITS;
+    static constexpr int UNITS = FOLD_UNIT + 1;
+    static constexpr int CB_LOADS = (CB_UNITS + PF_THREADS - 1) / PF_THREADS;
+    static constexpr int LOADS = CB_LOADS + 2 * PfShape<D>::KS;
+    static_assert(FRAG_UNITS == PfShape<D>::KS * PF_THREADS, "one fragment unit per thread and k-step");
+};
+
+template <int D, int DR>
+struct PfCodebookWords {
+    float cbv[256 * DR / PF_THREADS];
+    f32x4 aq[2 * PfShape<D>::KS];
+};
+
+template <int D, int DR>
+__device__ __forceinline__ bool pf_frag_ok(int s, int q, int h) { return DR == D || 16 * s + 4 * q + 4 + 8 * h <= DR; }
+
+template <int D, int DR>
+__device__ __forceinline__ void pf_codebook_request(PfCodebookWords<D, DR> &w, const float *__restrict__ cb, int K, int wave, int lane) {
+    constexpr int KS = PfShape<D>::KS;
+    constexpr bool HALF = PfShape<D>::HALF;
+    const int j = lane & 31, h = lane >> 5;
+#pragma unroll
+    for (int n = 0; n < 256 * DR / PF_THREADS; ++n) w.cbv[n] = (int)threadIdx.x + n * PF_THREADS < K * DR ? cb[threadIdx.x + n * PF_THREADS] : 0.0f;
+#pragma unroll
+    for (int i = 0; i < 2 * KS; ++i) w.aq[i] = f32x4{0.0f, 0.0f, 0.0f, 0.0f};
+    if ((!HALF || h == 0) && wave * 32 + j < K) {
+#pragma unroll
+        for (int s = 0; s < KS; ++s) {
+            if (pf_frag_ok<D, DR>(s, 0, h)) w.aq[2 * s] = *reinterpret_cast<const f32x4 *>(cb + (wave * 32 + j) * DR + 16 * s + (HALF ? 0 : 8 * h));
+            if (pf_frag_ok<D, DR>(s, 1, h)) w.aq[2 * s + 1] = *reinterpret_cast<const f32x4 *>(cb + (wave * 32 + j) * DR + 16 * s + (HALF ? 0 : 8 * h) + 4);
+        }
+    }
+}
+
+template <int D, int DR>
+__device__ __forceinline__ void pf_codebook_stage(const PfCodebookWords<D, DR> &w, float *s_cb, u32x4 *s_frag, u32x4 *s_fragl, float *s_c1,
+                                                  float *s_dc, int wave, int lane) {
+    constexpr int KS = PfShape<D>::KS, QS = PfShape<D>::QS;
+#pragma unroll
+    for (int n = 0; n < 256 * DR / PF_THREADS; ++n) {
+        const int i = threadIdx.x + n * PF_THREADS, k = i / DR, jj = i % DR;
+        s_cb[(k >> 2) * QS + 4 * jj + (k & 3)] = w.cbv[n];
+    }
+    if constexpr (DR != D) {
+#pragma unroll
+        for (int n = 0; n < 256 * (D - DR) / PF_THREADS; ++n) {
+            const int i = threadIdx.x + n * PF_THREADS, k = i / (D - DR), jj = DR + i % (D - DR);
+            s_cb[(k >> 2) * QS + 4 * jj + (k & 3)] = 0.0f;
+        }
+    }
+    float l2 = 0.0f, d2 = 0.0f;
+#pragma unroll
+    for (int s = 0; s < KS; ++s) {
+        half8 fh, fl;
+#pragma unroll
+        for (int e = 0; e < 8; ++e) {
+            const float x = e < 4 ? w.aq[2 * s][e] : w.aq[2 * s + 1][e - 4];
+            fh[e] = (_Float16)x;
+            const float rr = x - (float)fh[e];
+            fl[e] = (_Float16)rr;
+            l2 = __fmaf_rn(x, x, l2);
+            d2 = __fmaf_rn(rr, rr, d2);
+        }
+        s_frag[(wave * KS + s) * 64 + lane] = __builtin_bit_cast(u32x4, fh);
+        s_fragl[(wave * KS + s) * 64 + lane] = __builtin_bit_cast(u32x4, fl);
+    }
+    l2 += __shfl_xor(l2, 32, 64);
+    d2 += __shfl_xor(d2, 32, 64);
+    l2 = wave_max_nan(l2);
+    d2 = wave_max_nan(d2);
+    if (lane == 0) {
+        s_c1[wave] = l2;
+        s_dc[wave] = d2;
+    }
+}
+
+__device__ __forceinline__ void pf_codebook_fold(const float *s_c1, const float *s_dc, unsigned &c2b, unsigned &dcb) {
+    c2b = __float_as_uint(s_c1[0]), dcb = __float_as_uint(s_dc[0]);
+#pragma unroll
+    for (int w = 1; w < PF_WAVES; ++w) {
+        c2b = max(c2b, __float_as_uint(s_c1[w]));
+        dcb = max(dcb, __float_as_uint(s_dc[w]));
+    }
+}
+
+template <int D>
+__device__ __forceinline__ void pf_image_write(u32x4 *__restrict__ image, const float *s_cb, const u32x4 *s_frag, const u32x4 *s_fragl,
+                                               unsigned c2b, unsigned dcb) {
+    typedef PfImage<D> IM;
+    for (int i = threadIdx.x; i < IM::CB_UNITS; i += PF_THREADS)
+        image[i] = i % (D + 1) == D ? u32x4{0u, 0u, 0u, 0u} : reinterpret_cast<const u32x4 *>(s_cb)[i];
+    for (int i = threadIdx.x; i < IM::FRAG_UNITS; i += PF_THREADS) {
+        image[IM::CB_UNITS + i] = s_frag[i];
+        image[IM::CB_UNITS + IM::FRAG_UNITS + i] = s_fragl[i];
+    }
+    if (threadIdx.x == 0) image[IM::FOLD_UNIT] = u32x4{c2b, dcb, 0u, 0u};
+}
+
+}
diff --git a/gradient-quantization_amd/gq_amd/native.py b/gradient-quantization_amd/gq_amd/native.py
--- a/gradient-quantization_amd/gq_amd/native.py
+++ b/gradient-quantization_amd/gq_amd/native.py
@@ -1,5 +1,6 @@
 import ctypes
 import os
+import weakref
 
 import torch
 
@@ -122,8 +123,111 @@
 
 def profile_read(slot):
     ms = ctypes.c_float(0.0)
-    _check(lib().gq_profile_read(ctypes.c_int(slot), ctypes.byref(ms)), "gq_profile_read")
+    if _slot_in_image_lib.get(slot):
+        _check_image(image_lib().gq_hsq_image_profile_read(ctypes.c_int(slot), ctypes.byref(ms)), "gq_hsq_image_profile_read")
+    else:
+        _check(lib().gq_profile_read(ctypes.c_int(slot), ctypes.byref(ms)), "gq_profile_read")
     return ms.value
+
+
+IMAGE_EXPORTS = ["gq_hsq_image_abi_version", "gq_hsq_image_last_error", "gq_hsq_image_bytes", "gq_hsq_image_prepare",
+                 "gq_hsq_image_encode", "gq_hsq_image_encode_batched", "gq_hsq_image_profile_read"]
+IMAGE_ABI_VERSION = 1
+
+
+def _image_twin(path):
+    d, base = os.path.split(path)
+    return os.path.join(d, base.replace("libgq_hsq", "libgq_hsq_image", 1) if base.startswith("libgq_hsq") else base + ".image.so")
+
+
+IMAGE_LIB_PATH = os.environ.get("GQ_IMAGE_LIB_PATH") or _image_twin(LIB_PATH)
+IMAGE_ON = [os.environ.get("GQ_HSQ_IMAGE", "0") == "1" and (not os.environ.get("GQ_LIB_PATH") or os.path.exists(IMAGE_LIB_PATH))]
+_image_lib = None
+_slot_in_image_lib = {}
+
+
+def image_lib():
+    global _image_lib
+    if _image_lib is None:
+        if not os.path.exists(IMAGE_LIB_PATH):
+            raise GQNativeError("libgq_hsq_image.so not found at %s -- build it with `python gradient-quantization_amd/build.py` "
+                                "(there is no CPU fallback)" % IMAGE_LIB_PATH)
+        L = ctypes.CDLL(IMAGE_LIB_PATH)
+        L.gq_hsq_image_last_error.restype = ctypes.c_char_p
+        L.gq_hsq_image_abi_version.restype = ctypes.c_int
+        L.gq_hsq_image_bytes.restype = ctypes.c_size_t
+        for name in IMAGE_EXPORTS:
+            getattr(L, name)
+        if L.gq_hsq_image_abi_version() != IMAGE_ABI_VERSION:
+            raise GQNativeError("%s has ABI version %d, this binding is written for %d: rebuild it"
+                                % (IMAGE_LIB_PATH, L.gq_hsq_image_abi_version(), IMAGE_ABI_VERSION))
+        _image_lib = L
+    return _image_lib
+
+
+def _check_image(rc, what):
+    CALLS[0] += 1
+    if rc != 0:
+        raise GQNativeError("%s failed (%d): %s" % (what, rc, image_lib().gq_hsq_image_last_error().decode()))
+
+
+def hsq_image_shape_ok(d, K):
+    return d in (8, 12, 16, 24, 32) and 4 <= K <= 256 and K % 4 == 0
+
+
+class _ImageEntry(object):
+    __slots__ = ("ref", "version", "image", "ptr")
+
+
+_images = {}
+
+
+def hsq_image(codebook):
+    ent = _images.get(id(codebook))
+    if ent is not None and ent.version == codebook._version:
+        return ent
+    return _prepare_image(codebook, ent)
+
+
+def hsq_image_refresh(codebook):
+    return _prepare_image(codebook, _images.get(id(codebook)))
+
+
+def _prepare_image(codebook, ent):
+    K, d = int(codebook.shape[0]), int(codebook.shape[1])
+    cbp = _dev_ptr(codebook, torch.float32, "codebook")
+    if torch.cuda.is_current_stream_capturing():
+        raise GQNativeError("the codebook's image must be prepared before a stream capture begins (native.hsq_image(codebook))")
+    L = image_lib()
+    if ent is None:
+        nbytes = int(L.gq_hsq_image_bytes(ctypes.c_int(d), ctypes.c_int(K)))
+        if nbytes == 0:
+            raise GQNativeError("no prepared image for a codebook of d = %d, K = %d" % (d, K))
+        ent = _ImageEntry()
+        key = id(codebook)
+        ent.ref = weakref.ref(codebook, lambda _r, key=key: _images.pop(key, None))
+        ent.image = torch.empty(nbytes, dtype=torch.uint8, device=codebook.device)
+        ent.ptr = ctypes.c_void_p(ent.image.data_ptr())
+        _images[key] = ent
+    version = codebook._version
+    rc = L.gq_hsq_image_prepare(cbp, ctypes.c_int(d), ctypes.c_int(K), ent.ptr, _stream())
+    if rc != 0:
+        raise GQNativeError("gq_hsq_image_prepare failed (%d): %s" % (rc, L.gq_hsq_image_last_error().decode()))
+    ent.version = version
+    return ent
+
+
+def hsq_image_dump(grad, codebook, codes, u, partials):
+    K, d = codebook.shape
+    M = grad.numel() // d
+    L = image_lib()
+    dump = torch.zeros(int(L.gq_hsq_image_bytes(ctypes.c_int(d), ctypes.c_int(K))), dtype=torch.uint8, device=codebook.device)
+    rc = L.gq_hsq_image_encode(_dev_ptr(grad, torch.float32, "grad"), _dev_ptr(codebook, torch.float32, "codebook"), None,
+                               ctypes.c_int64(M), ctypes.c_int(d), ctypes.c_int(K), _dev_ptr(codes, None, "codes"),
+                               ctypes.c_int(_CODE_BYTES[codes.dtype]), _dev_ptr(u, torch.float32, "u"),
+                               _dev_ptr(partials, torch.float32, "partials"), ctypes.c_int(-1), ctypes.c_void_p(dump.data_ptr()), _stream())
+    _check_image(rc, "gq_hsq_image_encode")
+    return dump
 
 
 def device_info(device=0):
@@ -133,11 +237,24 @@
     return cus.value, arch.value.decode()
 
 
-def hsq_encode(grad, codebook, codes, u, partials, impl=ENCODE_AUTO, profile_slot=-1):
+def hsq_encode(grad, codebook, codes, u, partials, impl=ENCODE_AUTO, profile_slot=-1, image=None):
     K, d = codebook.shape
     M = grad.numel() // d
     assert grad.numel() == M * d and codes.numel() == M and u.numel() == M
     assert partials.numel() >= workspace_floats(M), "encode workspace too small: use native.new_workspace(device, M)"
+    if profile_slot >= 0:
+        _slot_in_image_lib[profile_slot] = False
+    if ((IMAGE_ON[0] if image is None else image) and impl in (ENCODE_AUTO, ENCODE_PREFILTER_D16K256) and hsq_image_shape_ok(d, K)
+            and grad.data_ptr() % 16 == 0 and codebook.data_ptr() % 16 == 0 and M < 2 ** 31):
+        ent = hsq_image(codebook)
+        rc = image_lib().gq_hsq_image_encode(_dev_ptr(grad, torch.float32, "grad"), _dev_ptr(codebook, torch.float32, "codebook"),
+                                             ent.ptr, ctypes.c_int64(M), ctypes.c_int(d), ctypes.c_int(K), _dev_ptr(codes, None, "codes"),
+                                             ctypes.c_int(_CODE_BYTES[codes.dtype]), _dev_ptr(u, torch.float32, "u"),
+                                             _dev_ptr(partials, torch.float32, "partials"), ctypes.c_int(profile_slot), None, _stream())
+        _check_image(rc, "gq_hsq_image_encode")
+        if profile_slot >= 0:
+            _slot_in_image_lib[profile_slot] = True
+        return
     rc = lib().gq_hsq_encode_ex(_dev_ptr(grad, torch.float32, "grad"), _dev_ptr(codebook, torch.float32, "codebook"),
                                 ctypes.c_int64(M), ctypes.c_int(d), ctypes.c_int(K), _dev_ptr(codes, None, "codes"),
                                 ctypes.c_int(_CODE_BYTES[codes.dtype]), _dev_ptr(u, torch.float32, "u"),
@@ -270,6 +387,15 @@
                                  opt(seg_minmax, torch.int32, "seg_minmax"), opt(workspace, torch.float32, "workspace"), None, 0, 0)
         self.ref = ctypes.byref(self.s)
         self.path = int(self.L.gq_hsq_batched_path(self.ref))
+        self.use_image = IMAGE_ON[0] and self.path == BATCH_PREFILTER and workspace is not None and codebook.data_ptr() % 16 == 0
+        self.image = None
+        if self.use_image and not torch.cuda.is_current_stream_capturing():
+            self.prepare_image()
+
+    def prepare_image(self):
+        if self.use_image:
+            self.image = hsq_image(self.keep[2])
+        return self.image
 
     def set_table(self, seg_table):
         self.keep_table = seg_table
@@ -294,6 +420,15 @@
 
     def encode(self, wire, ef_scale=None, profile_slot=-1):
         self.s.profile_slot = profile_slot
+        if profile_slot >= 0:
+            _slot_in_image_lib[profile_slot] = self.use_image
+        if self.use_image:
+            ent = self.prepare_image()
+            rc = image_lib().gq_hsq_image_encode_batched(self.ref, ent.ptr, self._wire(wire),
+                                                         ctypes.c_float(_NAN if ef_scale is None else ef_scale), _stream())
+            self.s.profile_slot = -1
+            _check_image(rc, "gq_hsq_image_encode_batched")
+            return
         rc = self.L.gq_hsq_encode_batched(self.ref, self._wire(wire), ctypes.c_float(_NAN if ef_scale is None else ef_scale),
                                           _stream())
         self.s.profile_slot = -1
diff --git a/gradient-quantization_amd/gq_amd/quantizers.py b/gradient-quantization_amd/gq_amd/quantizers.py
--- a/gradient-quantization_amd/gq_amd/quantizers.py
+++ b/gradient-quantization_amd/gq_amd/quantizers.py
@@ -516,9 +516,17 @@
             skip.update(self.dense_idx)
         return skip
 
+    def _prepare_images(self):
+        for g in self._groups:
+            b = getattr(g[2], "_batch", None)
+            for hb in (b, getattr(b, "b1", None)):
+                if isinstance(hb, native.HSQBatch):
+                    hb.prepare_image()
+
     def _capture_record(self, ent, all_grads, wire, slot, user, salt, scale, dev, generic=False):
         try:
             headers = None if generic else [g[2]._host[g[2]._last_slot].to(dev) for g in self._groups]
+            self._prepare_images()
             with _capturing(self._direct) as graph:
                 self._record_launches(all_grads, wire, slot, user, salt, scale, None, dev, headers=headers, table_current=generic)
             ent[1], ent[2] = _replayable(graph, self._direct), headers
@@ -529,6 +537,7 @@
     def _capture_step(self, fent, headers, all_grads, wire, slot, user, salt, scale, dev):
         after = ([g[2]._out_turn for g in self._groups], self._dense_turn)
         try:
+            self._prepare_images()
             with _capturing(self._direct) as graph:
                 resets = []
                 fuse = self._can_fuse_levels()
@@ -550,6 +559,7 @@
             self._set_turns((graph_key[2], graph_key[3]))
             hdrs2 = [g[2]._host[g[2]._last_slot].to(gathered.device) for g in self._groups] if self.two_phase else None
             calls = self._phase2_calls
+            self._prepare_images()
             with _capturing(self._direct) as graph:
                 again = self._decode_all(gathered, self.two_phase, (), phase2_headers=hdrs2)
             if self._phase2_calls != calls:
diff --git a/include/gq_hsq_image.h b/include/gq_hsq_image.h
--- /dev/null
+++ b/include/gq_hsq_image.h
@@ -0,0 +1,31 @@
+#ifndef GQ_HSQ_IMAGE_H
+#define GQ_HSQ_IMAGE_H
+
+#include <stddef.h>
+#include <stdint.h>
+
+#include "gq_hsq.h"
+
+#ifdef __cplusplus
+extern "C" {
+#endif
+
+#define GQ_HSQ_IMAGE_ABI_VERSION 1
+int gq_hsq_image_abi_version(void);
+const char *gq_hsq_image_last_error(void);
+
+size_t gq_hsq_image_bytes(int d, int K);
+
+int gq_hsq_image_prepare(const float *codebook, int d, int K, void *image, void *stream);
+
+int gq_hsq_image_encode(const float *grad, const float *codebook, const void *image, int64_t M, int d, int K, void *codes,
+                        int code_bytes, float *u, float *minmax_partials, int profile_slot, void *image_dump, void *stream);
+
+int gq_hsq_image_encode_batched(const gq_hsq_batch *b, const void *image, uint8_t *wire, float ef_scale, void *stream);
+
+int gq_hsq_image_profile_read(int slot, float *kernel_ms);
+
+#ifdef __cplusplus
+}
+#endif
+#endif
```
